# JeffreyXiang/ivid

Hardware: NVIDIA H100
Metric: 128x128 RGBD multiview samples/sec (higher is better)
Workload: dtype fp16 tensor-core operands, fp32 accumulate / residual stream / GroupNorm / softmax / sampler

## Files before the change

### include/ivid_b200.h

```cpp
#ifndef IVID_B200_H_
#define IVID_B200_H_

#include <stdint.h>

#ifdef __cplusplus
extern "C" {
#endif

#define IVID_OK 0
#define IVID_ERR_INVALID_ARGUMENT 1
#define IVID_ERR_NOT_IMPLEMENTED 2
#define IVID_ERR_CUDA 3
#define IVID_ERR_STATE 4

typedef struct ivid_unet ivid_unet_t;
typedef struct ivid_sampler ivid_sampler_t;

const char* ivid_last_error(void);
int ivid_version(void);
int ivid_device_info(int device, int* sm_count, int* cc_major, int* cc_minor);


int ivid_unet_create(const char* cfg_json, ivid_unet_t** out);
int ivid_unet_destroy(ivid_unet_t* h);

int ivid_unet_num_params(const ivid_unet_t* h, int* count);
int ivid_unet_param_info(const ivid_unet_t* h, int index, const char** name, int64_t shape[4], int* ndim,
                         int* is_buffer);
int ivid_unet_set_param(ivid_unet_t* h, const char* name, const float* host_data, const int64_t* shape, int ndim);
int ivid_unet_finalize(ivid_unet_t* h, int device);
int ivid_unet_set_precision(ivid_unet_t* h, int precision);
int ivid_fp8_e4m3_quantize(const float* in, uint8_t* out, uint64_t count);
int ivid_fp8_weight_exponent(const float* w, uint64_t count, int* e_out);
int ivid_unet_weight_arena(const ivid_unet_t* h, void** dev_ptr, uint64_t* bytes);

int ivid_unet_forward(ivid_unet_t* h, const float* x_dev, int Nx, const int64_t* t_dev, const int64_t* classes_dev,
                      float* eps_dev, int N, void* stream);

int ivid_conv_tile(int H, int W, int* tw, int* th, int* tn, int* fused_stats);

int ivid_unet_debug_tap(ivid_unet_t* h, int N, const char* layer, float* host_out, uint64_t capacity, int* C, int* H, int* W);

int ivid_unet_profile_begin(ivid_unet_t* h);
int ivid_unet_profile_end(ivid_unet_t* h, char* json_out, int capacity);

typedef struct {
  int kind;
  const float* y_dev;
  const float* mask_dev;
  const float* mask_rgb_dev;
  const float* noise_dev;
  uint64_t seed;
  uint32_t stream_id;
  int sr_scale;
} ivid_cond_t;
int ivid_unet_forward_cond(ivid_unet_t* h, const float* x_dev, int Nx, const ivid_cond_t* cond, const int64_t* t_dev,
                           const int64_t* classes_dev, float* eps_dev, int N, void* stream);

int ivid_unet_forward_hw(ivid_unet_t* h, const float* x_dev, int Nx, int H, int W, const ivid_cond_t* cond,
                         const int64_t* t_dev, const int64_t* classes_dev, float* eps_dev, int N, void* stream);

int ivid_unet_forward_reuse(ivid_unet_t* h, const float* x_dev, int Nx, int H, int W, const ivid_cond_t* cond,
                            const int64_t* t_dev, const int64_t* classes_dev, float* eps_dev, int N, int cache_branch,
                            void* stream);

int ivid_unet_forward_perturbed(ivid_unet_t* h, const float* x_dev, int Nx, int H, int W, const ivid_cond_t* cond,
                                const int64_t* t_dev, const int64_t* classes_dev, float* eps_dev, int N, int row0,
                                const int* layers_host, int num_layers, int cache_branch, void* stream);


int ivid_sampler_create(const double* betas, int timesteps, ivid_sampler_t** out);
int ivid_sampler_destroy(ivid_sampler_t* s);
int ivid_sampler_table(const ivid_sampler_t* s, int which, double* out, int count);

typedef struct {
  int kind;
  int use_cfg;
  float strength;
  int clip_denoised;
  float eta;
  const int64_t* classes_dev;
  ivid_cond_t cond;
  const float* replace_rgb_dev;
  const float* replace_rgb_mask_dev;
  double replace_rgb_weight;
  const float* replace_depth_dev;
  const float* replace_depth_mask_dev;
  double replace_depth_weight;
  const float* constrain_depth_dev;
  double constrain_depth_weight;
  const float* step_noise_dev;
  uint64_t seed;
  int height, width;
  int order;
  const float* prev_x0_dev;
  int t_last;
  int sde;
  int guidance_interval;
  int guidance_t_lo;
  int guidance_t_hi;
  int cache_interval;
  int cache_branch;
  int cache_reuse;
  int unipc;
  const float* prev2_x0_dev;
  int t_last2;
  const float* prev3_x0_dev;
  int t_last3;
  const float* prev_xt_dev;
  float* corrected_xt_dev;
  int pag;
  float pag_scale;
  const int* pag_layers;
  int pag_num_layers;
  int apg;
  double apg_eta;
  double apg_norm;
  double apg_momentum;
  float* apg_state_dev;
  int start_step;
  int dynamic_threshold;
  double threshold_ratio;
  double threshold_max;
} ivid_step_args_t;

int ivid_sampler_step(ivid_sampler_t* s, ivid_unet_t* unet, const float* x_t_dev, float* x_prev_dev,
                      float* pred_x0_dev, int N, int t, int t_prev, const ivid_step_args_t* args, void* stream);

int ivid_sampler_step_dev(ivid_sampler_t* s, ivid_unet_t* unet, const float* x_t_dev, float* x_prev_dev,
                          float* pred_x0_dev, int N, const int64_t* t_dev, const int64_t* t_prev_dev,
                          const ivid_step_args_t* args, void* stream);

int ivid_op_dynamic_threshold(const float* x_dev, int N, int M, double ratio, double threshold_max, float* s_out_dev,
                              float* x_out_dev, void* stream);

int ivid_op_apg(const float* d_c_dev, const float* d_u_dev, float* state_inout_dev, int N, int M, float s, double eta,
                double r, double beta, float* out_dev, void* stream);

int ivid_cfg_mix(const float* eps2n_dev, float strength, float* out_dev, uint64_t count, void* stream);

int ivid_guidance_mix(const float* eps_dev, uint64_t count, int cfg, float strength, int pag, float pag_scale, float* out_dev,
                      void* stream);

int ivid_sampler_run(ivid_sampler_t* s, ivid_unet_t* unet, float* x_inout_dev, int N, int steps,
                     const ivid_step_args_t* args, const float* noise_all_dev, const float* cond_noise_all_dev,
                     float* traj_x0_dev, float* traj_xt_dev, void* stream);

int ivid_sampler_diffuse(ivid_sampler_t* s, const float* x0_dev, const float* noise_dev, int N, uint64_t count_per_sample,
                         int t, uint64_t seed, float* out_dev, void* stream);

typedef struct ivid_warp ivid_warp_t;
typedef struct {
  double fov_deg;
  double near;
  double far;
  double atol;
  double rtol;
  int erode_rgb;
  double padding;
} ivid_warp_params_t;

int ivid_warp_create(int image_size, int render_size, int max_views, int batch, double near, double far, int device,
                     ivid_warp_t** out);
int ivid_warp_destroy(ivid_warp_t* w);
int ivid_warp_reset(ivid_warp_t* w);
int ivid_warp_num_views(const ivid_warp_t* w, int* n);
int ivid_warp_add_view(ivid_warp_t* w, const float* rgbd_dev, const float* modelviews_host, int shared_modelview,
                       const ivid_warp_params_t* params, void* stream);
int ivid_warp_mesh_from_depth(ivid_warp_t* w, const float* lin_depth_host, const float* modelview_host,
                              const ivid_warp_params_t* params, float* verts_host, uint32_t* faces_host, void* stream);
int ivid_warp_set_mesh(ivid_warp_t* w, int sample, int view, const float* verts_host, const uint32_t* faces_host,
                       const float* color_host, const float* modelview_host);
int ivid_warp_get_mesh(ivid_warp_t* w, int sample, int view, float* verts_host, uint32_t* faces_host, float* color_host);
int ivid_warp_render(ivid_warp_t* w, const float* target_mv_host, int shared_modelview, double fov_deg, float* color_dev,
                     float* depth_dev, float* mask_color_dev, float* mask_depth_dev, void* stream);
int ivid_warp_aggregate(ivid_warp_t* w, const float* target_mv_host, int shared_modelview, const ivid_warp_params_t* params,
                        float* cond_dev, void* stream);
int ivid_warp_postfilter(ivid_warp_t* w, const float* color_dev, const float* depth_dev, const float* mask_color_dev,
                         const float* mask_depth_dev, const ivid_warp_params_t* params, float* cond_dev, void* stream);

int ivid_warp_resolve_frame(ivid_warp_t* w, double project_near, double project_far, const uint8_t* lut_host, uint8_t* color8_host,
                            uint8_t* depth8_host, void* stream);

int ivid_warp_render_simple(ivid_warp_t* w, const float* verts_host, int nverts, const uint32_t* faces_host, int nfaces,
                            const float* color_host, const float* target_mv_host, double fov_deg, float* color_out_host,
                            float* depth_out_host, float* mask_out_host, void* stream);
int ivid_warp_forward_backward(ivid_warp_t* w, const float* lin_depth0_host, const float* color0_host, const float* mv1_host,
                               const float* mv0_host, int shared_modelview, const ivid_warp_params_t* params, float* out_host,
                               void* stream);

typedef struct {
  float origin[3];
  float voxel;
  int dims[3];
} ivid_fusion_grid_t;
int ivid_fusion_integrate(const float* depth_dev, const uint8_t* valid_dev, const float* color_dev, const float* modelviews_host,
                          int num_views, int image_size, float focal, const ivid_fusion_grid_t* grid, float trunc,
                          float* tsdf_sum_dev, float* weight_dev, float* color_sum_dev, float* color_weight_dev, void* stream);
int ivid_fusion_extract(const ivid_fusion_grid_t* grid, const float* tsdf_sum_dev, const float* weight_dev, const float* color_sum_dev,
                        const float* color_weight_dev, int64_t max_vertices, int64_t max_faces, float* vertices_dev,
                        uint8_t* colors_dev, int64_t* faces_dev, int64_t* num_vertices, int64_t* num_faces, void* stream);


int ivid_op_conv2d(const void* act_dev, int N, int H, int W, int Cin, const float* w_host, const float* bias_host,
                   int Cout, int ksize, const void* act2_dev, int Cin2, const float* w2_host, const float* bias2_host,
                   const float* residual_dev, void* out_dev, int out_fp16, void* stream);
int ivid_op_conv2d_e4m3(const void* act_dev, int N, int H, int W, int Cin, const float* w_host, const float* bias_host,
                        int Cout, int ksize, const void* act2_dev, int Cin2, const float* w2_host, const float* bias2_host,
                        const float* residual_dev, void* out_dev, int out_fp16, int* e_out, void* stream);
int ivid_op_group_norm(const float* x0_dev, int C0, const float* x1_dev, int C1, int N, int H, int W, int groups,
                       float eps, const float* gamma_host, const float* beta_host, const float* film_dev ,
                       int silu, int mode, void* out_fp16_dev, void* stream);
int ivid_op_group_norm_e4m3(const float* x0_dev, int C0, const float* x1_dev, int C1, int N, int H, int W, int groups,
                            float eps, const float* gamma_host, const float* beta_host, const float* film_dev,
                            int silu, int mode, void* out_e4m3_dev, void* stream);
typedef struct {
  const void* act0_dev; int C0; int ksize; const float* w0_host; const float* b0_host;
  int e4m3; int* e_out;
  const void* act1_dev; int C1; const void* act2_dev; int C2; const float* wskip_host; const float* bskip_host;
  const float* residual_dev; int residual_up;
  int N, H, W, Cout;
  void* out_dev; int out_mode; void* out16_dev; double* stats_dev;
} ivid_op_conv_t;
int ivid_op_conv2d_ex(const ivid_op_conv_t* args, void* stream);
typedef struct {
  const void* x0_dev; int C0; const void* x1_dev; int C1; int x_fp16;
  const double* stats0_dev; const double* stats1_dev;
  int N, H, W, groups; float eps;
  const float* gamma_host; const float* beta_host;
  const float* film_dev; int film_ld; int film_off; int film_add;
  int silu, mode;
  void* out_dev; int out_e4m3; void* out_lo_dev; void* out_raw16_dev; float* out_raw32_dev;
} ivid_op_gn_t;
int ivid_op_group_norm_apply(const ivid_op_gn_t* args, void* stream);
int ivid_op_gn_stats(const float* x_dev, int N, int H, int W, int C, double* stats_dev, void* stream);
typedef struct {
  int mode, conv;
  const void* x_dev; int N, H, W, C;
  const float* w_host; const float* b_host;
  float* out_dev; void* out16_dev; double* stats_dev; void* operand_dev;
} ivid_op_resample_t;
int ivid_op_resample(const ivid_op_resample_t* args, void* stream);
int ivid_op_attention(const void* qkv_dev, int N, int T, int C, void* out_dev, void* stream);
int ivid_op_attention_heads(const void* qkv_dev, int N, int T, int C, int head_channels, void* out_dev, void* stream);
int ivid_op_attention_perturbed(const void* qkv_dev, int N, int T, int C, int head_channels, int row0, void* out_dev,
                                void* stream);

#ifdef __cplusplus
}
#endif
#endif
```

### ivid_b200/_lib.py

```python
from __future__ import annotations

import ctypes
import os
from ctypes import POINTER, Structure, byref, c_char_p, c_double, c_float, c_int, c_int64, c_uint32, c_uint64, c_void_p

_HERE = os.path.dirname(os.path.abspath(__file__))
LIB_PATH = os.path.join(_HERE, "libivid_b200.so")

IVID_OK = 0
IVID_ERR_INVALID_ARGUMENT = 1
IVID_ERR_NOT_IMPLEMENTED = 2
IVID_ERR_CUDA = 3
IVID_ERR_STATE = 4


class CondT(Structure):
    _fields_ = [
        ("kind", c_int),
        ("y_dev", c_void_p),
        ("mask_dev", c_void_p),
        ("mask_rgb_dev", c_void_p),
        ("noise_dev", c_void_p),
        ("seed", c_uint64),
        ("stream_id", c_uint32),
        ("sr_scale", c_int),
    ]


class StepArgsT(Structure):
    _fields_ = [
        ("kind", c_int),
        ("use_cfg", c_int),
        ("strength", c_float),
        ("clip_denoised", c_int),
        ("eta", c_float),
        ("classes_dev", c_void_p),
        ("cond", CondT),
        ("replace_rgb_dev", c_void_p),
        ("replace_rgb_mask_dev", c_void_p),
        ("replace_rgb_weight", c_double),
        ("replace_depth_dev", c_void_p),
        ("replace_depth_mask_dev", c_void_p),
        ("replace_depth_weight", c_double),
        ("constrain_depth_dev", c_void_p),
        ("constrain_depth_weight", c_double),
        ("step_noise_dev", c_void_p),
        ("seed", c_uint64),
        ("height", c_int),
        ("width", c_int),
        ("order", c_int),
        ("prev_x0_dev", c_void_p),
        ("t_last", c_int),
        ("sde", c_int),
        ("guidance_interval", c_int),
        ("guidance_t_lo", c_int),
        ("guidance_t_hi", c_int),
        ("cache_interval", c_int),
        ("cache_branch", c_int),
        ("cache_reuse", c_int),
        ("unipc", c_int),
        ("prev2_x0_dev", c_void_p),
        ("t_last2", c_int),
        ("prev3_x0_dev", c_void_p),
        ("t_last3", c_int),
        ("prev_xt_dev", c_void_p),
        ("corrected_xt_dev", c_void_p),
        ("pag", c_int),
        ("pag_scale", c_float),
        ("pag_layers", POINTER(c_int)),
        ("pag_num_layers", c_int),
        ("apg", c_int),
        ("apg_eta", c_double),
        ("apg_norm", c_double),
        ("apg_momentum", c_double),
        ("apg_state_dev", c_void_p),
        ("start_step", c_int),
        ("dynamic_threshold", c_int),
        ("threshold_ratio", c_double),
        ("threshold_max", c_double),
    ]


class OpConvT(Structure):
    _fields_ = [
        ("act0_dev", c_void_p), ("C0", c_int), ("ksize", c_int), ("w0_host", c_void_p), ("b0_host", c_void_p),
        ("e4m3", c_int), ("e_out", POINTER(c_int)),
        ("act1_dev", c_void_p), ("C1", c_int), ("act2_dev", c_void_p), ("C2", c_int), ("wskip_host", c_void_p),
        ("bskip_host", c_void_p),
        ("residual_dev", c_void_p), ("residual_up", c_int),
        ("N", c_int), ("H", c_int), ("W", c_int), ("Cout", c_int),
        ("out_dev", c_void_p), ("out_mode", c_int), ("out16_dev", c_void_p), ("stats_dev", c_void_p),
    ]


class OpGnT(Structure):
    _fields_ = [
        ("x0_dev", c_void_p), ("C0", c_int), ("x1_dev", c_void_p), ("C1", c_int), ("x_fp16", c_int),
        ("stats0_dev", c_void_p), ("stats1_dev", c_void_p),
        ("N", c_int), ("H", c_int), ("W", c_int), ("groups", c_int), ("eps", c_float),
        ("gamma_host", c_void_p), ("beta_host", c_void_p),
        ("film_dev", c_void_p), ("film_ld", c_int), ("film_off", c_int), ("film_add", c_int),
        ("silu", c_int), ("mode", c_int),
        ("out_dev", c_void_p), ("out_e4m3", c_int), ("out_lo_dev", c_void_p), ("out_raw16_dev", c_void_p),
        ("out_raw32_dev", c_void_p),
    ]


class OpResampleT(Structure):
    _fields_ = [
        ("mode", c_int), ("conv", c_int),
        ("x_dev", c_void_p), ("N", c_int), ("H", c_int), ("W", c_int), ("C", c_int),
        ("w_host", c_void_p), ("b_host", c_void_p),
        ("out_dev", c_void_p), ("out16_dev", c_void_p), ("stats_dev", c_void_p), ("operand_dev", c_void_p),
    ]


class WarpParamsT(Structure):
    _fields_ = [("fov_deg", c_double), ("near", c_double), ("far", c_double), ("atol", c_double), ("rtol", c_double),
                ("erode_rgb", c_int), ("padding", c_double)]


class FusionGridT(Structure):
    _fields_ = [("origin", c_float * 3), ("voxel", c_float), ("dims", c_int * 3)]


SIGNATURES = {
    "ivid_last_error": (c_char_p, []),
    "ivid_version": (c_int, []),
    "ivid_device_info": (c_int, [c_int, POINTER(c_int), POINTER(c_int), POINTER(c_int)]),
    "ivid_unet_create": (c_int, [c_char_p, POINTER(c_void_p)]),
    "ivid_unet_destroy": (c_int, [c_void_p]),
    "ivid_unet_num_params": (c_int, [c_void_p, POINTER(c_int)]),
    "ivid_unet_param_info": (c_int, [c_void_p, c_int, POINTER(c_char_p), POINTER(c_int64), POINTER(c_int), POINTER(c_int)]),
    "ivid_unet_set_param": (c_int, [c_void_p, c_char_p, c_void_p, POINTER(c_int64), c_int]),
    "ivid_unet_finalize": (c_int, [c_void_p, c_int]),
    "ivid_unet_weight_arena": (c_int, [c_void_p, POINTER(c_void_p), POINTER(c_uint64)]),
    "ivid_unet_set_precision": (c_int, [c_void_p, c_int]),
    "ivid_fp8_e4m3_quantize": (c_int, [c_void_p, c_void_p, c_uint64]),
    "ivid_fp8_weight_exponent": (c_int, [c_void_p, c_uint64, POINTER(c_int)]),
    "ivid_unet_forward": (c_int, [c_void_p, c_void_p, c_int, c_void_p, c_void_p, c_void_p, c_int, c_void_p]),
    "ivid_unet_forward_cond": (c_int, [c_void_p, c_void_p, c_int, POINTER(CondT), c_void_p, c_void_p, c_void_p, c_int, c_void_p]),
    "ivid_unet_forward_hw": (c_int, [c_void_p, c_void_p, c_int, c_int, c_int, POINTER(CondT), c_void_p, c_void_p, c_void_p, c_int,
                                     c_void_p]),
    "ivid_unet_forward_reuse": (c_int, [c_void_p, c_void_p, c_int, c_int, c_int, POINTER(CondT), c_void_p, c_void_p, c_void_p,
                                        c_int, c_int, c_void_p]),
    "ivid_unet_forward_perturbed": (c_int, [c_void_p, c_void_p, c_int, c_int, c_int, POINTER(CondT), c_void_p, c_void_p, c_void_p,
                                            c_int, c_int, POINTER(c_int), c_int, c_int, c_void_p]),
    "ivid_conv_tile": (c_int, [c_int, c_int, POINTER(c_int), POINTER(c_int), POINTER(c_int), POINTER(c_int)]),
    "ivid_unet_debug_tap": (c_int, [c_void_p, c_int, c_char_p, c_void_p, c_uint64, POINTER(c_int), POINTER(c_int), POINTER(c_int)]),
    "ivid_unet_profile_begin": (c_int, [c_void_p]),
    "ivid_unet_profile_end": (c_int, [c_void_p, c_char_p, c_int]),
    "ivid_sampler_create": (c_int, [POINTER(c_double), c_int, POINTER(c_void_p)]),
    "ivid_sampler_destroy": (c_int, [c_void_p]),
    "ivid_sampler_table": (c_int, [c_void_p, c_int, POINTER(c_double), c_int]),
    "ivid_sampler_step": (c_int, [c_void_p, c_void_p, c_void_p, c_void_p, c_void_p, c_int, c_int, c_int, POINTER(StepArgsT), c_void_p]),
    "ivid_sampler_step_dev": (c_int, [c_void_p, c_void_p, c_void_p, c_void_p, c_void_p, c_int, c_void_p, c_void_p, POINTER(StepArgsT), c_void_p]),
    "ivid_cfg_mix": (c_int, [c_void_p, c_float, c_void_p, c_uint64, c_void_p]),
    "ivid_guidance_mix": (c_int, [c_void_p, c_uint64, c_int, c_float, c_int, c_float, c_void_p, c_void_p]),
    "ivid_op_dynamic_threshold": (c_int, [c_void_p, c_int, c_int, c_double, c_double, c_void_p, c_void_p, c_void_p]),
    "ivid_op_apg": (c_int, [c_void_p, c_void_p, c_void_p, c_int, c_int, c_float, c_double, c_double, c_double, c_void_p, c_void_p]),
    "ivid_sampler_run": (c_int, [c_void_p, c_void_p, c_void_p, c_int, c_int, POINTER(StepArgsT), c_void_p, c_void_p, c_void_p, c_void_p, c_void_p]),
    "ivid_sampler_diffuse": (c_int, [c_void_p, c_void_p, c_void_p, c_int, c_uint64, c_int, c_uint64, c_void_p, c_void_p]),
    "ivid_op_conv2d": (c_int, [c_void_p, c_int, c_int, c_int, c_int, c_void_p, c_void_p, c_int, c_int, c_void_p, c_int,
                               c_void_p, c_void_p, c_void_p, c_void_p, c_int, c_void_p]),
    "ivid_op_group_norm": (c_int, [c_void_p, c_int, c_void_p, c_int, c_int, c_int, c_int, c_int, c_float, c_void_p, c_void_p,
                                   c_void_p, c_int, c_int, c_void_p, c_void_p]),
    "ivid_op_conv2d_e4m3": (c_int, [c_void_p, c_int, c_int, c_int, c_int, c_void_p, c_void_p, c_int, c_int, c_void_p, c_int,
                                    c_void_p, c_void_p, c_void_p, c_void_p, c_int, POINTER(c_int), c_void_p]),
    "ivid_op_group_norm_e4m3": (c_int, [c_void_p, c_int, c_void_p, c_int, c_int, c_int, c_int, c_int, c_float, c_void_p,
                                        c_void_p, c_void_p, c_int, c_int, c_void_p, c_void_p]),
    "ivid_op_conv2d_ex": (c_int, [POINTER(OpConvT), c_void_p]),
    "ivid_op_group_norm_apply": (c_int, [POINTER(OpGnT), c_void_p]),
    "ivid_op_gn_stats": (c_int, [c_void_p, c_int, c_int, c_int, c_int, c_void_p, c_void_p]),
    "ivid_op_resample": (c_int, [POINTER(OpResampleT), c_void_p]),
    "ivid_op_attention": (c_int, [c_void_p, c_int, c_int, c_int, c_void_p, c_void_p]),
    "ivid_op_attention_heads": (c_int, [c_void_p, c_int, c_int, c_int, c_int, c_void_p, c_void_p]),
    "ivid_op_attention_perturbed": (c_int, [c_void_p, c_int, c_int, c_int, c_int, c_int, c_void_p, c_void_p]),
    "ivid_warp_create": (c_int, [c_int, c_int, c_int, c_int, c_double, c_double, c_int, POINTER(c_void_p)]),
    "ivid_warp_destroy": (c_int, [c_void_p]),
    "ivid_warp_reset": (c_int, [c_void_p]),
    "ivid_warp_num_views": (c_int, [c_void_p, POINTER(c_int)]),
    "ivid_warp_add_view": (c_int, [c_void_p, c_void_p, c_void_p, c_int, POINTER(WarpParamsT), c_void_p]),
    "ivid_warp_mesh_from_depth": (c_int, [c_void_p, c_void_p, c_void_p, POINTER(WarpParamsT), c_void_p, c_void_p, c_void_p]),
    "ivid_warp_set_mesh": (c_int, [c_void_p, c_int, c_int, c_void_p, c_void_p, c_void_p, c_void_p]),
    "ivid_warp_get_mesh": (c_int, [c_void_p, c_int, c_int, c_void_p, c_void_p, c_void_p]),
    "ivid_warp_render": (c_int, [c_void_p, c_void_p, c_int, c_double, c_void_p, c_void_p, c_void_p, c_void_p, c_void_p]),
    "ivid_warp_aggregate": (c_int, [c_void_p, c_void_p, c_int, POINTER(WarpParamsT), c_void_p, c_void_p]),
    "ivid_warp_resolve_frame": (c_int, [c_void_p, c_double, c_double, c_void_p, c_void_p, c_void_p, c_void_p]),
    "ivid_warp_render_simple": (c_int, [c_void_p, c_void_p, c_int, c_void_p, c_int, c_void_p, c_void_p, c_double, c_void_p, c_void_p, c_void_p, c_void_p]),
    "ivid_warp_forward_backward": (c_int, [c_void_p, c_void_p, c_void_p, c_void_p, c_void_p, c_int, POINTER(WarpParamsT), c_void_p, c_void_p]),
    "ivid_warp_postfilter": (c_int, [c_void_p, c_void_p, c_void_p, c_void_p, c_void_p, POINTER(WarpParamsT), c_void_p, c_void_p]),
    "ivid_fusion_integrate": (c_int, [c_void_p, c_void_p, c_void_p, c_void_p, c_int, c_int, c_float, POINTER(FusionGridT), c_float,
                                      c_void_p, c_void_p, c_void_p, c_void_p, c_void_p]),
    "ivid_fusion_extract": (c_int, [POINTER(FusionGridT), c_void_p, c_void_p, c_void_p, c_void_p, c_int64, c_int64, c_void_p, c_void_p,
                                    c_void_p, POINTER(c_int64), POINTER(c_int64), c_void_p]),
}

_lib = None


def lib() -> ctypes.CDLL:
    global _lib
    if _lib is None:
        if not os.path.exists(LIB_PATH):
            raise ImportError(
                f"{LIB_PATH} not found: build it with `python -m ivid_b200.build` (ivid_b200 has no CPU fallback)")
        l = ctypes.CDLL(LIB_PATH)
        for name, (res, args) in SIGNATURES.items():
            try:
                fn = getattr(l, name)
            except AttributeError:
                continue
            fn.restype = res
            fn.argtypes = args
        _lib = l
    return _lib


def last_error() -> str:
    m = lib().ivid_last_error()
    return m.decode() if m else ""


def check(status: int) -> None:
    if status == IVID_OK:
        return
    msg = last_error()
    if status == IVID_ERR_INVALID_ARGUMENT:
        raise AssertionError(msg)
    if status == IVID_ERR_NOT_IMPLEMENTED:
        raise NotImplementedError(msg)
    raise RuntimeError(f"ivid_b200 native error {status}: {msg}")


def ptr(t) -> c_void_p:
    if t is None:
        return c_void_p(None)
    return c_void_p(t.data_ptr())


def cur_stream(device=None) -> c_void_p:
    import torch
    return c_void_p(torch.cuda.current_stream(device).cuda_stream)
```

### ivid_b200/csrc/api.cu

```cuda
#include <algorithm>
#include <cmath>
#include <cstring>
#include <memory>
#include <string>
#include <vector>

#include "../../include/ivid_b200.h"
#include "ops.h"
#include "sampler.h"
#include "unet.h"

using namespace ivid;

struct ivid_unet { std::unique_ptr<Unet> impl; };
struct ivid_sampler { std::unique_ptr<Sampler> impl; };

static thread_local std::string g_last_error;
namespace ivid { void set_last_error(const std::string& msg) { g_last_error = msg; } }

template <class F>
static int guarded(F&& f) {
  try {
    f();
    return IVID_OK;
  } catch (const Error& e) {
    g_last_error = e.what();
    return e.code;
  } catch (const std::exception& e) {
    g_last_error = e.what();
    return IVID_ERR_STATE;
  } catch (...) {
    g_last_error = "unknown error";
    return IVID_ERR_STATE;
  }
}

#define IVID_NOT_NULL(p) IVID_REQUIRE((p) != nullptr, #p " must not be NULL")

extern "C" {

const char* ivid_last_error(void) { return g_last_error.c_str(); }
int ivid_version(void) { return 100; }

int ivid_device_info(int device, int* sm_count_out, int* cc_major, int* cc_minor) {
  return guarded([&] {
    cudaDeviceProp prop;
    IVID_CHECK_CUDA(cudaGetDeviceProperties(&prop, device));
    if (sm_count_out) *sm_count_out = prop.multiProcessorCount;
    if (cc_major) *cc_major = prop.major;
    if (cc_minor) *cc_minor = prop.minor;
  });
}

int ivid_unet_create(const char* cfg_json, ivid_unet_t** out) {
  return guarded([&] {
    IVID_NOT_NULL(cfg_json);
    IVID_NOT_NULL(out);
    auto h = std::make_unique<ivid_unet>();
    h->impl = std::make_unique<Unet>(std::string(cfg_json));
    *out = h.release();
  });
}
int ivid_unet_destroy(ivid_unet_t* h) {
  return guarded([&] { delete h; });
}
int ivid_unet_num_params(const ivid_unet_t* h, int* count) {
  return guarded([&] {
    IVID_NOT_NULL(h); IVID_NOT_NULL(count);
    *count = static_cast<int>(h->impl->params().size());
  });
}
int ivid_unet_param_info(const ivid_unet_t* h, int index, const char** name, int64_t shape[4], int* ndim, int* is_buffer) {
  return guarded([&] {
    IVID_NOT_NULL(h);
    const auto& ps = h->impl->params();
    IVID_REQUIRE(index >= 0 && index < static_cast<int>(ps.size()), "parameter index out of range");
    const ParamSpec& p = ps[index];
    if (name) *name = p.name.c_str();
    if (ndim) *ndim = static_cast<int>(p.shape.size());
    if (shape) for (size_t i = 0; i < 4; ++i) shape[i] = i < p.shape.size() ? p.shape[i] : 1;
    if (is_buffer) *is_buffer = p.is_buffer ? 1 : 0;
  });
}
int ivid_unet_set_param(ivid_unet_t* h, const char* name, const float* host_data, const int64_t* shape, int ndim) {
  return guarded([&] {
    IVID_NOT_NULL(h); IVID_NOT_NULL(name); IVID_NOT_NULL(host_data); IVID_NOT_NULL(shape);
    h->impl->set_param(name, host_data, shape, ndim);
  });
}
int ivid_unet_finalize(ivid_unet_t* h, int device) {
  return guarded([&] {
    IVID_NOT_NULL(h);
    h->impl->finalize(device);
  });
}
int ivid_unet_set_precision(ivid_unet_t* h, int precision) {
  return guarded([&] {
    IVID_NOT_NULL(h);
    h->impl->set_precision(precision);
  });
}
int ivid_fp8_e4m3_quantize(const float* in, uint8_t* out, uint64_t count) {
  return guarded([&] {
    IVID_REQUIRE(count == 0 || (in != nullptr && out != nullptr), "in and out must not be NULL");
    for (uint64_t i = 0; i < count; ++i) out[i] = fp8_e4m3_from_float(in[i]);
  });
}
int ivid_fp8_weight_exponent(const float* w, uint64_t count, int* e_out) {
  return guarded([&] {
    IVID_REQUIRE(count == 0 || w != nullptr, "w must not be NULL");
    IVID_NOT_NULL(e_out);
    float mx = 0.f;
    for (uint64_t i = 0; i < count; ++i) mx = std::max(mx, std::fabs(w[i]));
    *e_out = fp8_weight_exponent(mx);
  });
}
int ivid_unet_weight_arena(const ivid_unet_t* h, void** dev_ptr, uint64_t* bytes) {
  return guarded([&] {
    IVID_NOT_NULL(h);
    if (!h->impl->finalized()) throw Error(kErrState, "weight arena requested before finalize");
    if (dev_ptr) *dev_ptr = h->impl->arena();
    if (bytes) *bytes = h->impl->arena_bytes();
  });
}
int ivid_unet_forward_hw(ivid_unet_t* h, const float* x_dev, int Nx, int H, int W, const ivid_cond_t* cond,
                         const int64_t* t_dev, const int64_t* classes_dev, float* eps_dev, int N, void* stream) {
  return guarded([&] {
    IVID_NOT_NULL(h); IVID_NOT_NULL(x_dev); IVID_NOT_NULL(t_dev); IVID_NOT_NULL(eps_dev);
    h->impl->forward(x_dev, Nx, H, W, cond, t_dev, classes_dev, eps_dev, N, static_cast<cudaStream_t>(stream));
  });
}
int ivid_unet_forward_reuse(ivid_unet_t* h, const float* x_dev, int Nx, int H, int W, const ivid_cond_t* cond,
                            const int64_t* t_dev, const int64_t* classes_dev, float* eps_dev, int N, int cache_branch,
                            void* stream) {
  return guarded([&] {
    IVID_NOT_NULL(h); IVID_NOT_NULL(x_dev); IVID_NOT_NULL(t_dev); IVID_NOT_NULL(eps_dev);
    IVID_REQUIRE(cache_branch >= 0, "cache_branch must be in [0, num_res_blocks]");
    h->impl->forward(x_dev, Nx, H, W, cond, t_dev, classes_dev, eps_dev, N, static_cast<cudaStream_t>(stream), nullptr,
                     cache_branch);
  });
}
int ivid_unet_forward_perturbed(ivid_unet_t* h, const float* x_dev, int Nx, int H, int W, const ivid_cond_t* cond,
                                const int64_t* t_dev, const int64_t* classes_dev, float* eps_dev, int N, int row0,
                                const int* layers_host, int num_layers, int cache_branch, void* stream) {
  return guarded([&] {
    IVID_NOT_NULL(h); IVID_NOT_NULL(x_dev); IVID_NOT_NULL(t_dev); IVID_NOT_NULL(eps_dev);
    IVID_REQUIRE(num_layers >= 1 && layers_host != nullptr, "perturbed forward: at least one attention layer");
    IVID_REQUIRE(row0 >= 0 && row0 <= N, "perturbed forward: row0 must lie in [0, N]");
    AttnPerturb pert;
    pert.row0 = row0;
    pert.layers.assign(layers_host, layers_host + num_layers);
    h->impl->forward(x_dev, Nx, H, W, cond, t_dev, classes_dev, eps_dev, N, static_cast<cudaStream_t>(stream), nullptr,
                     cache_branch, &pert);
  });
}
int ivid_unet_forward(ivid_unet_t* h, const float* x_dev, int Nx, const int64_t* t_dev, const int64_t* classes_dev,
                      float* eps_dev, int N, void* stream) {
  const int S = h != nullptr ? h->impl->cfg().image_size : 0;
  return ivid_unet_forward_hw(h, x_dev, Nx, S, S, nullptr, t_dev, classes_dev, eps_dev, N, stream);
}
int ivid_unet_forward_cond(ivid_unet_t* h, const float* x_dev, int Nx, const ivid_cond_t* cond, const int64_t* t_dev,
                           const int64_t* classes_dev, float* eps_dev, int N, void* stream) {
  if (cond == nullptr) return guarded([&] { IVID_NOT_NULL(cond); });
  const int S = h != nullptr ? h->impl->cfg().image_size : 0;
  return ivid_unet_forward_hw(h, x_dev, Nx, S, S, cond, t_dev, classes_dev, eps_dev, N, stream);
}

int ivid_conv_tile(int H, int W, int* tw, int* th, int* tn, int* fused_stats) {
  return guarded([&] {
    int a, b, c;
    conv_tile(H, W, &a, &b, &c);
    if (tw) *tw = a;
    if (th) *th = b;
    if (tn) *tn = c;
    if (fused_stats) *fused_stats = conv_can_fuse_stats(H, W) ? 1 : 0;
  });
}

int ivid_unet_debug_tap(ivid_unet_t* h, int N, const char* layer, float* host_out, uint64_t capacity, int* C, int* H, int* W) {
  return guarded([&] {
    IVID_NOT_NULL(h); IVID_NOT_NULL(layer);
    h->impl->debug_tap(N, layer, host_out, static_cast<size_t>(capacity), C, H, W);
  });
}

int ivid_unet_profile_begin(ivid_unet_t* h) {
  return guarded([&] { IVID_NOT_NULL(h); h->impl->profile_begin(); });
}
int ivid_unet_profile_end(ivid_unet_t* h, char* json_out, int capacity) {
  return guarded([&] {
    IVID_NOT_NULL(h); IVID_NOT_NULL(json_out);
    const std::string js = h->impl->profile_end();
    IVID_REQUIRE(static_cast<int>(js.size()) < capacity, "profile buffer too small");
    std::memcpy(json_out, js.c_str(), js.size() + 1);
  });
}

int ivid_sampler_create(const double* betas, int timesteps, ivid_sampler_t** out) {
  return guarded([&] {
    IVID_NOT_NULL(betas); IVID_NOT_NULL(out);
    auto s = std::make_unique<ivid_sampler>();
    s->impl = std::make_unique<Sampler>(betas, timesteps);
    *out = s.release();
  });
}
int ivid_sampler_destroy(ivid_sampler_t* s) {
  return guarded([&] { delete s; });
}
int ivid_sampler_table(const ivid_sampler_t* s, int which, double* out, int count) {
  return guarded([&] {
    IVID_NOT_NULL(s); IVID_NOT_NULL(out);
    const auto& t = s->impl->table(which);
    IVID_REQUIRE(count == static_cast<int>(t.size()), "table length mismatch");
    std::memcpy(out, t.data(), sizeof(double) * t.size());
  });
}
int ivid_sampler_step(ivid_sampler_t* s, ivid_unet_t* unet, const float* x_t_dev, float* x_prev_dev, float* pred_x0_dev,
                      int N, int t, int t_prev, const ivid_step_args_t* args, void* stream) {
  return guarded([&] {
    IVID_NOT_NULL(s); IVID_NOT_NULL(unet); IVID_NOT_NULL(x_t_dev); IVID_NOT_NULL(x_prev_dev); IVID_NOT_NULL(args);
    s->impl->step(*unet->impl, x_t_dev, x_prev_dev, pred_x0_dev, N, t, t_prev, *args, t, static_cast<cudaStream_t>(stream));
  });
}
int ivid_sampler_step_dev(ivid_sampler_t* s, ivid_unet_t* unet, const float* x_t_dev, float* x_prev_dev, float* pred_x0_dev,
                          int N, const int64_t* t_dev, const int64_t* t_prev_dev, const ivid_step_args_t* args, void* stream) {
  return guarded([&] {
    IVID_NOT_NULL(s); IVID_NOT_NULL(unet); IVID_NOT_NULL(x_t_dev); IVID_NOT_NULL(x_prev_dev); IVID_NOT_NULL(args); IVID_NOT_NULL(t_dev);
    IVID_REQUIRE(args->kind == 0 || t_prev_dev != nullptr, "DDIM / DPM-Solver++ step needs t_prev");
    s->impl->step(*unet->impl, x_t_dev, x_prev_dev, pred_x0_dev, N, 0, 0, *args, 0, static_cast<cudaStream_t>(stream), t_dev, t_prev_dev);
  });
}
int ivid_cfg_mix(const float* eps2n_dev, float strength, float* out_dev, uint64_t count, void* stream) {
  return guarded([&] {
    IVID_NOT_NULL(eps2n_dev); IVID_NOT_NULL(out_dev);
    launch_cfg_mix(eps2n_dev, out_dev, static_cast<size_t>(count), strength, static_cast<cudaStream_t>(stream));
  });
}
int ivid_guidance_mix(const float* eps_dev, uint64_t count, int cfg, float strength, int pag, float pag_scale, float* out_dev,
                      void* stream) {
  return guarded([&] {
    IVID_NOT_NULL(eps_dev); IVID_NOT_NULL(out_dev);
    launch_guidance_mix(eps_dev, out_dev, static_cast<size_t>(count), cfg, strength, pag, pag_scale, static_cast<cudaStream_t>(stream));
  });
}
int ivid_op_dynamic_threshold(const float* x_dev, int N, int M, double ratio, double threshold_max, float* s_out_dev,
                              float* x_out_dev, void* stream) {
  return guarded([&] {
    IVID_NOT_NULL(x_dev); IVID_NOT_NULL(s_out_dev); IVID_NOT_NULL(x_out_dev);
    cudaStream_t st = static_cast<cudaStream_t>(stream);
    launch_dynamic_threshold(x_dev, N, M, ratio, threshold_max, s_out_dev, x_out_dev, st);
    IVID_CHECK_CUDA(cudaStreamSynchronize(st));
  });
}
int ivid_op_apg(const float* d_c_dev, const float* d_u_dev, float* state_inout_dev, int N, int M, float s, double eta,
                double r, double beta, float* out_dev, void* stream) {
  return guarded([&] {
    IVID_NOT_NULL(d_c_dev); IVID_NOT_NULL(d_u_dev); IVID_NOT_NULL(state_inout_dev); IVID_NOT_NULL(out_dev);
    cudaStream_t st = static_cast<cudaStream_t>(stream);
    launch_apg(d_c_dev, d_u_dev, state_inout_dev, N, M, s, eta, r, beta, out_dev, st);
    IVID_CHECK_CUDA(cudaStreamSynchronize(st));
  });
}
int ivid_sampler_run(ivid_sampler_t* s, ivid_unet_t* unet, float* x_inout_dev, int N, int steps,
                     const ivid_step_args_t* args, const float* noise_all_dev, const float* cond_noise_all_dev,
                     float* traj_x0_dev, float* traj_xt_dev, void* stream) {
  return guarded([&] {
    IVID_NOT_NULL(s); IVID_NOT_NULL(unet); IVID_NOT_NULL(x_inout_dev); IVID_NOT_NULL(args);
    s->impl->run(*unet->impl, x_inout_dev, N, steps, *args, noise_all_dev, cond_noise_all_dev, traj_x0_dev, traj_xt_dev,
                 static_cast<cudaStream_t>(stream));
  });
}
int ivid_sampler_diffuse(ivid_sampler_t* s, const float* x0_dev, const float* noise_dev, int N, uint64_t count_per_sample,
                         int t, uint64_t seed, float* out_dev, void* stream) {
  return guarded([&] {
    IVID_NOT_NULL(s); IVID_NOT_NULL(x0_dev); IVID_NOT_NULL(out_dev);
    s->impl->diffuse(x0_dev, noise_dev, N, static_cast<size_t>(count_per_sample), t, seed, out_dev,
                     static_cast<cudaStream_t>(stream));
  });
}

namespace {
struct DevBuf {
  void* p = nullptr;
  explicit DevBuf(size_t bytes) { if (bytes > 0) IVID_CHECK_CUDA(cudaMalloc(&p, bytes)); }
  ~DevBuf() { if (p) cudaFree(p); }
  DevBuf(const DevBuf&) = delete;
};
}

int ivid_op_conv2d_ex(const ivid_op_conv_t* a, void* stream) {
  return guarded([&] {
    IVID_NOT_NULL(a);
    IVID_NOT_NULL(a->act0_dev); IVID_NOT_NULL(a->w0_host); IVID_NOT_NULL(a->out_dev);
    IVID_REQUIRE(a->ksize == 3 || a->ksize == 1, "conv: kernel size must be 3 or 1");
    IVID_REQUIRE(a->C0 > 0 && a->C0 % 8 == 0 && a->C1 % 8 == 0 && a->C2 % 8 == 0, "conv: channels must be multiples of 8");
    IVID_REQUIRE(a->act1_dev == nullptr || a->wskip_host != nullptr, "conv: a skip input needs its weights (w2_host; wskip_host of ivid_op_conv2d_ex)");
    IVID_REQUIRE(a->act2_dev == nullptr || (a->act1_dev != nullptr && a->C2 > 0), "conv: act2_dev is the second part of a skip over act1_dev");
    IVID_REQUIRE(a->out_mode >= 0 && a->out_mode <= 2, "conv: out_mode must be 0, 1 or 2");
    const int C1 = a->act1_dev ? a->C1 : 0, C2 = a->act2_dev ? a->C2 : 0;
    const ConvPack pk = conv_pack(a->w0_host, a->b0_host, a->Cout, a->C0, a->ksize, conv_pad_k(a->C0), C1 ? a->wskip_host : nullptr,
                                  C1 ? a->bskip_host : nullptr, C1 + C2, C2 ? C1 : 0, a->e4m3 != 0);
    if (pk.refused != nullptr) throw Error(kErrInvalidArgument, std::string("conv: no e4m3 form: ") + pk.refused);
    cudaStream_t st = static_cast<cudaStream_t>(stream);
    DevBuf dw8(pk.w8.size()), dw(pk.w16.size() * 2), db(pk.bias.size() * 4);
    if (pk.e4m3) IVID_CHECK_CUDA(cudaMemcpyAsync(dw8.p, pk.w8.data(), pk.w8.size(), cudaMemcpyHostToDevice, st));
    if (pk.K > 0) IVID_CHECK_CUDA(cudaMemcpyAsync(dw.p, pk.w16.data(), pk.w16.size() * 2, cudaMemcpyHostToDevice, st));
    IVID_CHECK_CUDA(cudaMemcpyAsync(db.p, pk.bias.data(), pk.bias.size() * 4, cudaMemcpyHostToDevice, st));
    ConvDesc d;
    d.act0 = a->act0_dev; d.C0 = a->C0; d.taps0 = a->ksize * a->ksize;
    if (C1) { d.act1 = a->act1_dev; d.C1 = C1; d.taps1 = 1; }
    if (C2) { d.act2 = a->act2_dev; d.C2 = C2; d.taps2 = 1; }
    d.weight = dw.p; d.weight8 = dw8.p; d.acc_scale = std::ldexp(1.0f, -pk.e);
    d.cout_pad = pk.cout_pad; d.cout = a->Cout; d.bias = static_cast<const float*>(db.p);
    d.residual = a->residual_dev; d.ldr = a->Cout; d.residual_up = a->residual_up != 0;
    d.out = a->out_dev; d.ldc = a->Cout; d.out_mode = a->out_mode; d.out16 = a->out16_dev; d.stats = a->stats_dev;
    d.N = a->N; d.H = a->H; d.W = a->W;
    std::unique_ptr<ConvLaunch, void (*)(ConvLaunch*)> l(conv_launch_create(d), conv_launch_destroy);
    conv_launch_run(l.get(), st);
    IVID_CHECK_CUDA(cudaStreamSynchronize(st));
    if (a->e_out) *a->e_out = pk.e;
  });
}

static int op_conv2d(const void* act_dev, int N, int H, int W, int Cin, const float* w_host, const float* bias_host, int Cout,
                     int ksize, const void* act2_dev, int Cin2, const float* w2_host, const float* bias2_host,
                     const float* residual_dev, void* out_dev, int out_fp16, bool e4m3, int* e_out, void* stream) {
  ivid_op_conv_t a{};
  a.act0_dev = act_dev; a.C0 = Cin; a.ksize = ksize; a.w0_host = w_host; a.b0_host = bias_host;
  a.e4m3 = e4m3 ? 1 : 0; a.e_out = e_out;
  a.act1_dev = act2_dev; a.C1 = act2_dev ? Cin2 : 0; a.wskip_host = w2_host; a.bskip_host = bias2_host;
  a.residual_dev = residual_dev;
  a.N = N; a.H = H; a.W = W; a.Cout = Cout;
  a.out_dev = out_dev; a.out_mode = out_fp16 ? 1 : 0;
  return ivid_op_conv2d_ex(&a, stream);
}

int ivid_op_conv2d(const void* act_dev, int N, int H, int W, int Cin, const float* w_host, const float* bias_host,
                   int Cout, int ksize, const void* act2_dev, int Cin2, const float* w2_host, const float* bias2_host,
                   const float* residual_dev, void* out_dev, int out_fp16, void* stream) {
  return op_conv2d(act_dev, N, H, W, Cin, w_host, bias_host, Cout, ksize, act2_dev, Cin2, w2_host, bias2_host, residual_dev,
                   out_dev, out_fp16, false, nullptr, stream);
}
int ivid_op_conv2d_e4m3(const void* act_dev, int N, int H, int W, int Cin, const float* w_host, const float* bias_host,
                        int Cout, int ksize, const void* act2_dev, int Cin2, const float* w2_host, const float* bias2_host,
                        const float* residual_dev, void* out_dev, int out_fp16, int* e_out, void* stream) {
  return op_conv2d(act_dev, N, H, W, Cin, w_host, bias_host, Cout, ksize, act2_dev, Cin2, w2_host, bias2_host, residual_dev,
                   out_dev, out_fp16, true, e_out, stream);
}

int ivid_op_group_norm_apply(const ivid_op_gn_t* a, void* stream) {
  return guarded([&] {
    IVID_NOT_NULL(a);
    IVID_NOT_NULL(a->x0_dev); IVID_NOT_NULL(a->gamma_host); IVID_NOT_NULL(a->beta_host); IVID_NOT_NULL(a->out_dev);
    const int N = a->N, HW = a->H * a->W, C0 = a->C0, C1 = a->x1_dev ? a->C1 : 0, C = C0 + C1;
    IVID_REQUIRE(N > 0 && HW > 0 && C0 > 0, "group norm: empty tensor");
    IVID_REQUIRE(a->film_dev == nullptr || a->film_ld >= a->film_off + (a->film_add ? C : 2 * C),
                 "group norm: the FiLM row (film_off + C, or + 2C with a shift) must fit film_ld");
    const bool need0 = a->stats0_dev == nullptr, need1 = C1 > 0 && a->stats1_dev == nullptr;
    IVID_REQUIRE(!(need0 || need1) || !a->x_fp16, "group norm: statistics of fp16 sources must be supplied");
    cudaStream_t st = static_cast<cudaStream_t>(stream);
    DevBuf dg(C * 4), dbt(C * 4), st0(need0 ? static_cast<size_t>(N) * C0 * 16 : 0), st1(need1 ? static_cast<size_t>(N) * C1 * 16 : 0);
    IVID_CHECK_CUDA(cudaMemcpyAsync(dg.p, a->gamma_host, C * 4, cudaMemcpyHostToDevice, st));
    IVID_CHECK_CUDA(cudaMemcpyAsync(dbt.p, a->beta_host, C * 4, cudaMemcpyHostToDevice, st));
    if (need0) {
      IVID_CHECK_CUDA(cudaMemsetAsync(st0.p, 0, static_cast<size_t>(N) * C0 * 16, st));
      launch_gn_stats(static_cast<const float*>(a->x0_dev), static_cast<double*>(st0.p), N, HW, C0, st);
    }
    if (need1) {
      IVID_CHECK_CUDA(cudaMemsetAsync(st1.p, 0, static_cast<size_t>(N) * C1 * 16, st));
      launch_gn_stats(static_cast<const float*>(a->x1_dev), static_cast<double*>(st1.p), N, HW, C1, st);
    }
    GnApplyDesc g;
    g.x0 = a->x0_dev; g.x1 = C1 > 0 ? a->x1_dev : nullptr; g.C0 = C0; g.C1 = C1; g.x0_half = a->x_fp16 != 0;
    g.N = N; g.H = a->H; g.W = a->W; g.mode = a->mode; g.silu = a->silu;
    g.stats0 = need0 ? static_cast<const double*>(st0.p) : a->stats0_dev;
    g.stats1 = C1 == 0 ? nullptr : (need1 ? static_cast<const double*>(st1.p) : a->stats1_dev);
    g.groups = a->groups; g.eps = a->eps; g.gamma = static_cast<float*>(dg.p); g.beta = static_cast<float*>(dbt.p);
    g.film = a->film_dev; g.film_ld = a->film_ld; g.film_off = a->film_off; g.film_add = a->film_add != 0;
    g.out_act = a->out_dev; g.out_e4m3 = a->out_e4m3 != 0; g.out_lo = a->out_lo_dev;
    g.out_raw16 = a->out_raw16_dev; g.out_raw32 = a->out_raw32_dev;
    launch_gn_apply(g, st);
    IVID_CHECK_CUDA(cudaStreamSynchronize(st));
  });
}

int ivid_op_gn_stats(const float* x_dev, int N, int H, int W, int C, double* stats_dev, void* stream) {
  return guarded([&] {
    IVID_NOT_NULL(x_dev); IVID_NOT_NULL(stats_dev);
    IVID_REQUIRE(N > 0 && N <= 65535 && H > 0 && W > 0 && C > 0 && C % 4 == 0,
                 "gn_stats: N in [1, 65535], positive H and W, C a positive multiple of 4");
    cudaStream_t st = static_cast<cudaStream_t>(stream);
    launch_gn_stats(x_dev, stats_dev, N, H * W, C, st);
    IVID_CHECK_CUDA(cudaStreamSynchronize(st));
  });
}

int ivid_op_resample(const ivid_op_resample_t* a, void* stream) {
  return guarded([&] {
    IVID_NOT_NULL(a);
    IVID_NOT_NULL(a->x_dev); IVID_NOT_NULL(a->out_dev);
    IVID_REQUIRE(a->mode == 1 || a->mode == 2, "resample: mode must be 1 (up) or 2 (down)");
    IVID_REQUIRE(a->conv == 0 || a->conv == 1, "resample: conv must be 0 or 1");
    const int N = a->N, H = a->H, W = a->W, C = a->C;
    IVID_REQUIRE(N > 0 && N <= 65535 && H > 0 && W > 0 && C > 0 && C % 8 == 0,
                 "resample: N in [1, 65535], positive H and W, C a positive multiple of 8");
    IVID_REQUIRE(a->mode == 1 || (H % 2 == 0 && W % 2 == 0), "resample: downsampling needs an even H and W");
    IVID_REQUIRE(a->conv == 1 || a->operand_dev == nullptr, "resample: operand_dev belongs to the conv forms");
    if (a->conv) IVID_NOT_NULL(a->w_host);
    const int Ho = a->mode == 1 ? 2 * H : H / 2, Wo = a->mode == 1 ? 2 * W : W / 2;
    cudaStream_t st = static_cast<cudaStream_t>(stream);
    if (a->conv) {
      const ConvPack pk = conv_pack(a->w_host, a->b_host, C, C, 3, a->mode == 2 ? C : conv_pad_k(C), nullptr, nullptr, 0, 0, false);
      const size_t op_elems = static_cast<size_t>(N) * Ho * Wo * (a->mode == 2 ? 9 * C : C);
      DevBuf dw(pk.w16.size() * 2), db(pk.bias.size() * 4), dop(a->operand_dev ? 0 : op_elems * 2);
      void* opnd = a->operand_dev ? a->operand_dev : dop.p;
      IVID_CHECK_CUDA(cudaMemcpyAsync(dw.p, pk.w16.data(), pk.w16.size() * 2, cudaMemcpyHostToDevice, st));
      IVID_CHECK_CUDA(cudaMemcpyAsync(db.p, pk.bias.data(), pk.bias.size() * 4, cudaMemcpyHostToDevice, st));
      ConvDesc d;
      d.act0 = opnd; d.C0 = a->mode == 2 ? 9 * C : C; d.taps0 = a->mode == 2 ? 1 : 9;
      d.weight = dw.p; d.cout_pad = pk.cout_pad; d.cout = C; d.bias = static_cast<const float*>(db.p);
      d.out = a->out_dev; d.out16 = a->out16_dev; d.out_mode = 0; d.ldc = C; d.N = N; d.H = Ho; d.W = Wo;
      const bool fused = a->stats_dev != nullptr && conv_can_fuse_stats(Ho, Wo);
      if (fused) d.stats = a->stats_dev;
      std::unique_ptr<ConvLaunch, void (*)(ConvLaunch*)> l(conv_launch_create(d), conv_launch_destroy);
      if (a->mode == 2) launch_im2col_s2(a->x_dev, opnd, N, H, W, C, st);
      else launch_upsample2x_h16(a->x_dev, opnd, N, H, W, C, st);
      conv_launch_run(l.get(), st);
      if (a->stats_dev != nullptr && !fused) launch_gn_stats(a->out_dev, a->stats_dev, N, Ho * Wo, C, st);
    } else {
      launch_resample_f32(static_cast<const float*>(a->x_dev), a->out_dev, a->out16_dev, N, H, W, C, a->mode, st);
      if (a->stats_dev != nullptr) launch_gn_stats(a->out_dev, a->stats_dev, N, Ho * Wo, C, st);
    }
    IVID_CHECK_CUDA(cudaStreamSynchronize(st));
  });
}

static int op_group_norm(const float* x0_dev, int C0, const float* x1_dev, int C1, int N, int H, int W, int groups,
                         float eps, const float* gamma_host, const float* beta_host, const float* film_dev, int silu,
                         int mode, void* out_dev, bool e4m3, void* stream) {
  ivid_op_gn_t a{};
  a.x0_dev = x0_dev; a.C0 = C0; a.x1_dev = x1_dev; a.C1 = x1_dev ? C1 : 0;
  a.N = N; a.H = H; a.W = W; a.groups = groups; a.eps = eps; a.gamma_host = gamma_host; a.beta_host = beta_host;
  a.film_dev = film_dev; a.film_ld = 2 * (a.C0 + a.C1); a.film_off = 0;
  a.silu = silu; a.mode = mode; a.out_dev = out_dev; a.out_e4m3 = e4m3 ? 1 : 0;
  return ivid_op_group_norm_apply(&a, stream);
}

int ivid_op_group_norm(const float* x0_dev, int C0, const float* x1_dev, int C1, int N, int H, int W, int groups,
                       float eps, const float* gamma_host, const float* beta_host, const float* film_dev, int silu,
                       int mode, void* out_fp16_dev, void* stream) {
  return op_group_norm(x0_dev, C0, x1_dev, C1, N, H, W, groups, eps, gamma_host, beta_host, film_dev, silu, mode, out_fp16_dev,
                       false, stream);
}
int ivid_op_group_norm_e4m3(const float* x0_dev, int C0, const float* x1_dev, int C1, int N, int H, int W, int groups,
                            float eps, const float* gamma_host, const float* beta_host, const float* film_dev, int silu,
                            int mode, void* out_e4m3_dev, void* stream) {
  return op_group_norm(x0_dev, C0, x1_dev, C1, N, H, W, groups, eps, gamma_host, beta_host, film_dev, silu, mode, out_e4m3_dev,
                       true, stream);
}

int ivid_op_attention(const void* qkv_dev, int N, int T, int C, void* out_dev, void* stream) {
  return guarded([&] {
    IVID_NOT_NULL(qkv_dev); IVID_NOT_NULL(out_dev);
    cudaStream_t st = static_cast<cudaStream_t>(stream);
    std::unique_ptr<AttnLaunch, void (*)(AttnLaunch*)> l(attn_launch_create(qkv_dev, N, T, C, 64, out_dev), attn_launch_destroy);
    attn_launch_run(l.get(), st);
    IVID_CHECK_CUDA(cudaStreamSynchronize(st));
  });
}

int ivid_op_attention_heads(const void* qkv_dev, int N, int T, int C, int head_channels, void* out_dev, void* stream) {
  return guarded([&] {
    IVID_NOT_NULL(qkv_dev); IVID_NOT_NULL(out_dev);
    cudaStream_t st = static_cast<cudaStream_t>(stream);
    std::unique_ptr<AttnLaunch, void (*)(AttnLaunch*)> l(attn_launch_create(qkv_dev, N, T, C, head_channels, out_dev), attn_launch_destroy);
    attn_launch_run(l.get(), st);
    IVID_CHECK_CUDA(cudaStreamSynchronize(st));
  });
}

int ivid_op_attention_perturbed(const void* qkv_dev, int N, int T, int C, int head_channels, int row0, void* out_dev,
                                void* stream) {
  return guarded([&] {
    IVID_NOT_NULL(qkv_dev); IVID_NOT_NULL(out_dev);
    IVID_REQUIRE(row0 >= 0 && row0 <= N, "attention: row0 must lie in [0, N]");
    cudaStream_t st = static_cast<cudaStream_t>(stream);
    std::unique_ptr<AttnLaunch, void (*)(AttnLaunch*)> l(attn_launch_create(qkv_dev, N, T, C, head_channels, out_dev, row0),
                                                         attn_launch_destroy);
    attn_launch_run(l.get(), st);
    IVID_CHECK_CUDA(cudaStreamSynchronize(st));
  });
}

}
```

### ivid_b200/csrc/common.cuh

```cuda
#pragma once
#include <cuda.h>
#include <cuda_fp16.h>
#include <cuda_fp8.h>
#include <cuda_runtime.h>
#include <stdint.h>

namespace ivid {

__device__ __forceinline__ uint32_t smem_u32(const void* p) {
  return static_cast<uint32_t>(__cvta_generic_to_shared(p));
}

__device__ __forceinline__ float silu_f(float x) {
  float e, r;
  asm("ex2.approx.ftz.f32 %0, %1;" : "=f"(e) : "f"(x * -1.4426950408889634f));
  asm("rcp.approx.ftz.f32 %0, %1;" : "=f"(r) : "f"(1.0f + e));
  return x * r;
}

__device__ __forceinline__ __half split_term(float v, int seg) {
  const __half hi = __float2half_rn(v);
  return seg == 1 ? __float2half_rn(v - __half2float(hi)) : hi;
}

__device__ __forceinline__ void mbar_init(uint64_t* bar, uint32_t count) {
  asm volatile("mbarrier.init.shared::cta.b64 [%0], %1;\n" ::"r"(smem_u32(bar)), "r"(count));
}
__device__ __forceinline__ void fence_barrier_init() {
  asm volatile("fence.mbarrier_init.release.cluster;\n" ::: "memory");
}
__device__ __forceinline__ void fence_proxy_async_smem() {
  asm volatile("fence.proxy.async.shared::cta;\n" ::: "memory");
}
__device__ __forceinline__ void mbar_arrive_expect_tx(uint64_t* bar, uint32_t bytes) {
  asm volatile("mbarrier.arrive.expect_tx.shared::cta.b64 _, [%0], %1;\n" ::"r"(smem_u32(bar)), "r"(bytes)
               : "memory");
}
__device__ __forceinline__ void mbar_arrive(uint64_t* bar) {
  asm volatile("mbarrier.arrive.shared::cta.b64 _, [%0];\n" ::"r"(smem_u32(bar)) : "memory");
}
#ifndef IVID_MBAR_SPIN_LIMIT
#define IVID_MBAR_SPIN_LIMIT (1u << 26)
#endif
__device__ __forceinline__ void mbar_wait(uint64_t* bar, uint32_t parity) {
  uint32_t done = 0;
  uint32_t spins = 0;
  const uint32_t addr = smem_u32(bar);
  while (true) {
    asm volatile(
        "{\n\t"
        ".reg .pred p;\n\t"
        "mbarrier.try_wait.parity.shared::cta.b64 p, [%1], %2;\n\t"
        "selp.b32 %0, 1, 0, p;\n\t"
        "}\n"
        : "=r"(done)
        : "r"(addr), "r"(parity)
        : "memory");
    if (done) break;
    if (++spins > IVID_MBAR_SPIN_LIMIT) { __trap(); }
  }
}

__device__ __forceinline__ void bulk_load_1d(void* dst, const void* src, uint32_t bytes, uint64_t* bar) {
  asm volatile("cp.async.bulk.shared::cluster.global.mbarrier::complete_tx::bytes [%0], [%1], %2, [%3];\n" ::"r"(smem_u32(dst)),
               "l"(src), "r"(bytes), "r"(smem_u32(bar))
               : "memory");
}

__device__ __forceinline__ void tma_prefetch_desc(const CUtensorMap* m) {
  asm volatile("prefetch.tensormap [%0];\n" ::"l"(reinterpret_cast<uint64_t>(m)) : "memory");
}
__device__ __forceinline__ void tma_load_2d(const CUtensorMap* m, uint64_t* bar, void* dst, int c0, int c1) {
  asm volatile(
      "cp.async.bulk.tensor.2d.shared::cluster.global.mbarrier::complete_tx::bytes [%0], [%1, {%3, %4}], [%2];\n"
      ::"r"(smem_u32(dst)), "l"(reinterpret_cast<uint64_t>(m)), "r"(smem_u32(bar)), "r"(c0), "r"(c1)
      : "memory");
}
__device__ __forceinline__ void tma_load_3d(const CUtensorMap* m, uint64_t* bar, void* dst, int c0, int c1, int c2) {
  asm volatile(
      "cp.async.bulk.tensor.3d.shared::cluster.global.mbarrier::complete_tx::bytes [%0], [%1, {%3, %4, %5}], [%2];\n"
      ::"r"(smem_u32(dst)), "l"(reinterpret_cast<uint64_t>(m)), "r"(smem_u32(bar)), "r"(c0), "r"(c1), "r"(c2)
      : "memory");
}
__device__ __forceinline__ void tma_load_4d(const CUtensorMap* m, uint64_t* bar, void* dst, int c0, int c1, int c2,
                                            int c3) {
  asm volatile(
      "cp.async.bulk.tensor.4d.shared::cluster.global.mbarrier::complete_tx::bytes [%0], [%1, {%3, %4, %5, %6}], "
      "[%2];\n" ::"r"(smem_u32(dst)),
      "l"(reinterpret_cast<uint64_t>(m)), "r"(smem_u32(bar)), "r"(c0), "r"(c1), "r"(c2), "r"(c3)
      : "memory");
}
__device__ __forceinline__ void tma_prefetch_l2_4d(const CUtensorMap* m, int c0, int c1, int c2, int c3) {
  asm volatile("cp.async.bulk.prefetch.tensor.4d.L2.global.tile [%0, {%1, %2, %3, %4}];\n" ::"l"(reinterpret_cast<uint64_t>(m)),
               "r"(c0), "r"(c1), "r"(c2), "r"(c3)
               : "memory");
}
__device__ __forceinline__ void tma_store_4d(const CUtensorMap* m, const void* src, int c0, int c1, int c2, int c3) {
  asm volatile("cp.async.bulk.tensor.4d.global.shared::cta.bulk_group [%0, {%2, %3, %4, %5}], [%1];\n" ::"l"(
                   reinterpret_cast<uint64_t>(m)),
               "r"(smem_u32(src)), "r"(c0), "r"(c1), "r"(c2), "r"(c3)
               : "memory");
}
__device__ __forceinline__ void tma_store_commit() { asm volatile("cp.async.bulk.commit_group;\n" ::: "memory"); }
__device__ __forceinline__ void tma_store_wait_read() { asm volatile("cp.async.bulk.wait_group.read 0;\n" ::: "memory"); }

__device__ __forceinline__ void wgmma_fence() { asm volatile("wgmma.fence.sync.aligned;\n" ::: "memory"); }
__device__ __forceinline__ void wgmma_commit() { asm volatile("wgmma.commit_group.sync.aligned;\n" ::: "memory"); }
template <int kPending>
__device__ __forceinline__ void wgmma_wait() { asm volatile("wgmma.wait_group.sync.aligned %0;\n" ::"n"(kPending) : "memory"); }
template <int R>
__device__ __forceinline__ void reg_fence(float (&d)[R]) {
#pragma unroll
  for (int i = 0; i < R; ++i) asm volatile("" : "+f"(d[i])::"memory");
}

__device__ __forceinline__ uint64_t make_smem_desc_sw128(uint32_t smem_addr, uint32_t sbo_bytes, uint32_t lbo_bytes) {
  uint64_t d = 0;
  d |= static_cast<uint64_t>((smem_addr & 0x3FFFF) >> 4);
  d |= static_cast<uint64_t>((lbo_bytes >> 4) & 0x3FFF) << 16;
  d |= static_cast<uint64_t>((sbo_bytes >> 4) & 0x3FFF) << 32;
  d |= static_cast<uint64_t>(1) << 62;
  return d;
}

template <int N>
__device__ void wgmma_ss(float (&d)[N / 2], uint64_t desc_a, uint64_t desc_b, uint32_t scale_d);
template <int N>
__device__ void wgmma_rs_tb(float (&d)[N / 2], const uint32_t (&a)[4], uint64_t desc_b, uint32_t scale_d);
template <>
__device__ __forceinline__ void wgmma_ss<16>(float (&d)[8], uint64_t desc_a, uint64_t desc_b, uint32_t scale_d) {
  asm volatile(
      "{\n\t.reg .pred p;\n\tsetp.ne.b32 p, %10, 0;\n\t"
      "wgmma.mma_async.sync.aligned.m64n16k16.f32.f16.f16 {%0, %1, %2, %3, %4, %5, %6, %7}, %8, %9, p, 1, 1, 0, 0;\n\t}\n"
      : "+f"(d[0]), "+f"(d[1]), "+f"(d[2]), "+f"(d[3]), "+f"(d[4]), "+f"(d[5]), "+f"(d[6]), "+f"(d[7])
      : "l"(desc_a), "l"(desc_b), "r"(scale_d));
}
template <>
__device__ __forceinline__ void wgmma_ss<64>(float (&d)[32], uint64_t desc_a, uint64_t desc_b, uint32_t scale_d) {
  asm volatile(
      "{\n\t.reg .pred p;\n\tsetp.ne.b32 p, %34, 0;\n\t"
      "wgmma.mma_async.sync.aligned.m64n64k16.f32.f16.f16 {%0, %1, %2, %3, %4, %5, %6, %7, %8, %9, %10, %11, %12, %13, %14, %15, %16, %17, %18, %19, %20, %21, %22, %23, %24, %25, %26, %27, %28, %29, %30, %31}, %32, %33, p, 1, 1, 0, 0;\n\t}\n"
      : "+f"(d[0]), "+f"(d[1]), "+f"(d[2]), "+f"(d[3]), "+f"(d[4]), "+f"(d[5]), "+f"(d[6]), "+f"(d[7]), "+f"(d[8]), "+f"(d[9]), "+f"(d[10]), "+f"(d[11]), "+f"(d[12]), "+f"(d[13]), "+f"(d[14]), "+f"(d[15]), "+f"(d[16]), "+f"(d[17]), "+f"(d[18]), "+f"(d[19]), "+f"(d[20]), "+f"(d[21]), "+f"(d[22]), "+f"(d[23]), "+f"(d[24]), "+f"(d[25]), "+f"(d[26]), "+f"(d[27]), "+f"(d[28]), "+f"(d[29]), "+f"(d[30]), "+f"(d[31])
      : "l"(desc_a), "l"(desc_b), "r"(scale_d));
}
template <>
__device__ __forceinline__ void wgmma_ss<128>(float (&d)[64], uint64_t desc_a, uint64_t desc_b, uint32_t scale_d) {
  asm volatile(
      "{\n\t.reg .pred p;\n\tsetp.ne.b32 p, %66, 0;\n\t"
      "wgmma.mma_async.sync.aligned.m64n128k16.f32.f16.f16 {%0, %1, %2, %3, %4, %5, %6, %7, %8, %9, %10, %11, %12, %13, %14, %15, %16, %17, %18, %19, %20, %21, %22, %23, %24, %25, %26, %27, %28, %29, %30, %31, %32, %33, %34, %35, %36, %37, %38, %39, %40, %41, %42, %43, %44, %45, %46, %47, %48, %49, %50, %51, %52, %53, %54, %55, %56, %57, %58, %59, %60, %61, %62, %63}, %64, %65, p, 1, 1, 0, 0;\n\t}\n"
      : "+f"(d[0]), "+f"(d[1]), "+f"(d[2]), "+f"(d[3]), "+f"(d[4]), "+f"(d[5]), "+f"(d[6]), "+f"(d[7]), "+f"(d[8]), "+f"(d[9]), "+f"(d[10]), "+f"(d[11]), "+f"(d[12]), "+f"(d[13]), "+f"(d[14]), "+f"(d[15]), "+f"(d[16]), "+f"(d[17]), "+f"(d[18]), "+f"(d[19]), "+f"(d[20]), "+f"(d[21]), "+f"(d[22]), "+f"(d[23]), "+f"(d[24]), "+f"(d[25]), "+f"(d[26]), "+f"(d[27]), "+f"(d[28]), "+f"(d[29]), "+f"(d[30]), "+f"(d[31]), "+f"(d[32]), "+f"(d[33]), "+f"(d[34]), "+f"(d[35]), "+f"(d[36]), "+f"(d[37]), "+f"(d[38]), "+f"(d[39]), "+f"(d[40]), "+f"(d[41]), "+f"(d[42]), "+f"(d[43]), "+f"(d[44]), "+f"(d[45]), "+f"(d[46]), "+f"(d[47]), "+f"(d[48]), "+f"(d[49]), "+f"(d[50]), "+f"(d[51]), "+f"(d[52]), "+f"(d[53]), "+f"(d[54]), "+f"(d[55]), "+f"(d[56]), "+f"(d[57]), "+f"(d[58]), "+f"(d[59]), "+f"(d[60]), "+f"(d[61]), "+f"(d[62]), "+f"(d[63])
      : "l"(desc_a), "l"(desc_b), "r"(scale_d));
}
template <>
__device__ __forceinline__ void wgmma_rs_tb<64>(float (&d)[32], const uint32_t (&a)[4], uint64_t desc_b, uint32_t scale_d) {
  asm volatile(
      "{\n\t.reg .pred p;\n\tsetp.ne.b32 p, %37, 0;\n\t"
      "wgmma.mma_async.sync.aligned.m64n64k16.f32.f16.f16 {%0, %1, %2, %3, %4, %5, %6, %7, %8, %9, %10, %11, %12, %13, %14, %15, %16, %17, %18, %19, %20, %21, %22, %23, %24, %25, %26, %27, %28, %29, %30, %31}, {%32, %33, %34, %35}, %36, p, 1, 1, 1;\n\t}\n"
      : "+f"(d[0]), "+f"(d[1]), "+f"(d[2]), "+f"(d[3]), "+f"(d[4]), "+f"(d[5]), "+f"(d[6]), "+f"(d[7]), "+f"(d[8]), "+f"(d[9]), "+f"(d[10]), "+f"(d[11]), "+f"(d[12]), "+f"(d[13]), "+f"(d[14]), "+f"(d[15]), "+f"(d[16]), "+f"(d[17]), "+f"(d[18]), "+f"(d[19]), "+f"(d[20]), "+f"(d[21]), "+f"(d[22]), "+f"(d[23]), "+f"(d[24]), "+f"(d[25]), "+f"(d[26]), "+f"(d[27]), "+f"(d[28]), "+f"(d[29]), "+f"(d[30]), "+f"(d[31])
      : "r"(a[0]), "r"(a[1]), "r"(a[2]), "r"(a[3]), "l"(desc_b), "r"(scale_d));
}


template <int N>
__device__ void wgmma_ss_e4m3(float (&d)[N / 2], uint64_t desc_a, uint64_t desc_b, uint32_t scale_d);
template <>
__device__ __forceinline__ void wgmma_ss_e4m3<16>(float (&d)[8], uint64_t desc_a, uint64_t desc_b, uint32_t scale_d) {
  asm volatile(
      "{\n\t.reg .pred p;\n\tsetp.ne.b32 p, %10, 0;\n\t"
      "wgmma.mma_async.sync.aligned.m64n16k32.f32.e4m3.e4m3 {%0, %1, %2, %3, %4, %5, %6, %7}, %8, %9, p, 1, 1;\n\t}\n"
      : "+f"(d[0]), "+f"(d[1]), "+f"(d[2]), "+f"(d[3]), "+f"(d[4]), "+f"(d[5]), "+f"(d[6]), "+f"(d[7])
      : "l"(desc_a), "l"(desc_b), "r"(scale_d));
}
template <>
__device__ __forceinline__ void wgmma_ss_e4m3<64>(float (&d)[32], uint64_t desc_a, uint64_t desc_b, uint32_t scale_d) {
  asm volatile(
      "{\n\t.reg .pred p;\n\tsetp.ne.b32 p, %34, 0;\n\t"
      "wgmma.mma_async.sync.aligned.m64n64k32.f32.e4m3.e4m3 {%0, %1, %2, %3, %4, %5, %6, %7, %8, %9, %10, %11, %12, %13, %14, %15, %16, %17, %18, %19, %20, %21, %22, %23, %24, %25, %26, %27, %28, %29, %30, %31}, %32, %33, p, 1, 1;\n\t}\n"
      : "+f"(d[0]), "+f"(d[1]), "+f"(d[2]), "+f"(d[3]), "+f"(d[4]), "+f"(d[5]), "+f"(d[6]), "+f"(d[7]), "+f"(d[8]), "+f"(d[9]), "+f"(d[10]), "+f"(d[11]), "+f"(d[12]), "+f"(d[13]), "+f"(d[14]), "+f"(d[15]), "+f"(d[16]), "+f"(d[17]), "+f"(d[18]), "+f"(d[19]), "+f"(d[20]), "+f"(d[21]), "+f"(d[22]), "+f"(d[23]), "+f"(d[24]), "+f"(d[25]), "+f"(d[26]), "+f"(d[27]), "+f"(d[28]), "+f"(d[29]), "+f"(d[30]), "+f"(d[31])
      : "l"(desc_a), "l"(desc_b), "r"(scale_d));
}
template <>
__device__ __forceinline__ void wgmma_ss_e4m3<128>(float (&d)[64], uint64_t desc_a, uint64_t desc_b, uint32_t scale_d) {
  asm volatile(
      "{\n\t.reg .pred p;\n\tsetp.ne.b32 p, %66, 0;\n\t"
      "wgmma.mma_async.sync.aligned.m64n128k32.f32.e4m3.e4m3 {%0, %1, %2, %3, %4, %5, %6, %7, %8, %9, %10, %11, %12, %13, %14, %15, %16, %17, %18, %19, %20, %21, %22, %23, %24, %25, %26, %27, %28, %29, %30, %31, %32, %33, %34, %35, %36, %37, %38, %39, %40, %41, %42, %43, %44, %45, %46, %47, %48, %49, %50, %51, %52, %53, %54, %55, %56, %57, %58, %59, %60, %61, %62, %63}, %64, %65, p, 1, 1;\n\t}\n"
      : "+f"(d[0]), "+f"(d[1]), "+f"(d[2]), "+f"(d[3]), "+f"(d[4]), "+f"(d[5]), "+f"(d[6]), "+f"(d[7]), "+f"(d[8]), "+f"(d[9]), "+f"(d[10]), "+f"(d[11]), "+f"(d[12]), "+f"(d[13]), "+f"(d[14]), "+f"(d[15]), "+f"(d[16]), "+f"(d[17]), "+f"(d[18]), "+f"(d[19]), "+f"(d[20]), "+f"(d[21]), "+f"(d[22]), "+f"(d[23]), "+f"(d[24]), "+f"(d[25]), "+f"(d[26]), "+f"(d[27]), "+f"(d[28]), "+f"(d[29]), "+f"(d[30]), "+f"(d[31]), "+f"(d[32]), "+f"(d[33]), "+f"(d[34]), "+f"(d[35]), "+f"(d[36]), "+f"(d[37]), "+f"(d[38]), "+f"(d[39]), "+f"(d[40]), "+f"(d[41]), "+f"(d[42]), "+f"(d[43]), "+f"(d[44]), "+f"(d[45]), "+f"(d[46]), "+f"(d[47]), "+f"(d[48]), "+f"(d[49]), "+f"(d[50]), "+f"(d[51]), "+f"(d[52]), "+f"(d[53]), "+f"(d[54]), "+f"(d[55]), "+f"(d[56]), "+f"(d[57]), "+f"(d[58]), "+f"(d[59]), "+f"(d[60]), "+f"(d[61]), "+f"(d[62]), "+f"(d[63])
      : "l"(desc_a), "l"(desc_b), "r"(scale_d));
}

__device__ __forceinline__ float4 ldg_f4(const float* p) { return __ldg(reinterpret_cast<const float4*>(p)); }
__device__ __forceinline__ void stg_f4(float* p, float4 v) { *reinterpret_cast<float4*>(p) = v; }
__device__ __forceinline__ uint32_t pack_h2(float a, float b) {
  __half2 h = __floats2half2_rn(a, b);
  return *reinterpret_cast<uint32_t*>(&h);
}
__device__ __forceinline__ uint16_t pack_e4m3x2(float a, float b) {
  return static_cast<uint16_t>(__nv_cvt_float2_to_fp8x2(make_float2(a, b), __NV_SATFINITE, __NV_E4M3));
}

}
```

### ivid_b200/csrc/conv_gemm.cuh

```cuda
#pragma once
#include <type_traits>

#include "common.cuh"

namespace ivid {

struct ConvGemmParams {
  int N, H, W;
  int TW, TH, TN;
  int tiles_w, tiles_h, tiles_n;
  int n_blocks;
  int seg_chunks[3];
  int seg_taps[3];
  int Cout;
  int ldc;
  int ldr;
  int out_mode;
  const float* bias;
  const float* residual;
  int res_up;
  void* out;
  __half* out16;
  double* stats;
  float acc_scale;
};

struct ConvMaps {
  CUtensorMap a[3];
  CUtensorMap b;
  CUtensorMap r;
  CUtensorMap o;
  CUtensorMap o16;
};
struct ConvMaps8 : ConvMaps {
  CUtensorMap b8;
};

template <int BN, bool SLAB = false>
struct ConvGemmCfg {
  static constexpr int BM = 128;
  static constexpr int BK = 64;
  static constexpr int A_BYTES = BM * BK * 2;
  static constexpr int B_BYTES = ((BN * BK * 2 + 1023) / 1024) * 1024;
  static constexpr int STAGE_BYTES = A_BYTES + B_BYTES;
  static constexpr int STAGES = BN == 128 && !SLAB ? 3 : 4;
  static constexpr int SLAB_BYTES = 16 * 10 * 128;
  static constexpr int SLAB_STAGES = 2;
  static constexpr int RING_BYTES = SLAB ? SLAB_STAGES * SLAB_BYTES + STAGES * B_BYTES : STAGES * STAGE_BYTES;
  static constexpr int BAR_BYTES = 128;
  static constexpr int STAT_BYTES = 8 * 2 * BN * 4;
  static constexpr bool STATS_ON_RING = SLAB;
  static constexpr int SMEM_BYTES = RING_BYTES + BAR_BYTES + (STATS_ON_RING ? 0 : STAT_BYTES) + 1024;
  static constexpr int CONSUMER_THREADS = 256;
  static constexpr int THREADS = CONSUMER_THREADS + 32;

  static constexpr int F32_CH = SLAB ? BN / 4 : (BN < 32 ? BN : 32);
  static constexpr int F32_BOX = BM * F32_CH * 4;
  static constexpr int UNIT_BOXES = !SLAB && BN == 128 ? 2 : 1;
  static constexpr int UNIT_CH = F32_CH * UNIT_BOXES;
  static constexpr int UNITS = BN / UNIT_CH;
  static constexpr int UNIT_STRIDE = SLAB ? B_BYTES : STAGE_BYTES;
  static constexpr int F16_CH = BN < 64 ? BN : 64;
  static constexpr int F16_BOX = BM * F16_CH * 2;
  static constexpr int F16_TILE = BM * BN * 2;
  static_assert(UNIT_BOXES * F32_BOX <= UNIT_STRIDE, "an fp32 unit must fit its ring slot");
  static_assert(SLAB ? UNITS == STAGES : UNITS < STAGES && F16_TILE <= STAGE_BYTES, "fp32 units and the fp16 tile must fit the ring");
  static_assert(!SLAB || F16_TILE + STAT_BYTES <= SLAB_STAGES * SLAB_BYTES, "the fp16 tile and statistics must fit the slab slots");
};

struct ConvKCursor {
  int seg = 0, t = 0, ch = 0, base = 0;
};

template <int BN, bool A8 = false, bool SLAB = false>
__global__ void __launch_bounds__(ConvGemmCfg<BN>::THREADS, 2)
conv_gemm_kernel(const __grid_constant__ std::conditional_t<A8, ConvMaps8, ConvMaps> maps, const __grid_constant__ ConvGemmParams p) {
  using Cfg = ConvGemmCfg<BN, SLAB>;
  constexpr int STAGES = Cfg::STAGES;
  constexpr int SLAB_STAGES = Cfg::SLAB_STAGES;
  extern __shared__ uint8_t smem_raw[];
  uint8_t* smem = smem_raw + ((1024u - (smem_u32(smem_raw) & 1023u)) & 1023u);
  uint64_t* full_bar = reinterpret_cast<uint64_t*>(smem + Cfg::RING_BYTES);
  uint64_t* empty_bar = full_bar + STAGES;
  uint64_t* slab_full = empty_bar + STAGES;
  uint64_t* slab_empty = slab_full + SLAB_STAGES;
  float* stat_smem = reinterpret_cast<float*>(Cfg::STATS_ON_RING ? smem + Cfg::F16_TILE : smem + Cfg::RING_BYTES + Cfg::BAR_BYTES);
  uint8_t* const slab_ring = smem;
  uint8_t* const w_ring = smem + SLAB_STAGES * Cfg::SLAB_BYTES;

  const int tid = threadIdx.x;
  const int warp = tid >> 5, lane = tid & 31;
  const int wg = warp >> 2;

  if (tid == 0) {
    for (int s = 0; s < STAGES; ++s) {
      mbar_init(&full_bar[s], 1);
      mbar_init(&empty_bar[s], 8u);
    }
    if constexpr (SLAB) {
      for (int s = 0; s < SLAB_STAGES; ++s) {
        mbar_init(&slab_full[s], 1);
        mbar_init(&slab_empty[s], 8u);
      }
    }
    fence_barrier_init();
  }
  __syncthreads();

  int nunits = 0;
  for (int sg = 0; sg < 3; ++sg) nunits += p.seg_chunks[sg] * p.seg_taps[sg];
  const int nunits8 = A8 ? p.seg_chunks[0] * p.seg_taps[0] : 0;

  const int mt = static_cast<int>(blockIdx.x) / p.n_blocks, nb = static_cast<int>(blockIdx.x) % p.n_blocks;
  const int colbase = nb * BN;
  const int tiles_per_img = p.tiles_w * p.tiles_h;
  const int tn = mt / tiles_per_img;
  const int rem = mt - tn * tiles_per_img;
  const int th = rem / p.tiles_w;
  const int tw = rem - th * p.tiles_w;
  const int n0 = tn * p.TN, h0 = th * p.TH, w0 = tw * p.TW;
  uint8_t* const unit_ring = SLAB ? w_ring : smem;

  if (warp == Cfg::CONSUMER_THREADS / 32) {
    if (lane == 0) {
      const int rw0 = p.res_up ? w0 >> 1 : w0, rh0 = p.res_up ? h0 >> 1 : h0;
      tma_prefetch_desc(&maps.a[0]);
      tma_prefetch_desc(&maps.b);
      if constexpr (A8) tma_prefetch_desc(&maps.b8);
      if (p.residual != nullptr) {
#pragma unroll
        for (int q = 0; q < Cfg::UNITS * Cfg::UNIT_BOXES; ++q) tma_prefetch_l2_4d(&maps.r, colbase + q * Cfg::F32_CH, rw0, rh0, n0);
      }
      if constexpr (SLAB) {
        const uint32_t slab_bytes = static_cast<uint32_t>(p.TW * (p.TH + 2)) * 128u;
        uint32_t u = 0, a = 0;
        int base = 0;
#pragma unroll 1
        for (int sg = 0; sg < 3; ++sg) {
          const int chunks = p.seg_chunks[sg];
          const int nx = p.seg_taps[sg] == 9 ? 3 : 1;
          const bool e4m3 = A8 && sg == 0;
#pragma unroll 1
          for (int ch = 0; ch < chunks; ++ch) {
#pragma unroll 1
            for (int xi = 0; xi < nx; ++xi, ++a) {
              const int sl = static_cast<int>(a % SLAB_STAGES);
              if (a >= SLAB_STAGES) mbar_wait(&slab_empty[sl], ((a / SLAB_STAGES) - 1) & 1);
              mbar_arrive_expect_tx(&slab_full[sl], nx == 3 ? slab_bytes : static_cast<uint32_t>(Cfg::A_BYTES));
              tma_load_4d(&maps.a[sg], &slab_full[sl], slab_ring + sl * Cfg::SLAB_BYTES, ch * (e4m3 ? 128 : 64),
                          w0 + (nx == 3 ? xi - 1 : 0), h0 - (nx == 3 ? 1 : 0), n0);
#pragma unroll 1
              for (int yi = 0; yi < nx; ++yi, ++u) {
                const int s = static_cast<int>(u % STAGES);
                if (u >= STAGES) mbar_wait(&empty_bar[s], ((u / STAGES) - 1) & 1);
                mbar_arrive_expect_tx(&full_bar[s], BN * Cfg::BK * 2);
                const int t = nx == 3 ? 3 * yi + xi : 0;
                uint8_t* sb = w_ring + s * Cfg::B_BYTES;
                if constexpr (A8) {
                  if (e4m3) { tma_load_2d(&maps.b8, &full_bar[s], sb, (t * chunks + ch) * 128, colbase); continue; }
                }
                tma_load_2d(&maps.b, &full_bar[s], sb, base + (t * chunks + ch) * 64, colbase);
              }
            }
          }
          if (!e4m3) base += p.seg_taps[sg] * chunks * 64;
        }
      } else {
        ConvKCursor c;
        while (p.seg_chunks[c.seg] == 0) ++c.seg;
#pragma unroll 1
        for (int u = 0; u < nunits; ++u) {
          const uint32_t g = static_cast<uint32_t>(u);
          const int s = static_cast<int>(g % STAGES);
          if (g >= STAGES) mbar_wait(&empty_bar[s], ((g / STAGES) - 1) & 1);
          const int taps = p.seg_taps[c.seg], chunks = p.seg_chunks[c.seg];
          uint8_t* sa = smem + s * Cfg::STAGE_BYTES;
          uint8_t* sb = sa + Cfg::A_BYTES;
          const int dy = (taps == 9) ? (c.t / 3 - 1) : 0;
          const int dx = (taps == 9) ? (c.t % 3 - 1) : 0;
          mbar_arrive_expect_tx(&full_bar[s], Cfg::A_BYTES + BN * Cfg::BK * 2);
          bool e4m3 = false;
          if constexpr (A8) {
            if (c.seg == 0) {
              tma_load_4d(&maps.a[0], &full_bar[s], sa, c.ch * 128, w0 + dx, h0 + dy, n0);
              tma_load_2d(&maps.b8, &full_bar[s], sb, (c.t * chunks + c.ch) * 128, colbase);
              e4m3 = true;
            }
          }
          if (!e4m3) {
            const int kcol = c.base + (c.t * chunks + c.ch) * 64;
            tma_load_4d(&maps.a[c.seg], &full_bar[s], sa, c.ch * 64, w0 + dx, h0 + dy, n0);
            tma_load_2d(&maps.b, &full_bar[s], sb, kcol, colbase);
          }
          if (++c.ch == chunks) {
            c.ch = 0;
            if (++c.t == taps) { c.t = 0; if (!A8 || c.seg != 0) c.base += taps * chunks * 64; ++c.seg; }
          }
          while (c.seg < 3 && p.seg_chunks[c.seg] == 0) ++c.seg;
        }
      }
      if (p.residual != nullptr) {
        const uint32_t bytes = static_cast<uint32_t>(Cfg::UNIT_BOXES * Cfg::F32_BOX) >> (p.res_up ? 2 : 0);
#pragma unroll 1
        for (int i = 0; i < Cfg::UNITS; ++i) {
          const uint32_t g = static_cast<uint32_t>(nunits + i);
          const int s = static_cast<int>(g % STAGES);
          const int q = SLAB ? s : i;
          if (g >= STAGES) mbar_wait(&empty_bar[s], ((g / STAGES) - 1) & 1);
          mbar_arrive_expect_tx(&full_bar[s], bytes);
#pragma unroll
          for (int k = 0; k < Cfg::UNIT_BOXES; ++k)
            tma_load_4d(&maps.r, &full_bar[s], unit_ring + s * Cfg::UNIT_STRIDE + k * Cfg::F32_BOX,
                        colbase + q * Cfg::UNIT_CH + k * Cfg::F32_CH, rw0, rh0, n0);
        }
      }
    }
    return;
  }

  float acc[BN / 2];
#pragma unroll
  for (int i = 0; i < BN / 2; ++i) acc[i] = 0.f;

  if constexpr (SLAB) {
    const uint32_t row_bytes = static_cast<uint32_t>(p.TW) * 128u;
    uint32_t u = 0, a = 0;
#pragma unroll 1
    for (int sg = 0; sg < 3; ++sg) {
      const int nx = p.seg_taps[sg] == 9 ? 3 : 1;
      const int loads = p.seg_chunks[sg] * nx;
#pragma unroll 1
      for (int l = 0; l < loads; ++l, ++a) {
        const uint32_t sl = a % SLAB_STAGES;
        mbar_wait(&slab_full[sl], (a / SLAB_STAGES) & 1);
        const uint32_t sa = smem_u32(slab_ring + sl * Cfg::SLAB_BYTES) + wg * 64 * 128;
#pragma unroll 1
        for (int yi = 0; yi < nx; ++yi, ++u) {
          const uint32_t s = u % STAGES;
          mbar_wait(&full_bar[s], (u / STAGES) & 1);
          wgmma_fence();
          const uint64_t da = make_smem_desc_sw128(sa + yi * row_bytes, 1024, 16);
          const uint64_t db = make_smem_desc_sw128(smem_u32(w_ring + s * Cfg::B_BYTES), 1024, 16);
          if (A8 && sg == 0) {
#pragma unroll
            for (int k = 0; k < 4; ++k) wgmma_ss_e4m3<BN>(acc, da + 2 * k, db + 2 * k, (u | k) != 0 ? 1u : 0u);
          } else {
#pragma unroll
            for (int k = 0; k < 4; ++k) wgmma_ss<BN>(acc, da + 2 * k, db + 2 * k, (u | k) != 0 ? 1u : 0u);
          }
          wgmma_commit();
          wgmma_wait<1>();
          if (u > 0 && lane == 0) {
            mbar_arrive(&empty_bar[(u - 1) % STAGES]);
            if (yi == 0) mbar_arrive(&slab_empty[(a - 1) % SLAB_STAGES]);
          }
        }
      }
    }
    wgmma_wait<0>();
    reg_fence(acc);
    if (lane == 0) {
      mbar_arrive(&empty_bar[(u - 1) % STAGES]);
      mbar_arrive(&slab_empty[(a - 1) % SLAB_STAGES]);
    }
  } else {
#pragma unroll 1
    for (int u = 0; u < nunits; ++u) {
      const uint32_t g = static_cast<uint32_t>(u);
      const int s = static_cast<int>(g % STAGES);
      mbar_wait(&full_bar[s], (g / STAGES) & 1);
      const uint32_t sa = smem_u32(smem + s * Cfg::STAGE_BYTES);
      const uint32_t sb = sa + Cfg::A_BYTES;
      wgmma_fence();
      const uint64_t da = make_smem_desc_sw128(sa + wg * 64 * 128, 1024, 16);
      const uint64_t db = make_smem_desc_sw128(sb, 1024, 16);
      if (A8 && u < nunits8) {
#pragma unroll
        for (int k = 0; k < 4; ++k) wgmma_ss_e4m3<BN>(acc, da + 2 * k, db + 2 * k, (u | k) != 0 ? 1u : 0u);
      } else {
#pragma unroll
        for (int k = 0; k < 4; ++k) wgmma_ss<BN>(acc, da + 2 * k, db + 2 * k, (u | k) != 0 ? 1u : 0u);
      }
      wgmma_commit();
      wgmma_wait<1>();
      if (u > 0 && lane == 0) mbar_arrive(&empty_bar[(g - 1) % STAGES]);
    }
    wgmma_wait<0>();
    reg_fence(acc);
    if (lane == 0) mbar_arrive(&empty_bar[static_cast<uint32_t>(nunits - 1) % STAGES]);
  }

  const int wr = warp & 3;
  const int quad = lane & 3;
  constexpr int RB32 = Cfg::F32_CH * 4, RB16 = Cfg::F16_CH * 2;
  const uint32_t s_res = static_cast<uint32_t>(nunits) % STAGES;
  auto row_base = [](uint32_t r, int rb) {
    const uint32_t m = rb >= 128 ? 7u : rb == 64 ? 3u : rb == 32 ? 1u : 0u;
    return r * rb ^ ((((r * rb) >> 7) & m) << 4);
  };
  const uint32_t units_u32 = smem_u32(unit_ring);
  auto unit_at = [&](int u) { return units_u32 + (SLAB ? u : (s_res + u) % STAGES) * Cfg::UNIT_STRIDE; };
  auto f32_at = [&](int j, uint32_t t) {
    if constexpr (Cfg::F32_CH >= 8) {
      const int cl = 8 * j;
      return unit_at(cl / Cfg::UNIT_CH) + (cl % Cfg::UNIT_CH) / Cfg::F32_CH * Cfg::F32_BOX + (t ^ (cl % Cfg::F32_CH) * 4);
    } else {
      return unit_at(2 * j + (quad >> 1)) + t;
    }
  };
  const int rows_per_n = p.TW * p.TH;
  bool ok[2];
#pragma unroll
  for (int i = 0; i < 2; ++i) ok[i] = n0 + (wg * 64 + wr * 16 + (lane >> 2) + 8 * i) / rows_per_n < p.N;

  if (p.residual != nullptr) {
#pragma unroll 1
    for (int q = 0; q < Cfg::UNITS; ++q) {
      const uint32_t g = static_cast<uint32_t>(nunits + q);
      mbar_wait(&full_bar[g % STAGES], (g / STAGES) & 1);
    }
  }
  {
    uint32_t tr[2];
#pragma unroll
    for (int i = 0; i < 2; ++i) {
      const int row = wg * 64 + wr * 16 + (lane >> 2) + 8 * i;
      const int nl = row / rows_per_n, hl = (row / p.TW) % p.TH, xl = row % p.TW;
      const uint32_t rr = p.res_up ? (nl * (p.TH >> 1) + (hl >> 1)) * (p.TW >> 1) + (xl >> 1) : row;
      tr[i] = row_base(rr, RB32) ^ ((8 * quad) % RB32);
    }
    const float* bias = p.bias + colbase + 2 * quad;
#pragma unroll
    for (int j = 0; j < BN / 8; ++j) {
      const float2 b = make_float2(__ldg(bias + 8 * j), __ldg(bias + 8 * j + 1));
#pragma unroll
      for (int i = 0; i < 2; ++i) {
        float v0, v1;
        if (A8) {
          v0 = fmaf(acc[4 * j + 2 * i], p.acc_scale, b.x); v1 = fmaf(acc[4 * j + 2 * i + 1], p.acc_scale, b.y);
        } else {
          v0 = acc[4 * j + 2 * i] + b.x; v1 = acc[4 * j + 2 * i + 1] + b.y;
        }
        if (p.residual != nullptr) {
          float r0, r1;
          asm volatile("ld.shared.v2.f32 {%0, %1}, [%2];\n" : "=f"(r0), "=f"(r1) : "r"(f32_at(j, tr[i])) : "memory");
          v0 += r0; v1 += r1;
        }
        acc[4 * j + 2 * i] = v0; acc[4 * j + 2 * i + 1] = v1;
      }
    }
  }

  if (p.out_mode == 2) {
    const uint32_t hw = static_cast<uint32_t>(p.H) * p.W;
#pragma unroll
    for (int i = 0; i < 2; ++i) {
      if (!ok[i]) continue;
      const int row = wg * 64 + wr * 16 + (lane >> 2) + 8 * i;
      const int nl = row / rows_per_n, hl = (row / p.TW) % p.TH, xl = row % p.TW;
      float* o = reinterpret_cast<float*>(p.out) + (static_cast<size_t>(n0 + nl) * p.Cout + colbase + 2 * quad) * hw +
                 static_cast<uint32_t>(h0 + hl) * p.W + (w0 + xl);
#pragma unroll
      for (int j = 0; j < BN / 8; ++j, o += 8 * static_cast<size_t>(hw)) {
        const int c = colbase + 8 * j + 2 * quad;
        if (c >= p.Cout) continue;
        o[0] = acc[4 * j + 2 * i];
        if (c + 1 < p.Cout) o[hw] = acc[4 * j + 2 * i + 1];
      }
    }
    return;
  }
  asm volatile("bar.sync 1, %0;\n" ::"n"(Cfg::CONSUMER_THREADS) : "memory");

  const uint32_t f16_u32 = SLAB ? smem_u32(slab_ring) : smem_u32(smem) + ((s_res + Cfg::UNITS) % STAGES) * Cfg::STAGE_BYTES;
  uint32_t t32[2], t16[2];
#pragma unroll
  for (int i = 0; i < 2; ++i) {
    const uint32_t row = wg * 64 + wr * 16 + (lane >> 2) + 8 * i;
    t32[i] = row_base(row, RB32) ^ ((8 * quad) % RB32);
    t16[i] = row_base(row, RB16) ^ (4 * quad);
  }
  const bool do_stats = p.stats != nullptr;
  const int c_left = p.Cout - (colbase + 2 * quad);
  const uint32_t st_u32 = smem_u32(stat_smem) + (warp * 2 * BN + 2 * quad) * 4;
#pragma unroll
  for (int j = 0; j < BN / 8; ++j) {
    float s0 = 0.f, s1 = 0.f, q0 = 0.f, q1 = 0.f;
#pragma unroll
    for (int i = 0; i < 2; ++i) {
      float v0 = acc[4 * j + 2 * i], v1 = acc[4 * j + 2 * i + 1];
      const uint32_t a16 = f16_u32 + (8 * j) / Cfg::F16_CH * Cfg::F16_BOX + (t16[i] ^ ((8 * j) % Cfg::F16_CH) * 2);
      if (p.out_mode == 0) {
        asm volatile("st.shared.v2.f32 [%0], {%1, %2};\n" ::"r"(f32_at(j, t32[i])), "f"(v0), "f"(v1) : "memory");
        if (p.out16 != nullptr) asm volatile("st.shared.b32 [%0], %1;\n" ::"r"(a16), "r"(pack_h2(v0, v1)) : "memory");
      } else {
        const __half2 hv = __floats2half2_rn(v0, v1);
        asm volatile("st.shared.b32 [%0], %1;\n" ::"r"(a16), "r"(*reinterpret_cast<const uint32_t*>(&hv)) : "memory");
        const float2 r = __half22float2(hv);
        v0 = r.x; v1 = r.y;
      }
      if (ok[i] && 8 * j < c_left) {
        s0 += v0; s1 += v1;
        q0 = fmaf(v0, v0, q0); q1 = fmaf(v1, v1, q1);
      }
    }
    if (do_stats) {
#pragma unroll
      for (int off = 4; off < 32; off <<= 1) {
        s0 += __shfl_xor_sync(0xffffffffu, s0, off);
        s1 += __shfl_xor_sync(0xffffffffu, s1, off);
        q0 += __shfl_xor_sync(0xffffffffu, q0, off);
        q1 += __shfl_xor_sync(0xffffffffu, q1, off);
      }
      if (lane < 4) {
        const uint32_t st = st_u32 + 32 * j;
        asm volatile("st.shared.v2.f32 [%0], {%1, %2};\n" ::"r"(st), "f"(s0), "f"(s1) : "memory");
        asm volatile("st.shared.v2.f32 [%0], {%1, %2};\n" ::"r"(st + 4 * BN), "f"(q0), "f"(q1) : "memory");
      }
    }
  }
  fence_proxy_async_smem();
  asm volatile("bar.sync 1, %0;\n" ::"n"(Cfg::CONSUMER_THREADS) : "memory");
  if (tid == 0) {
    if (p.out_mode == 0) {
#pragma unroll
      for (int q = 0; q < Cfg::UNITS * Cfg::UNIT_BOXES; ++q) {
        const int u = q / Cfg::UNIT_BOXES, k = q % Cfg::UNIT_BOXES;
        const int col = colbase + q * Cfg::F32_CH;
        if (col < p.Cout)
          tma_store_4d(&maps.o, unit_ring + (SLAB ? u : (s_res + u) % STAGES) * Cfg::UNIT_STRIDE + k * Cfg::F32_BOX, col, w0, h0, n0);
      }
    }
    if (p.out_mode == 1 || p.out16 != nullptr) {
#pragma unroll
      for (int q = 0; q < BN / Cfg::F16_CH; ++q) {
        const int col = colbase + q * Cfg::F16_CH;
        if (col < p.Cout) tma_store_4d(&maps.o16, (SLAB ? slab_ring : smem + ((s_res + Cfg::UNITS) % STAGES) * Cfg::STAGE_BYTES) + q * Cfg::F16_BOX, col, w0, h0, n0);
      }
    }
    tma_store_commit();
  }
  if (do_stats) {
    const int n_tile = (128 + rows_per_n - 1) / rows_per_n;
    for (int e = tid; e < n_tile * BN; e += Cfg::CONSUMER_THREADS) {
      const int sn = e / BN, c = e - sn * BN;
      const int n = n0 + sn, col = colbase + c;
      if (n >= p.N || col >= p.Cout) continue;
      float ssum = 0.f, qsum = 0.f;
      for (int w8 = 0; w8 < 8; ++w8) {
        if ((w8 * 16) / rows_per_n != sn) continue;
        ssum += stat_smem[w8 * 2 * BN + c];
        qsum += stat_smem[w8 * 2 * BN + BN + c];
      }
      double* st = p.stats + (static_cast<size_t>(n) * p.Cout + col) * 2;
      atomicAdd(st, static_cast<double>(ssum));
      atomicAdd(st + 1, static_cast<double>(qsum));
    }
  }
  if (tid == 0) tma_store_wait_read();
}

}
```

### ivid_b200/csrc/ops.cu

```cuda
#include "ops.h"

#include <algorithm>
#include <cmath>
#include <mutex>

#include "attention.cuh"
#include "attention_hd.cuh"
#include "conv_gemm.cuh"
#include "elementwise.cuh"
#include "embed.cuh"

namespace ivid {

struct ConvLaunch {
  ConvMaps8 maps;
  ConvGemmParams p;
  int BN;
  bool a8;
  bool slab;
  int grid;
};

int conv_pad_cout(int cout) {
  if (cout >= 64) return ((cout + 63) / 64) * 64;
  return ((cout + 15) / 16) * 16;
}
static int pow2_divisor(int v, int cap) {
  int t = 1;
  while (t * 2 <= cap && v % (t * 2) == 0) t *= 2;
  return t;
}
void conv_tile(int H, int W, int* TW, int* TH, int* TN) {
  IVID_REQUIRE(H > 0 && W > 0, "conv: spatial size must be positive");
  *TW = pow2_divisor(W, 16);
  *TH = pow2_divisor(H, 128 / *TW);
  *TN = 128 / (*TW * *TH);
}
bool conv_can_fuse_stats(int H, int W) {
  int TW, TH, TN;
  conv_tile(H, W, &TW, &TH, &TN);
  return TW * TH >= 32;
}
int conv_pick_bn(int cout_pad) {
  if (cout_pad % 128 == 0) return 128;
  if (cout_pad % 64 == 0) return 64;
  if (cout_pad % 16 == 0 && cout_pad <= 48) return 16;
  throw Error(kErrInvalidArgument, "conv: unsupported padded Cout " + std::to_string(cout_pad));
}

bool conv_can_res_up(int W, int cout) { return W >= 16 && W % 2 == 0 && cout % 8 == 0; }
bool conv_can_out16(int cout) { return cout % 8 == 0; }
int conv_pad_k(int c) { return ((c + 63) / 64) * 64; }
int conv_pad_k8(int c) { return ((c + 127) / 128) * 128; }
int conv_seg_cols(int taps, int c) { return taps * conv_pad_k(c); }

ConvPack conv_pack(const float* w, const float* b, int cout, int cin, int ksz, int pitch, const float* w2, const float* b2,
                   int cin2, int cin2a, bool e4m3) {
  ConvPack pk;
  const int taps = ksz * ksz;
  pk.cout_pad = conv_pad_cout(cout);
  float scale = 1.f;
  if (e4m3) {
    IVID_REQUIRE(pitch == conv_pad_k(cin), "internal: an e4m3 segment 0 is an ordinary 3x3 or 1x1 conv");
    float mx = 0.f;
    for (size_t i = 0; i < static_cast<size_t>(cout) * cin * taps; ++i) mx = std::max(mx, std::fabs(w[i]));
    const int e = fp8_weight_exponent(mx);
    const float kMinNormal16 = std::ldexp(1.0f, -14);
    if (cin % 16 != 0) pk.refused = "its input channels are not a multiple of 16";
    else if (e < -100 || e > 100) pk.refused = "its weight exponent is outside [-100, 100]";
    for (size_t i = 0; pk.refused == nullptr && i < static_cast<size_t>(cout) * cin2; ++i) {
      const float v = std::fabs(w2[i]), sv = v * std::ldexp(1.0f, e);
      if (sv > 65504.f) pk.refused = "its skip weights times 2^e overflow fp16";
      else if (v >= kMinNormal16 && sv < kMinNormal16) pk.refused = "its skip weights times 2^e become fp16 subnormals";
    }
    pk.e4m3 = pk.refused == nullptr;
    if (pk.e4m3) { pk.e = e; scale = std::ldexp(1.0f, e); }
  }
  const int s0 = cin2a > 0 ? cin2a : cin2, s1 = cin2 - s0;
  const int k0 = pk.e4m3 ? 0 : conv_seg_cols(1, taps * pitch);
  pk.K = k0 + conv_seg_cols(1, s0) + conv_seg_cols(1, s1);
  pk.w16.assign(static_cast<size_t>(pk.cout_pad) * pk.K, __float2half_rn(0.f));
  const int cp8 = conv_pad_k8(cin), K8 = pk.e4m3 ? taps * cp8 : 0;
  pk.w8.assign(static_cast<size_t>(pk.cout_pad) * K8, 0);
  for (int co = 0; co < cout; ++co) {
    __half* row = pk.w16.data() + static_cast<size_t>(co) * pk.K;
    for (int tap = 0; tap < taps; ++tap)
      for (int ci = 0; ci < cin; ++ci) {
        const float v = w[(static_cast<size_t>(co) * cin + ci) * taps + tap];
        if (pk.e4m3) pk.w8[static_cast<size_t>(co) * K8 + tap * cp8 + ci] = fp8_e4m3_from_float(v * scale);
        else row[tap * pitch + ci] = __float2half_rn(v);
      }
    for (int ci = 0; ci < cin2; ++ci)
      row[k0 + (ci < s0 ? ci : conv_pad_k(s0) + ci - s0)] = __float2half_rn(w2[static_cast<size_t>(co) * cin2 + ci] * scale);
  }
  pk.bias.assign(pk.cout_pad, 0.f);
  for (int i = 0; i < cout; ++i) {
    if (b != nullptr) pk.bias[i] = b[i];
    if (b2 != nullptr) pk.bias[i] += b2[i];
  }
  return pk;
}

template <int BN, bool SLAB>
static void epilogue_box_channels(int* f32_ch, int* f16_ch) {
  *f32_ch = ConvGemmCfg<BN, SLAB>::F32_CH;
  *f16_ch = ConvGemmCfg<BN, SLAB>::F16_CH;
}
static void epilogue_box_channels(int BN, bool slab, int* f32_ch, int* f16_ch) {
  switch (BN) {
    case 128: slab ? epilogue_box_channels<128, true>(f32_ch, f16_ch) : epilogue_box_channels<128, false>(f32_ch, f16_ch); break;
    case 64: slab ? epilogue_box_channels<64, true>(f32_ch, f16_ch) : epilogue_box_channels<64, false>(f32_ch, f16_ch); break;
    default: slab ? epilogue_box_channels<16, true>(f32_ch, f16_ch) : epilogue_box_channels<16, false>(f32_ch, f16_ch); break;
  }
}

ConvLaunch* conv_launch_create(const ConvDesc& d) {
  IVID_REQUIRE(d.C0 > 0 && d.C0 % 8 == 0, "conv: segment-0 channels must be a positive multiple of 8");
  IVID_REQUIRE(d.C1 % 8 == 0, "conv: segment-1 channels must be a multiple of 8");
  IVID_REQUIRE(d.taps0 == 9 || d.taps0 == 1, "conv: only 3x3 (pad 1) and 1x1 kernels are on this path");
  IVID_REQUIRE(d.taps1 == 9 || d.taps1 == 1, "conv: only 3x3 (pad 1) and 1x1 kernels are on this path");
  IVID_REQUIRE(d.C2 % 8 == 0 && (d.taps2 == 9 || d.taps2 == 1), "conv: segment 2 must be a multiple of 8 channels, 3x3 or 1x1");
  IVID_REQUIRE(d.N > 0 && static_cast<int64_t>(d.N) * d.H * d.W < (int64_t{1} << 31),
               "conv: N*H*W must be below 2^31 (32-bit pixel indices in the epilogue)");
  const bool a8 = d.weight8 != nullptr;
  IVID_REQUIRE(!a8 || d.C0 % 16 == 0, "conv: an e4m3 segment 0 needs a multiple of 16 channels (16-byte TMA rows)");
  auto* l = new ConvLaunch();
  l->a8 = a8;
  ConvGemmParams& p = l->p;
  p.N = d.N; p.H = d.H; p.W = d.W;
  conv_tile(d.H, d.W, &p.TW, &p.TH, &p.TN);
  p.tiles_w = d.W / p.TW;
  p.tiles_h = d.H / p.TH;
  p.tiles_n = (d.N + p.TN - 1) / p.TN;
  const bool any3x3 = d.taps0 == 9 || (d.C1 > 0 && d.taps1 == 9) || (d.C2 > 0 && d.taps2 == 9);
  l->slab = any3x3 && p.TN == 1 && p.TW >= 8;
  IVID_REQUIRE(!l->slab || p.TW * (p.TH + 2) * 128 <= (ConvGemmCfg<128, true>::SLAB_BYTES), "internal: conv slab larger than its slot");
  l->BN = conv_pick_bn(d.cout_pad);
  p.n_blocks = d.cout_pad / l->BN;
  p.seg_chunks[0] = a8 ? conv_pad_k8(d.C0) / 128 : conv_pad_k(d.C0) / 64; p.seg_taps[0] = d.taps0;
  p.acc_scale = d.acc_scale;
  p.seg_chunks[1] = conv_pad_k(d.C1) / 64; p.seg_taps[1] = d.C1 > 0 ? d.taps1 : 0;
  p.seg_chunks[2] = conv_pad_k(d.C2) / 64; p.seg_taps[2] = d.C2 > 0 ? d.taps2 : 0;
  p.Cout = d.cout; p.ldc = d.ldc; p.ldr = d.ldr; p.out_mode = d.out_mode;
  p.bias = d.bias; p.residual = d.residual; p.out = d.out;
  p.stats = (d.stats != nullptr && conv_can_fuse_stats(d.H, d.W) && d.out_mode != 2) ? d.stats : nullptr;
  IVID_REQUIRE(d.stats == nullptr || p.stats != nullptr, "conv: fused statistics need >= 32 pixels per sample per warp");
  IVID_REQUIRE(d.out_mode == 2 || (d.cout % 8 == 0 && d.ldc % 8 == 0), "conv: NHWC output needs Cout % 8 == 0");
  IVID_REQUIRE(d.residual == nullptr || (d.out_mode != 2 && d.ldr % 4 == 0 && d.ldr >= d.cout),
               "conv: residual needs an NHWC output and a row pitch of >= Cout, a multiple of 4 elements");
  p.res_up = 0;
  if (d.residual != nullptr && d.residual_up) {
    IVID_REQUIRE(conv_can_res_up(d.W, d.cout) && d.H % 2 == 0, "conv: upsampled residual needs an even W >= 16 and Cout % 8 == 0");
    p.res_up = 1;
  }
  auto aligned = [](const void* q) { return (reinterpret_cast<uintptr_t>(q) & 15u) == 0; };
  IVID_REQUIRE(d.out_mode == 2 || (aligned(d.out) && aligned(d.out16) && aligned(d.residual)),
               "conv: NHWC output, fp16 copy and residual must be 16-byte aligned");
  p.out16 = nullptr;
  if (d.out16 != nullptr) {
    IVID_REQUIRE(d.out_mode == 0 && conv_can_out16(d.cout), "conv: fp16 output copy needs an fp32 NHWC output and Cout % 8 == 0");
    p.out16 = static_cast<__half*>(d.out16);
  }
  const int Ktot = (a8 ? 0 : conv_seg_cols(d.taps0, d.C0)) + conv_seg_cols(d.taps1, d.C1) + conv_seg_cols(d.taps2, d.C2);
  ConvMaps8& M = l->maps;
  auto rows = [&](int taps) { return l->slab && taps == 9 ? p.TH + 2 : p.TH; };
  M.a[0] = a8 ? make_act_map(d.act0, d.N, d.H, d.W, d.C0, p.TW, rows(d.taps0), p.TN, CU_TENSOR_MAP_DATA_TYPE_UINT8)
              : make_act_map(d.act0, d.N, d.H, d.W, d.C0, p.TW, rows(d.taps0), p.TN);
  M.a[1] = d.C1 > 0 ? make_act_map(d.act1, d.N, d.H, d.W, d.C1, p.TW, rows(d.taps1), p.TN) : M.a[0];
  M.a[2] = d.C2 > 0 ? make_act_map(d.act2, d.N, d.H, d.W, d.C2, p.TW, rows(d.taps2), p.TN) : M.a[0];
  if (a8) {
    M.b8 = make_weight_map(d.weight8, d.cout_pad, d.taps0 * conv_pad_k8(d.C0), l->BN, CU_TENSOR_MAP_DATA_TYPE_UINT8);
    M.b = Ktot > 0 ? make_weight_map(d.weight, d.cout_pad, Ktot, l->BN) : M.b8;
  } else {
    M.b = make_weight_map(d.weight, d.cout_pad, Ktot, l->BN);
  }
  int f32_ch = 0, f16_ch = 0;
  epilogue_box_channels(l->BN, l->slab, &f32_ch, &f16_ch);
  const auto f32 = CU_TENSOR_MAP_DATA_TYPE_FLOAT32;
  M.r = M.o = M.o16 = M.a[0];
  if (d.residual != nullptr) {
    const int up = p.res_up ? 1 : 0;
    M.r = make_act_map(d.residual, d.N, d.H >> up, d.W >> up, d.cout, p.TW >> up, p.TH >> up, p.TN, f32, d.ldr, f32_ch);
  }
  if (d.out_mode == 0) M.o = make_act_map(d.out, d.N, d.H, d.W, d.cout, p.TW, p.TH, p.TN, f32, d.ldc, f32_ch);
  const void* o16 = d.out_mode == 1 ? d.out : d.out_mode == 0 ? d.out16 : nullptr;
  if (o16 != nullptr) M.o16 = make_act_map(o16, d.N, d.H, d.W, d.cout, p.TW, p.TH, p.TN, CU_TENSOR_MAP_DATA_TYPE_FLOAT16, d.ldc, f16_ch);
  l->grid = p.tiles_w * p.tiles_h * p.tiles_n * p.n_blocks;
  return l;
}
void conv_launch_destroy(ConvLaunch* l) { delete l; }
int conv_launch_bn(const ConvLaunch* l) { return l->BN; }
bool conv_launch_a8(const ConvLaunch* l) { return l->a8; }

template <int BN, bool A8, bool SLAB>
static void run_conv(const ConvLaunch* l, cudaStream_t s) {
  using Cfg = ConvGemmCfg<BN, SLAB>;
  static std::once_flag once;
  std::call_once(once, [] {
    IVID_CHECK_CUDA(cudaFuncSetAttribute(conv_gemm_kernel<BN, A8, SLAB>, cudaFuncAttributeMaxDynamicSharedMemorySize, Cfg::SMEM_BYTES));
  });
  if constexpr (A8) conv_gemm_kernel<BN, true, SLAB><<<l->grid, Cfg::THREADS, Cfg::SMEM_BYTES, s>>>(l->maps, l->p);
  else conv_gemm_kernel<BN, false, SLAB><<<l->grid, Cfg::THREADS, Cfg::SMEM_BYTES, s>>>(static_cast<const ConvMaps&>(l->maps), l->p);
  IVID_CHECK_CUDA(cudaGetLastError());
}
template <bool A8, bool SLAB>
static void run_conv_bn(const ConvLaunch* l, cudaStream_t s) {
  switch (l->BN) {
    case 128: run_conv<128, A8, SLAB>(l, s); break;
    case 64: run_conv<64, A8, SLAB>(l, s); break;
    default: run_conv<16, A8, SLAB>(l, s); break;
  }
}
void conv_launch_run_out(const ConvLaunch* l, void* out, cudaStream_t s) {
  IVID_REQUIRE(l->p.out_mode == 2, "internal: only an NCHW conv output is patched at run time (NHWC outputs are in tensor maps)");
  ConvLaunch tmp = *l;
  tmp.p.out = out;
  conv_launch_run(&tmp, s);
}
void conv_launch_run(const ConvLaunch* l, cudaStream_t s) {
  if (l->a8) {
    if (l->slab) run_conv_bn<true, true>(l, s);
    else run_conv_bn<true, false>(l, s);
  } else {
    if (l->slab) run_conv_bn<false, true>(l, s);
    else run_conv_bn<false, false>(l, s);
  }
}

static int ew_grid(size_t work_items, int block) {
  const size_t blocks = (work_items + block - 1) / block;
  const size_t cap = static_cast<size_t>(sm_count()) * 16;
  return static_cast<int>(std::max<size_t>(1, std::min(blocks, cap)));
}

struct AttnLaunch {
  CUtensorMap mapQ, mapKV;
  AttnParams p;
  AttnHdParams hp;
  int head_ch = 64;
  int nv = 0;
  bool qres = false;
  int smem = 0;
  int grid;
  int N = 0, T = 0, C = 0, row0 = 0;
  const __half* qkv = nullptr;
  __half* out = nullptr;
};

AttnLaunch* attn_launch_create(const void* qkv, int N, int T, int C, int head_ch, void* out, int row0) {
  if (head_ch <= 0 || head_ch % 64 != 0)
    throw Error(kErrNotImplemented, "attention: head width " + std::to_string(head_ch) + " is not a multiple of 64");
  IVID_REQUIRE(C % head_ch == 0, "attention: channels must be a multiple of the head width " + std::to_string(head_ch));
  IVID_REQUIRE(T >= 1, "attention: sequence length must be positive");
  if (row0 < 0) row0 = N;
  IVID_REQUIRE(row0 <= N, "attention: the perturbed-row start must lie in [0, N]");
  auto* l = new AttnLaunch();
  l->N = N; l->T = T; l->C = C; l->row0 = row0;
  l->qkv = static_cast<const __half*>(qkv);
  l->out = static_cast<__half*>(out);
  l->head_ch = head_ch;
  l->p.N = N; l->p.T = T; l->p.C = C; l->p.heads = C / 64;
  l->p.q_tiles = (T + 127) / 128;
  l->p.out = reinterpret_cast<__half*>(out);
  const uint64_t dims[3] = {static_cast<uint64_t>(3 * C), static_cast<uint64_t>(T), static_cast<uint64_t>(N)};
  const uint64_t str[2] = {static_cast<uint64_t>(3 * C) * 2, static_cast<uint64_t>(T) * 3 * C * 2};
  const uint32_t boxq[3] = {64, 128, 1};
  const uint32_t boxkv[3] = {64, AttnCfg::KV, 1};
  l->mapQ = make_tensor_map(CU_TENSOR_MAP_DATA_TYPE_FLOAT16, 3, const_cast<void*>(qkv), dims, str, boxq,
                            CU_TENSOR_MAP_SWIZZLE_128B);
  l->mapKV = make_tensor_map(CU_TENSOR_MAP_DATA_TYPE_FLOAT16, 3, const_cast<void*>(qkv), dims, str, boxkv,
                             CU_TENSOR_MAP_SWIZZLE_128B);
  l->grid = row0 * l->p.heads * l->p.q_tiles;
  if (head_ch == 64) return l;
  using Cfg = AttnHdCfg;
  const int k = head_ch / 64;
  const int slices = (k + 3) / 4;
  l->nv = (k + slices - 1) / slices;
  l->qres = k <= Cfg::RESIDENT_Q_MAX_CHUNKS;
  AttnHdParams& hp = l->hp;
  hp.N = N; hp.T = T; hp.C = C; hp.d = head_ch; hp.heads = C / head_ch; hp.chunks = k;
  hp.q_tiles = l->p.q_tiles;
  hp.slices = (k + l->nv - 1) / l->nv;
  hp.scale_log2 = static_cast<float>(1.4426950408889634 / std::sqrt(static_cast<double>(head_ch)));
  hp.out = l->p.out;
  const int q_bytes = l->qres ? k * Cfg::QCHUNK_BYTES : 0;
  const int fixed = q_bytes + 1024  + 1024 ;
  const int budget = l->nv == 2 ? Cfg::MAX_SMEM_2CTA : Cfg::MAX_SMEM;
  hp.stages = std::min(Cfg::MAX_STAGES, (budget - fixed) / Cfg::stage_bytes(l->qres));
  IVID_REQUIRE(hp.stages >= 4, "attention: shared-memory ring too shallow");
  l->smem = fixed + hp.stages * Cfg::stage_bytes(l->qres);
  l->grid = row0 * hp.heads * hp.q_tiles * hp.slices;
  return l;
}
void attn_launch_destroy(AttnLaunch* l) { delete l; }

template <int NV, bool QRES>
static void run_attn_hd(const AttnLaunch* l, cudaStream_t s) {
  static std::once_flag once;
  std::call_once(once, [] {
    IVID_CHECK_CUDA(cudaFuncSetAttribute(attention_hd_kernel<NV, QRES>, cudaFuncAttributeMaxDynamicSharedMemorySize, AttnHdCfg::MAX_SMEM));
  });
  attention_hd_kernel<NV, QRES><<<l->grid, AttnHdCfg::THREADS, l->smem, s>>>(l->mapQ, l->mapKV, l->hp);
  IVID_CHECK_CUDA(cudaGetLastError());
}

void attn_launch_run(const AttnLaunch* l, cudaStream_t s) {
  attn_launch_run_identity(l, s);
  attn_launch_run_softmax(l, s);
}
void attn_launch_run_identity(const AttnLaunch* l, cudaStream_t s) {
  if (l->row0 == l->N) return;
  const size_t rows = static_cast<size_t>(l->N - l->row0) * l->T;
  attention_identity_kernel<<<ew_grid(rows * (l->C / 8), 256), 256, 0, s>>>(l->qkv, l->out, static_cast<size_t>(l->row0) * l->T, rows,
                                                                         l->C, l->head_ch);
  IVID_CHECK_CUDA(cudaGetLastError());
}
void attn_launch_run_softmax(const AttnLaunch* l, cudaStream_t s) {
  if (l->row0 == 0) return;
  if (l->head_ch != 64) {
    switch (l->nv * 2 + (l->qres ? 1 : 0)) {
      case 5: run_attn_hd<2, true>(l, s); break;
      case 7: run_attn_hd<3, true>(l, s); break;
      case 9: run_attn_hd<4, true>(l, s); break;
      case 6: run_attn_hd<3, false>(l, s); break;
      case 8: run_attn_hd<4, false>(l, s); break;
      default: throw Error(kErrState, "internal: attention slice width " + std::to_string(l->nv));
    }
    return;
  }
  static std::once_flag once;
  std::call_once(once, [] {
    IVID_CHECK_CUDA(cudaFuncSetAttribute(attention_kernel, cudaFuncAttributeMaxDynamicSharedMemorySize, AttnCfg::SMEM_BYTES));
  });
  attention_kernel<<<l->grid, AttnCfg::THREADS, AttnCfg::SMEM_BYTES, s>>>(l->mapQ, l->mapKV, l->p);
  IVID_CHECK_CUDA(cudaGetLastError());
}


void launch_gn_stats(const float* x, double* stats, int N, int HW, int C, cudaStream_t s) {
  IVID_REQUIRE(C % 4 == 0, "gn_stats: C % 4");
  dim3 grid((HW + kStatsPixPerBlock - 1) / kStatsPixPerBlock, N);
  gn_stats_kernel<<<grid, 256, 0, s>>>(x, stats, HW, C);
  IVID_CHECK_CUDA(cudaGetLastError());
}

void launch_gn_apply(const GnApplyDesc& d, cudaStream_t s) {
  IVID_REQUIRE(d.C0 % 8 == 0 && d.C1 % 8 == 0, "gn_apply: channel counts must be multiples of 8");
  const int C = d.C0 + d.C1;
  IVID_REQUIRE(d.groups >= 1 && d.groups <= 64 && C % d.groups == 0, "group norm: groups must divide channels (<= 64 groups)");
  IVID_REQUIRE(d.stats0 != nullptr && d.gamma != nullptr && d.beta != nullptr, "gn_apply: statistics / affine parameters missing");
  GnApplyParams p;
  p.x0 = static_cast<const float*>(d.x0); p.x1 = static_cast<const float*>(d.x1); p.C0 = d.C0; p.C1 = d.C1; p.N = d.N; p.H = d.H; p.W = d.W; p.mode = d.mode;
  p.x0h = d.x0_half ? reinterpret_cast<const __half*>(d.x0) : nullptr;
  p.x1h = d.x0_half ? reinterpret_cast<const __half*>(d.x1) : nullptr;
  p.silu = d.silu ? 1 : 0;
  p.stats0 = d.stats0; p.stats1 = d.stats1; p.groups = d.groups; p.inv_count = 1.0 / (static_cast<double>(d.H) * d.W);
  p.eps = d.eps; p.gamma = d.gamma; p.beta = d.beta; p.film = d.film; p.film_ld = d.film_ld; p.film_off = d.film_off;
  p.film_add = d.film_add ? 1 : 0;
  p.out_act = reinterpret_cast<__half*>(d.out_act); p.out_raw16 = reinterpret_cast<__half*>(d.out_raw16);
  p.out_act8 = d.out_e4m3 ? reinterpret_cast<uint8_t*>(d.out_act) : nullptr;
  p.out_raw32 = d.out_raw32;
  p.out_lo = reinterpret_cast<__half*>(d.out_lo);
  IVID_REQUIRE(d.out_lo == nullptr || (d.mode == 0 && d.x0_half && d.out_raw16 == nullptr && d.out_raw32 == nullptr),
               "gn_apply: the split (hi/lo) output exists on the same-resolution fp16-source path only");
  IVID_REQUIRE(!d.out_e4m3 || (d.out_lo == nullptr && C % 16 == 0), "gn_apply: an e4m3 output needs C % 16 == 0 and no split output");
  const int Ho = d.mode == 1 ? d.H * 2 : (d.mode == 2 ? d.H / 2 : d.H);
  const int Wo = d.mode == 1 ? d.W * 2 : (d.mode == 2 ? d.W / 2 : d.W);
  {
    const int blocks_per_n = std::max(1, (sm_count() * 3) / std::max(d.N, 1));
    const int by_wave = (Ho * Wo + blocks_per_n - 1) / blocks_per_n;
    const int small = std::max(1, 1024 / (C / 8));
    p.pix_per_block = std::max(1, std::min(Ho * Wo, std::max(by_wave, small)));
  }
  int pix_space = Ho * Wo;
  if (d.mode == 1) {
    pix_space = d.H * d.W;
    p.pix_per_block = std::max(1, (p.pix_per_block + 3) / 4);
  }
  dim3 grid((pix_space + p.pix_per_block - 1) / p.pix_per_block, d.N);
  const size_t smem = static_cast<size_t>(C) * 8;
  if (p.mode == 0 && p.x0h != nullptr && p.out_raw16 == nullptr && p.out_raw32 == nullptr) {
    const bool hoist = 256 % (C / 8) == 0;
    if (p.out_lo != nullptr) {
      if (hoist) gn_apply_h16_kernel<true, true><<<grid, 256, smem, s>>>(p);
      else gn_apply_h16_kernel<false, true><<<grid, 256, smem, s>>>(p);
    } else if (d.out_e4m3) {
      if (hoist) gn_apply_h16_kernel<true, false, true><<<grid, 256, smem, s>>>(p);
      else gn_apply_h16_kernel<false, false, true><<<grid, 256, smem, s>>>(p);
    } else if (hoist) gn_apply_h16_kernel<true><<<grid, 256, smem, s>>>(p);
    else gn_apply_h16_kernel<false><<<grid, 256, smem, s>>>(p);
  } else if (d.out_e4m3) {
    gn_apply_kernel<true><<<grid, 256, smem, s>>>(p);
  } else {
    gn_apply_kernel<><<<grid, 256, smem, s>>>(p);
  }
  IVID_CHECK_CUDA(cudaGetLastError());
}
void launch_im2col_s2(const void* x16, void* col, int N, int H, int W, int C, cudaStream_t s) {
  IVID_REQUIRE(C % 8 == 0 && H % 2 == 0 && W % 2 == 0, "im2col_s2: C % 8, even spatial size");
  const size_t items = static_cast<size_t>(N) * (H / 2) * (W / 2) * 9 * (C / 8);
  im2col_s2_h16_kernel<<<ew_grid(items, 256), 256, 0, s>>>(reinterpret_cast<const __half*>(x16), reinterpret_cast<__half*>(col), N, H, W, C);
  IVID_CHECK_CUDA(cudaGetLastError());
}
void launch_upsample2x_h16(const void* x16, void* out, int N, int H, int W, int C, cudaStream_t s) {
  IVID_REQUIRE(C % 8 == 0, "upsample2x: C % 8");
  const size_t items = static_cast<size_t>(N) * H * W * 4 * (C / 8);
  upsample2x_h16_kernel<<<ew_grid(items, 256), 256, 0, s>>>(reinterpret_cast<const __half*>(x16), reinterpret_cast<__half*>(out), N, H, W, C);
  IVID_CHECK_CUDA(cudaGetLastError());
}
void launch_resample_f32(const float* x, float* out, void* out16, int N, int H, int W, int C, int mode, cudaStream_t s) {
  IVID_REQUIRE(C % 4 == 0 && (mode == 1 || (H % 2 == 0 && W % 2 == 0)), "resample_f32: C % 4, even spatial size for pooling");
  const size_t items = static_cast<size_t>(N) * (mode == 1 ? 4 * H * W : (H / 2) * (W / 2)) * (C / 4);
  resample_f32_kernel<<<ew_grid(items, 256), 256, 0, s>>>(x, out, reinterpret_cast<__half*>(out16), N, H, W, C, mode);
  IVID_CHECK_CUDA(cudaGetLastError());
}
void launch_pack_input(const float* x, void* out, int N, int Nx, int Cin, int HW, cudaStream_t s) {
  IVID_REQUIRE(Cin >= 1 && Cin <= 16, "pack_input: 1..16 input channels (two-term split inside 64 operand channels)");
  pack_input_kernel<<<ew_grid(static_cast<size_t>(N) * HW, 256), 256, 0, s>>>(x, reinterpret_cast<__half*>(out), N, Nx,
                                                                                 Cin, HW);
  IVID_CHECK_CUDA(cudaGetLastError());
}

void launch_eps_gather(const float* Y, const float* bias, float* eps, int N, int H, int W, int Co, int ldy, cudaStream_t s) {
  IVID_REQUIRE(Co >= 1 && Co <= 7 && 9 * Co <= ldy, "eps_gather: 9*Co tap columns must fit the row pitch");
  IVID_REQUIRE(Co != 4 || ldy % 4 == 0, "eps_gather: row pitch must keep float4 alignment");
  eps_gather_kernel<<<ew_grid(static_cast<size_t>(N) * H * W, 256), 256, 0, s>>>(Y, bias, eps, N, H, W, Co, ldy);
  IVID_CHECK_CUDA(cudaGetLastError());
}

void launch_posenc(const int64_t* t, int Nt, const float* freqs, int half, float* out, int N, cudaStream_t s) {
  posenc_kernel<<<N, 128, 0, s>>>(t, Nt, freqs, half, out, N);
  IVID_CHECK_CUDA(cudaGetLastError());
}

void launch_film_table(const float* emb, const float* Wp, const float* bias, float* x_t, float* out, int N, int K, int O, cudaStream_t s) {
  IVID_REQUIRE(K % 32 == 0 && O % 4 == 0, "film table: K % 32 == 0");
  static std::once_flag once;
  std::call_once(once, [] {
    IVID_CHECK_CUDA(cudaFuncSetAttribute(film_table_kernel, cudaFuncAttributeMaxDynamicSharedMemorySize, FilmCfg::SMEM_BYTES));
  });
  const int nblk = (N + 31) / 32;
  silu_transpose_kernel<<<std::min(256, (nblk * K * 32 + 255) / 256), 256, 0, s>>>(emb, x_t, N, K, 1);
  const int tiles = (O + FilmCfg::TO - 1) / FilmCfg::TO;
  dim3 grid(std::min(tiles, std::max(1, sm_count() / nblk)), nblk);
  film_table_kernel<<<grid, FilmCfg::THREADS, FilmCfg::SMEM_BYTES, s>>>(Wp, x_t, bias, out, N, K, O);
  IVID_CHECK_CUDA(cudaGetLastError());
}

void launch_linear(const float* in, const float* W, const float* bias, float* out, int N, int K, int O, int silu_in,
                   const float* label_emb, const int64_t* classes, int Ncls, cudaStream_t s) {
  if ((K == 256 || K == 512 || K == 1024) && O <= 8192) {
    dim3 grid((O + 7) / 8, (N + 31) / 32);
    const size_t smem = static_cast<size_t>(32) * K * 4;
    static std::once_flag once;
    std::call_once(once, [] {
      IVID_CHECK_CUDA(cudaFuncSetAttribute(linear_warp_kernel<2>, cudaFuncAttributeMaxDynamicSharedMemorySize, 32 * 256 * 4));
      IVID_CHECK_CUDA(cudaFuncSetAttribute(linear_warp_kernel<4>, cudaFuncAttributeMaxDynamicSharedMemorySize, 32 * 512 * 4));
      IVID_CHECK_CUDA(cudaFuncSetAttribute(linear_warp_kernel<8>, cudaFuncAttributeMaxDynamicSharedMemorySize, 32 * 1024 * 4));
    });
    auto go = [&](auto kern) { kern<<<grid, 256, smem, s>>>(in, W, bias, out, N, O, silu_in, label_emb, classes, Ncls); };
    if (K == 256) go(linear_warp_kernel<2>); else if (K == 512) go(linear_warp_kernel<4>); else go(linear_warp_kernel<8>);
    IVID_CHECK_CUDA(cudaGetLastError());
    return;
  }
  if (K % 32 == 0) {
    if (O >= 128 * 64) {
      dim3 grid((O + 127) / 128, (N + 31) / 32);
      linear_tiled_kernel<4><<<grid, 256, 0, s>>>(in, W, bias, out, N, K, O, silu_in, label_emb, classes, Ncls);
    } else {
      dim3 grid((O + 63) / 64, (N + 31) / 32);
      linear_tiled_kernel<2><<<grid, 256, 0, s>>>(in, W, bias, out, N, K, O, silu_in, label_emb, classes, Ncls);
    }
    IVID_CHECK_CUDA(cudaGetLastError());
    return;
  }
  dim3 grid((O + 63) / 64, (N + 31) / 32);
  linear_rows_kernel<<<grid, 256, 0, s>>>(in, W, bias, out, N, K, O, silu_in, label_emb, classes, Ncls);
  IVID_CHECK_CUDA(cudaGetLastError());
}

}
```

### ivid_b200/csrc/ops.h

```cpp
#pragma once
#include <cuda.h>
#include <cuda_fp16.h>
#include <cuda_runtime.h>
#include <stdint.h>

#include <vector>

#include "host_util.h"

namespace ivid {

struct ConvLaunch;
struct AttnLaunch;

struct ConvDesc {
  const void* act0 = nullptr; int C0 = 0; int taps0 = 9;
  const void* act1 = nullptr; int C1 = 0; int taps1 = 1;
  const void* act2 = nullptr; int C2 = 0; int taps2 = 1;
  void* out16 = nullptr;
  const void* weight = nullptr;
  const void* weight8 = nullptr;
  float acc_scale = 1.f;
  int cout_pad = 0;
  int cout = 0;
  const float* bias = nullptr;
  const float* residual = nullptr; int ldr = 0;
  bool residual_up = false;
  void* out = nullptr; int ldc = 0; int out_mode = 0;
  double* stats = nullptr;
  int N = 0, H = 0, W = 0;
};

ConvLaunch* conv_launch_create(const ConvDesc& d);
void conv_launch_destroy(ConvLaunch* l);
void conv_launch_run(const ConvLaunch* l, cudaStream_t s);
int conv_launch_bn(const ConvLaunch* l);
bool conv_launch_a8(const ConvLaunch* l);
void conv_launch_run_out(const ConvLaunch* l, void* out, cudaStream_t s);
int conv_pick_bn(int cout_pad);
bool conv_can_out16(int cout);
bool conv_can_res_up(int W, int cout);
void conv_tile(int H, int W, int* TW, int* TH, int* TN);
bool conv_can_fuse_stats(int H, int W);
int conv_pad_cout(int cout);
int conv_pad_k(int c);
int conv_pad_k8(int c);
int conv_seg_cols(int taps, int c);

struct ConvPack {
  std::vector<__half> w16;
  std::vector<uint8_t> w8;
  std::vector<float> bias;
  int cout_pad = 0, K = 0;
  bool e4m3 = false;
  int e = 0;
  const char* refused = nullptr;
};
ConvPack conv_pack(const float* w, const float* b, int cout, int cin, int ksz, int pitch, const float* w2, const float* b2,
                   int cin2, int cin2a, bool e4m3);

AttnLaunch* attn_launch_create(const void* qkv, int N, int T, int C, int head_ch, void* out, int row0 = -1);
void attn_launch_destroy(AttnLaunch* l);
void attn_launch_run(const AttnLaunch* l, cudaStream_t s);
void attn_launch_run_softmax(const AttnLaunch* l, cudaStream_t s);
void attn_launch_run_identity(const AttnLaunch* l, cudaStream_t s);

void launch_gn_stats(const float* x, double* stats, int N, int HW, int C, cudaStream_t s);
struct GnApplyDesc {
  const void* x0 = nullptr; const void* x1 = nullptr; int C0 = 0, C1 = 0;
  bool x0_half = false;
  int N = 0, H = 0, W = 0; int mode = 0; int silu = 1;
  const double* stats0 = nullptr; const double* stats1 = nullptr;
  int groups = 32; float eps = 1e-5f;
  const float* gamma = nullptr; const float* beta = nullptr;
  const float* film = nullptr; int film_ld = 0, film_off = 0;
  bool film_add = false;
  void* out_act = nullptr; void* out_raw16 = nullptr; float* out_raw32 = nullptr;
  void* out_lo = nullptr;
  bool out_e4m3 = false;
};
void launch_gn_apply(const GnApplyDesc& d, cudaStream_t s);
void launch_eps_gather(const float* Y, const float* bias, float* eps, int N, int H, int W, int Co, int ldy, cudaStream_t s);
void launch_im2col_s2(const void* x16, void* col, int N, int H, int W, int C, cudaStream_t s);
void launch_upsample2x_h16(const void* x16, void* out, int N, int H, int W, int C, cudaStream_t s);
void launch_resample_f32(const float* x, float* out, void* out16, int N, int H, int W, int C, int mode, cudaStream_t s);
void launch_pack_input(const float* x, void* out, int N, int Nx, int Cin, int HW, cudaStream_t s);

struct CondPackDesc {
  const float* x = nullptr; const float* y = nullptr; const float* mask = nullptr; const float* mask_rgb = nullptr;
  const float* noise = nullptr; void* out = nullptr; int N = 0, Nx = 0, H = 0, W = 0; int kind = 0;
  int scale = 2;
  uint64_t seed = 0; uint32_t stream = 0; const int* stream_dev = nullptr;
};
void launch_cond_pack(const CondPackDesc& d, cudaStream_t s);
void launch_cfg_mix(const float* eps2, float* out, size_t count, float strength, cudaStream_t s);
void launch_guidance_mix(const float* eps, float* out, size_t count, int cfg, float strength, int pag, float pag_scale,
                         cudaStream_t s);
void launch_dynamic_threshold(const float* x, int N, int M, double ratio, double threshold_max, float* s_out, float* x_out,
                              cudaStream_t s);
void launch_apg(const float* dc, const float* du, float* state, int N, int M, float s, double eta, double norm, double beta,
                float* out, cudaStream_t st);

void launch_posenc(const int64_t* t, int Nt, const float* freqs, int half, float* out, int N, cudaStream_t s);
void launch_film_table(const float* emb, const float* Wp, const float* bias, float* x_t, float* out, int N, int K, int O, cudaStream_t s);
void launch_linear(const float* in, const float* W, const float* bias, float* out, int N, int K, int O, int silu_in,
                   const float* label_emb, const int64_t* classes, int Ncls, cudaStream_t s);

}
```

### ivid_b200/csrc/unet.cu

```cuda
#include "unet.h"

#include <algorithm>
#include <cmath>
#include <cstring>

#include "json_min.h"

namespace ivid {

static UnetConfig parse_config(const std::string& text) {
  JsonValue j;
  try {
    j = JsonParser(text).parse();
  } catch (const std::exception& e) {
    throw Error(kErrInvalidArgument, e.what());
  }
  IVID_REQUIRE(j.kind == JsonValue::kObject, "backbone config must be a JSON object");
  if (j.has("backbone") && j.at("backbone").kind == JsonValue::kObject) j = JsonValue(j.at("backbone"));
  if (j.has("args") && j.at("args").kind == JsonValue::kObject) j = JsonValue(j.at("args"));
  UnetConfig c;
  auto geti = [&](const char* k, int& dst, bool required) {
    if (j.has(k)) dst = static_cast<int>(j.at(k).num);
    else IVID_REQUIRE(!required, std::string("backbone config: missing '") + k + "'");
  };
  auto getb = [&](const char* k, bool& dst) { if (j.has(k)) dst = j.at(k).kind == JsonValue::kBool ? j.at(k).b : j.at(k).num != 0; };
  geti("image_size", c.image_size, true);
  geti("in_channels", c.in_channels, true);
  geti("model_channels", c.model_channels, true);
  geti("out_channels", c.out_channels, true);
  geti("num_res_blocks", c.num_res_blocks, true);
  IVID_REQUIRE(j.has("attention_resolutions"), "backbone config: missing 'attention_resolutions'");
  for (auto& v : j.at("attention_resolutions").arr) c.attention_resolutions.push_back(static_cast<int>(v.num));
  if (j.has("channel_mult")) {
    c.channel_mult.clear();
    for (auto& v : j.at("channel_mult").arr) c.channel_mult.push_back(v.num);
  }
  if (j.has("dropout")) c.dropout = j.at("dropout").num;
  getb("conv_resample", c.conv_resample);
  geti("num_classes", c.num_classes, false);
  getb("has_null_class", c.has_null_class);
  if (c.num_classes == 0) c.has_null_class = false;
  getb("use_fp16", c.use_fp16);
  geti("num_groups", c.num_groups, false);
  geti("num_heads", c.num_heads, false);
  geti("num_head_channels", c.num_head_channels, false);
  getb("use_scale_shift_norm", c.use_scale_shift_norm);
  getb("resblock_updown", c.resblock_updown);
  return c;
}

Unet::Unet(const std::string& cfg_json) : cfg_(parse_config(cfg_json)) { build_topology(); }

int Unet::add_param(const std::string& name, std::vector<int64_t> shape, bool is_buffer) {
  ParamSpec p;
  p.name = name;
  p.shape = std::move(shape);
  p.is_buffer = is_buffer;
  pindex_[name] = static_cast<int>(params_.size());
  params_.push_back(std::move(p));
  return static_cast<int>(params_.size()) - 1;
}

const ParamSpec& Unet::P(const std::string& name) const {
  auto it = pindex_.find(name);
  if (it == pindex_.end()) throw Error(kErrState, "internal: unknown parameter " + name);
  const ParamSpec& p = params_[it->second];
  if (!p.set) throw Error(kErrState, "parameter '" + name + "' was never set (load_state_dict incomplete)");
  return p;
}

void Unet::build_topology() {
  const UnetConfig& c = cfg_;
  IVID_REQUIRE(c.in_channels <= 16, "in_channels must be <= 16");
  IVID_REQUIRE(c.num_groups >= 1 && c.num_groups <= 64, "num_groups must be in [1,64]");
  const int mc = c.model_channels;
  const int E = mc * 4;
  embed_dim_ = E;

  add_param("time_embed.0.freqs", {mc / 2}, true);
  add_param("time_embed.1.weight", {E, mc});
  add_param("time_embed.1.bias", {E});
  add_param("time_embed.3.weight", {E, E});
  add_param("time_embed.3.bias", {E});
  if (c.num_classes > 0) add_param("label_emb.weight", {c.num_classes, E});

  auto head_width = [&](int ch) {
    int hc;
    if (c.num_head_channels != -1) {
      IVID_REQUIRE(c.num_head_channels > 0 && ch % c.num_head_channels == 0,
                   "q,k,v channels " + std::to_string(ch) + " is not divisible by num_head_channels " + std::to_string(c.num_head_channels));
      hc = c.num_head_channels;
    } else {
      IVID_REQUIRE(c.num_heads > 0 && ch % c.num_heads == 0,
                   "attention channels " + std::to_string(ch) + " are not divisible by num_heads " + std::to_string(c.num_heads));
      hc = ch / c.num_heads;
    }
    if (hc % 64 != 0)
      throw Error(kErrNotImplemented, "attention head width " + std::to_string(hc) + " is not a multiple of 64 channels");
    return hc;
  };
  std::vector<int> widths;
  auto add_res = [&](const std::string& pfx, int cin, int cout, int mode, int cat0 = 0) {
    ResBlockDef r;
    r.pfx = pfx; r.cin = cin; r.cout = cout; r.mode = mode; r.cat0 = cat0;
    IVID_REQUIRE(cin % c.num_groups == 0 && cout % c.num_groups == 0, "num_groups must divide channels");
    widths.insert(widths.end(), {cin, cout, cat0});
    add_param(pfx + ".in_layers.0.weight", {cin});
    add_param(pfx + ".in_layers.0.bias", {cin});
    add_param(pfx + ".in_layers.2.weight", {cout, cin, 3, 3});
    add_param(pfx + ".in_layers.2.bias", {cout});
    const int ew = c.use_scale_shift_norm ? 2 * cout : cout;
    add_param(pfx + ".emb_layers.1.weight", {ew, E});
    add_param(pfx + ".emb_layers.1.bias", {ew});
    add_param(pfx + ".out_layers.0.weight", {cout});
    add_param(pfx + ".out_layers.0.bias", {cout});
    add_param(pfx + ".out_layers.3.weight", {cout, cout, 3, 3});
    add_param(pfx + ".out_layers.3.bias", {cout});
    r.skip_conv = (cin != cout);
    if (r.skip_conv) {
      add_param(pfx + ".skip_connection.weight", {cout, cin, 1, 1});
      add_param(pfx + ".skip_connection.bias", {cout});
    }
    r.film_off = film_total_;
    film_total_ += ew;
    res_.push_back(r);
    return static_cast<int>(res_.size()) - 1;
  };
  auto add_attn = [&](const std::string& pfx, int ch) {
    AttnBlockDef a;
    a.pfx = pfx; a.C = ch; a.head_ch = head_width(ch);
    add_param(pfx + ".norm.weight", {ch});
    add_param(pfx + ".norm.bias", {ch});
    add_param(pfx + ".qkv.weight", {3 * ch, ch, 1});
    add_param(pfx + ".qkv.bias", {3 * ch});
    add_param(pfx + ".proj_out.weight", {ch, ch, 1});
    add_param(pfx + ".proj_out.bias", {ch});
    attn_.push_back(a);
    return static_cast<int>(attn_.size()) - 1;
  };
  auto add_resample = [&](const std::string& pfx, int ch, int mode) {
    ResampleDef r;
    r.pfx = pfx; r.C = ch; r.mode = mode; r.conv = c.conv_resample;
    widths.push_back(ch);
    if (r.conv) {
      const std::string sub = mode == 2 ? ".op" : ".conv";
      add_param(pfx + sub + ".weight", {ch, ch, 3, 3});
      add_param(pfx + sub + ".bias", {ch});
    }
    resample_.push_back(r);
    return static_cast<int>(resample_.size()) - 1;
  };
  auto in_attn = [&](int ds) {
    return std::find(c.attention_resolutions.begin(), c.attention_resolutions.end(), ds) != c.attention_resolutions.end();
  };

  int ch = static_cast<int>(c.channel_mult[0] * mc);
  const int input_ch = ch;
  in_ch_stem_ = ch;
  add_param("input_blocks.0.0.weight", {ch, c.in_channels, 3, 3});
  add_param("input_blocks.0.0.bias", {ch});
  {
    BlockDef b;
    b.is_input = true;
    blocks_.push_back(b);
  }
  int ds = c.image_size;
  std::vector<int> input_block_chs{ch};
  int ib = 1;
  const int levels = static_cast<int>(c.channel_mult.size());
  for (int level = 0; level < levels; ++level) {
    const int outc = static_cast<int>(c.channel_mult[level] * mc);
    for (int r = 0; r < c.num_res_blocks; ++r) {
      BlockDef b;
      b.is_input = true;
      const std::string pfx = "input_blocks." + std::to_string(ib);
      b.layers.push_back({LayerKind::kResBlock, add_res(pfx + ".0", ch, outc, 0)});
      ch = outc;
      if (in_attn(ds)) b.layers.push_back({LayerKind::kAttention, add_attn(pfx + ".1", ch)});
      blocks_.push_back(b);
      input_block_chs.push_back(ch);
      ++ib;
    }
    if (level != levels - 1) {
      BlockDef b;
      b.is_input = true;
      if (c.resblock_updown) b.layers.push_back({LayerKind::kResBlock, add_res("input_blocks." + std::to_string(ib) + ".0", ch, ch, 2)});
      else b.layers.push_back({LayerKind::kResample, add_resample("input_blocks." + std::to_string(ib) + ".0", ch, 2)});
      blocks_.push_back(b);
      input_block_chs.push_back(ch);
      ++ib;
      ds /= 2;
    }
  }
  {
    BlockDef b;
    b.layers.push_back({LayerKind::kResBlock, add_res("middle_block.0", ch, ch, 0)});
    b.layers.push_back({LayerKind::kAttention, add_attn("middle_block.1", ch)});
    b.layers.push_back({LayerKind::kResBlock, add_res("middle_block.2", ch, ch, 0)});
    blocks_.push_back(b);
  }
  int ob = 0;
  for (int level = levels - 1; level >= 0; --level) {
    const int outc = static_cast<int>(mc * c.channel_mult[level]);
    for (int i = 0; i <= c.num_res_blocks; ++i) {
      BlockDef b;
      b.is_output = true;
      const std::string pfx = "output_blocks." + std::to_string(ob);
      const int ich = input_block_chs.back();
      input_block_chs.pop_back();
      int li = 0;
      b.layers.push_back({LayerKind::kResBlock, add_res(pfx + "." + std::to_string(li++), ch + ich, outc, 0, ch)});
      ch = outc;
      if (in_attn(ds)) b.layers.push_back({LayerKind::kAttention, add_attn(pfx + "." + std::to_string(li++), ch)});
      if (level != 0 && i == c.num_res_blocks) {
        if (c.resblock_updown) b.layers.push_back({LayerKind::kResBlock, add_res(pfx + "." + std::to_string(li++), ch, ch, 1)});
        else b.layers.push_back({LayerKind::kResample, add_resample(pfx + "." + std::to_string(li++), ch, 1)});
        ds *= 2;
      }
      blocks_.push_back(b);
      ++ob;
    }
  }
  final_ch_ = ch;
  IVID_REQUIRE(ch == input_ch, "final channel count must equal the stem width (adm.py:486 uses input_ch)");
  for (int w : widths)
    if (w % 8 != 0)
      throw Error(kErrNotImplemented, "channel width " + std::to_string(w) + " is not a multiple of 8 (16-byte NHWC fp16 rows)");
  add_param("out.0.weight", {ch});
  add_param("out.0.bias", {ch});
  add_param("out.2.weight", {c.out_channels, input_ch, 3, 3});
  add_param("out.2.bias", {c.out_channels});
}

void Unet::set_param(const std::string& name, const float* data, const int64_t* shape, int ndim) {
  auto it = pindex_.find(name);
  if (it == pindex_.end()) throw Error(kErrInvalidArgument, "unexpected key in state_dict: " + name);
  ParamSpec& p = params_[it->second];
  bool same = static_cast<int>(p.shape.size()) == ndim;
  for (int i = 0; same && i < ndim; ++i) same = p.shape[i] == shape[i];
  if (!same) throw Error(kErrInvalidArgument, "size mismatch for " + name);
  p.host.assign(data, data + p.numel());
  p.set = true;
}

namespace {
struct ArenaBuilder {
  std::vector<uint8_t> buf;
  size_t alloc(size_t bytes) {
    const size_t off = (buf.size() + 255) & ~size_t(255);
    buf.resize(off + bytes, 0);
    return off;
  }
  template <class T> T* at(size_t off) { return reinterpret_cast<T*>(buf.data() + off); }
};

void pack_stem_rows(__half* dst, int Ktot, const float* w, int cout, int cin, int cin_pad) {
  for (int co = 0; co < cout; ++co)
    for (int tap = 0; tap < 9; ++tap)
      for (int ci = 0; ci < cin; ++ci) {
        const float v = w[(static_cast<size_t>(co) * cin + ci) * 9 + tap];
        const __half hi = __float2half_rn(v);
        const __half lo = __float2half_rn(v - __half2float(hi));
        __half* row = dst + static_cast<size_t>(co) * Ktot + tap * cin_pad;
        row[ci] = hi; row[cin + ci] = hi; row[2 * cin + ci] = lo;
      }
}

void pack_out_rows(__half* dst, int C, int Cp, const float* w, int co_n) {
  const int K = 3 * Cp;
  for (int tap = 0; tap < 9; ++tap)
    for (int c = 0; c < co_n; ++c)
      for (int ci = 0; ci < C; ++ci) {
        const float v = w[(static_cast<size_t>(c) * C + ci) * 9 + tap];
        const __half hi = __float2half_rn(v);
        const __half lo = __float2half_rn(v - __half2float(hi));
        __half* row = dst + static_cast<size_t>(tap * co_n + c) * K;
        row[ci] = hi; row[Cp + ci] = hi; row[2 * Cp + ci] = lo;
      }
}
}

void Unet::set_precision(int precision) {
  IVID_REQUIRE(precision == 0 || precision == 1, "precision must be 0 (fp16) or 1 (fp8 ResBlock convs)");
  precision_ = precision;
}

void Unet::finalize(int device) {
  IVID_CHECK_CUDA(cudaSetDevice(device));
  for (const auto& p : params_)
    if (!p.set) throw Error(kErrState, "parameter '" + p.name + "' was never set (load_state_dict incomplete)");
  plans_.clear();
  if (arena_) { cudaFree(arena_); arena_ = nullptr; }
  device_ = device;
  ArenaBuilder ab;
  auto put_f32 = [&](const std::vector<float>& v, size_t pad_to = 0) {
    const size_t n = std::max(v.size(), pad_to);
    const size_t off = ab.alloc(n * 4);
    std::memcpy(ab.at<float>(off), v.data(), v.size() * 4);
    return off;
  };
  auto pack_gn = [&](const std::string& pfx, int C) {
    GnW g; g.C = C;
    g.g_off = put_f32(P(pfx + ".weight").host);
    g.b_off = put_f32(P(pfx + ".bias").host);
    return g;
  };
  auto put_conv = [&](const std::string& wname, const std::string& bname, int cout, int cin, int pitch, int ksz,
                       const std::string& skip_w = "", const std::string& skip_b = "", int cin2 = 0, int cin2a = 0,
                       bool e4m3 = false) {
    const ConvPack pk = conv_pack(P(wname).host.data(), P(bname).host.data(), cout, cin, ksz, pitch,
                                  cin2 > 0 ? P(skip_w).host.data() : nullptr, cin2 > 0 ? P(skip_b).host.data() : nullptr,
                                  cin2, cin2a, e4m3);
    ConvW cw;
    cw.cout = cout; cw.cout_pad = pk.cout_pad; cw.K = pk.K; cw.fp8 = pk.e4m3; cw.e8 = pk.e;
    if (pk.e4m3) {
      cw.w8_off = ab.alloc(pk.w8.size());
      std::memcpy(ab.at<uint8_t>(cw.w8_off), pk.w8.data(), pk.w8.size());
    }
    if (pk.K > 0) {
      cw.w_off = ab.alloc(pk.w16.size() * 2);
      std::memcpy(ab.at<__half>(cw.w_off), pk.w16.data(), pk.w16.size() * 2);
    }
    cw.b_off = put_f32(pk.bias);
    return cw;
  };
  auto pack_lin = [&](const std::string& pfx) {
    const ParamSpec& w = P(pfx + ".weight");
    LinW l; l.O = static_cast<int>(w.shape[0]); l.K = static_cast<int>(w.shape[1]);
    l.w_off = put_f32(w.host);
    l.b_off = put_f32(P(pfx + ".bias").host);
    return l;
  };

  freqs_off_ = put_f32(P("time_embed.0.freqs").host);
  te1_ = pack_lin("time_embed.1");
  te2_ = pack_lin("time_embed.3");
  if (cfg_.num_classes > 0) label_off_ = put_f32(P("label_emb.weight").host);
  {
    film_.O = film_total_; film_.K = embed_dim_;
    film_.w_off = ab.alloc(static_cast<size_t>(film_total_) * embed_dim_ * 4);
    film_.b_off = ab.alloc(static_cast<size_t>(film_total_) * 4);
    for (const auto& r : res_) {
      const auto& w = P(r.pfx + ".emb_layers.1.weight").host;
      const auto& b = P(r.pfx + ".emb_layers.1.bias").host;
      if (embed_dim_ % 32 == 0) {
        float* dst = ab.at<float>(film_.w_off);
        const int rows_w = static_cast<int>(w.size() / embed_dim_);
        for (int o = 0; o < rows_w; ++o)
          for (int kc = 0; kc < embed_dim_; kc += 32)
            for (int g = 0; g < 8; ++g)
              std::memcpy(dst + (static_cast<size_t>(kc / 32) * film_total_ + r.film_off + o) * 32 + ((g ^ ((r.film_off + o) & 7)) << 2),
                          w.data() + static_cast<size_t>(o) * embed_dim_ + kc + g * 4, 16);
      } else {
        std::memcpy(ab.at<float>(film_.w_off) + static_cast<size_t>(r.film_off) * embed_dim_, w.data(), w.size() * 4);
      }
      std::memcpy(ab.at<float>(film_.b_off) + r.film_off, b.data(), b.size() * 4);
    }
  }
  in_conv_ = put_conv("input_blocks.0.0.weight", "input_blocks.0.0.bias", in_ch_stem_, cfg_.in_channels, 64, 3);
  IVID_REQUIRE(3 * cfg_.in_channels <= 64, "in_channels must be <= 21 (two-term input split inside 64 operand channels)");
  pack_stem_rows(ab.at<__half>(in_conv_.w_off), in_conv_.K, P("input_blocks.0.0.weight").host.data(), in_ch_stem_, cfg_.in_channels, 64);
  for (auto& r : resample_)
    if (r.conv) {
      const std::string sub = r.mode == 2 ? ".op" : ".conv";
      r.w = put_conv(r.pfx + sub + ".weight", r.pfx + sub + ".bias", r.C, r.C, r.mode == 2 ? r.C : conv_pad_k(r.C), 3);
    }
  for (auto& r : res_) {
    r.gn1 = pack_gn(r.pfx + ".in_layers.0", r.cin);
    r.conv1 = put_conv(r.pfx + ".in_layers.2.weight", r.pfx + ".in_layers.2.bias", r.cout, r.cin, conv_pad_k(r.cin), 3,
                       "", "", 0, 0, precision_ == 1);
    r.gn2 = pack_gn(r.pfx + ".out_layers.0", r.cout);
    r.conv2 = put_conv(r.pfx + ".out_layers.3.weight", r.pfx + ".out_layers.3.bias", r.cout, r.cout, conv_pad_k(r.cout), 3,
                       r.pfx + ".skip_connection.weight", r.pfx + ".skip_connection.bias", r.skip_conv ? r.cin : 0, r.cat0,
                       precision_ == 1);
  }
  for (auto& a : attn_) {
    a.gn = pack_gn(a.pfx + ".norm", a.C);
    a.qkv = put_conv(a.pfx + ".qkv.weight", a.pfx + ".qkv.bias", 3 * a.C, a.C, conv_pad_k(a.C), 1);
    a.proj = put_conv(a.pfx + ".proj_out.weight", a.pfx + ".proj_out.bias", a.C, a.C, conv_pad_k(a.C), 1);
  }
  out_gn_ = pack_gn("out.0", final_ch_);
  out_conv_ = put_conv("out.2.weight", "out.2.bias", cfg_.out_channels, final_ch_, conv_pad_k(final_ch_), 3);
  out_split_ = 9 * cfg_.out_channels <= 64 && getenv("IVID_NO_OUTSPLIT") == nullptr;
  if (out_split_) {
    out1x1_.cout = 64; out1x1_.cout_pad = 64; out1x1_.K = 3 * conv_pad_k(final_ch_);
    out1x1_.w_off = ab.alloc(static_cast<size_t>(64) * out1x1_.K * 2);
    pack_out_rows(ab.at<__half>(out1x1_.w_off), final_ch_, conv_pad_k(final_ch_), P("out.2.weight").host.data(), cfg_.out_channels);
    out1x1_.b_off = put_f32(std::vector<float>(64, 0.f));
  }

  arena_bytes_ = (ab.buf.size() + 255) & ~size_t(255);
  IVID_CHECK_CUDA(cudaMalloc(&arena_, arena_bytes_));
  IVID_CHECK_CUDA(cudaMemcpy(arena_, ab.buf.data(), ab.buf.size(), cudaMemcpyHostToDevice));
}

Unet::~Unet() {
  plans_.clear();
  if (cap_stream_) cudaStreamDestroy(cap_stream_);
  if (arena_) cudaFree(arena_);
}

struct Plan {
  int N = 0;
  int H = 0, W = 0;
  AttnPerturb pert;
  uint64_t last_use = 0;
  uint8_t* ws = nullptr;
  size_t ws_bytes = 0;
  double* stats_base = nullptr;
  size_t stats_bytes = 0;
  struct OpRec {
    const char* label;
    double flops;
    double bytes;
    std::string note;
    std::function<void(cudaStream_t)> fn;
    int block;
  };
  std::vector<OpRec> ops;
  int op_block = -1;
  void add_op(const char* label, double flops, double bytes, std::string note, std::function<void(cudaStream_t)> fn) {
    ops.push_back(OpRec{label, flops, bytes, std::move(note), std::move(fn), op_block});
  }
  int n_blocks = 0;
  std::vector<size_t> block_stats;
  bool cache_valid = false;
  bool kept(int block, int branch) const {
    return branch < 0 || block < 0 || block <= branch || block >= n_blocks - 1 - branch;
  }
  void run(cudaStream_t s, cudaEvent_t* ev = nullptr, int branch = -1) const {
    if (branch < 0) {
      IVID_CHECK_CUDA(cudaMemsetAsync(stats_base, 0, stats_bytes, s));
    } else {
      uint8_t* base = reinterpret_cast<uint8_t*>(stats_base);
      const size_t head = block_stats[branch + 1], tail = block_stats[n_blocks - 1 - branch];
      IVID_CHECK_CUDA(cudaMemsetAsync(base, 0, head, s));
      if (tail < stats_bytes) IVID_CHECK_CUDA(cudaMemsetAsync(base + tail, 0, stats_bytes - tail, s));
    }
    if (ev) IVID_CHECK_CUDA(cudaEventRecord(ev[0], s));
    for (size_t i = 0; i < ops.size(); ++i) {
      if (kept(ops[i].block, branch)) ops[i].fn(s);
      if (ev) IVID_CHECK_CUDA(cudaEventRecord(ev[i + 1], s));
    }
  }
  std::vector<ConvLaunch*> convs;
  std::vector<AttnLaunch*> attns;
  const float* x = nullptr; int Nx = 0; ivid_cond_t cond{}; const int64_t* t = nullptr; const int64_t* classes = nullptr;
  float* eps = nullptr;
  const HeadHook* hook = nullptr;
  const int* cond_stream_dev = nullptr;
  struct GraphKey {
    const void* x; int Nx; const void* t; const void* classes; void* eps;
    int kind; const void* y; const void* mask; const void* mask_rgb; const void* noise; uint64_t seed; uint32_t stream_id;
    const void* stream_dev;
    uint64_t hook_key;
    int sr_scale;
    int cache_branch;
    bool operator==(const GraphKey& o) const {
      return hook_key == o.hook_key && sr_scale == o.sr_scale && cache_branch == o.cache_branch && x == o.x && Nx == o.Nx && t == o.t && classes == o.classes && eps == o.eps && kind == o.kind && y == o.y && mask == o.mask &&
             mask_rgb == o.mask_rgb && noise == o.noise && seed == o.seed && stream_id == o.stream_id && stream_dev == o.stream_dev;
    }
  };
  struct GraphEntry { GraphKey key; cudaGraphExec_t exec; uint64_t last_use; };
  struct Tap { std::string name; const float* d32; const __half* d16; int C, H, W; };
  std::vector<Tap> taps;
  std::vector<GraphEntry> graphs;
  uint64_t runs = 0;
  uint64_t graph_hits = 0, graph_captures = 0;
  ~Plan() {
    for (auto& g : graphs) cudaGraphExecDestroy(g.exec);
    for (auto* c : convs) conv_launch_destroy(c);
    for (auto* a : attns) attn_launch_destroy(a);
    if (ws) cudaFree(ws);
  }
};

namespace {
enum Slot { kIn, kA1, kA2, kXh, kXr, kH, kQkv, kCol, kPe, kE1, kEmb, kFilm, kXt, kSlots };
struct Act {
  float* data = nullptr;
  __half* d16 = nullptr;
  double* stats = nullptr;
  bool has16 = false;
  int id = -1;
  int C = 0, H = 0, W = 0;
};
struct BlockOut {
  int C, H, W;
  bool may16;
  bool need32 = false;
  bool only16 = false;
  size_t off16 = 0, off32 = 0;
};
}

void Unet::check_geometry(int H, int W) const {
  const int levels = static_cast<int>(cfg_.channel_mult.size());
  const int m = 1 << (levels - 1);
  if (H <= 0 || W <= 0 || H % m != 0 || W % m != 0)
    throw Error(kErrState, "input size " + std::to_string(H) + "x" + std::to_string(W) + " is not a multiple of " + std::to_string(m) +
                               " (2^(levels-1)): the skip connections' sizes would not match after " + std::to_string(levels - 1) + " downsamplings");
}

Plan* Unet::get_plan(int N, int H, int W, const AttnPerturb& pert) {
  Plan* found = nullptr;
  for (auto& p : plans_)
    if (p->N == N && p->H == H && p->W == W && p->pert.row0 == pert.row0 && p->pert.layers == pert.layers) found = p.get();
  if (found == nullptr) {
    check_geometry(H, W);
    if (plans_.size() >= 4) {
      IVID_CHECK_CUDA(cudaDeviceSynchronize());
      plans_.erase(plans_.begin());
    }
    plans_.emplace_back(build_plan(N, H, W, pert));
    found = plans_.back().get();
  }
  found->last_use = ++plan_uses_;
  return found;
}

Plan* Unet::build_plan(int N, int SH, int SW, const AttnPerturb& pert) {
  std::unique_ptr<Plan> plan(new Plan());
  plan->N = N;
  plan->pert = pert;
  std::vector<bool> perturbed(attn_.size(), false);
  for (int i : pert.layers) perturbed[i] = true;
  plan->H = SH; plan->W = SW;
  plan->n_blocks = static_cast<int>(blocks_.size());
  plan->block_stats.assign(blocks_.size(), 0);
  Plan* pl = plan.get();
  const int G = cfg_.num_groups;
  const float eps = 1e-5f;
  auto W8 = [&](size_t off) { return arena_ + off; };
  auto Wf = [&](size_t off) { return reinterpret_cast<const float*>(arena_ + off); };
  auto bind = [&](ConvDesc& d, const ConvW& w) {
    d.weight = w.K > 0 ? W8(w.w_off) : nullptr;
    d.weight8 = w.fp8 ? W8(w.w8_off) : nullptr;
    d.acc_scale = std::ldexp(1.0f, -w.e8);
    d.cout_pad = w.cout_pad; d.cout = w.cout; d.bias = Wf(w.b_off);
  };

  size_t slot_bytes[kSlots] = {}, slot_off[kSlots] = {};
  std::vector<BlockOut> outs;
  size_t stats_bytes = 0, stats_off = 0;
  auto walk = [&](uint8_t* base) {
    const bool create = base != nullptr;
    auto scratch = [&](Slot s, size_t bytes) -> void* {
      if (!create) { slot_bytes[s] = std::max(slot_bytes[s], bytes); return nullptr; }
      IVID_REQUIRE(bytes <= slot_bytes[s], "internal: scratch request exceeds its slot");
      return base + slot_off[s];
    };
    auto s16 = [&](Slot s, int H, int Wd, int C) { return scratch(s, static_cast<size_t>(N) * H * Wd * C * 2); };
    auto s32 = [&](Slot s, int H, int Wd, int C) { return static_cast<float*>(scratch(s, static_cast<size_t>(N) * H * Wd * C * 4)); };
    auto sop = [&](Slot s, int H, int Wd, int C, bool e4m3) { return scratch(s, static_cast<size_t>(N) * H * Wd * C * (e4m3 ? 1 : 2)); };
    size_t soff = 0;
    auto take_stats = [&](int C) -> double* {
      const size_t o = soff;
      soff += (static_cast<size_t>(N) * C * 16 + 255) & ~size_t(255);
      if (!create) return nullptr;
      IVID_REQUIRE(soff <= stats_bytes, "internal: statistics request exceeds the arena");
      return reinterpret_cast<double*>(base + stats_off + o);
    };
    int next_id = 0;
    auto new_act = [&](int C, int H, int Wd, bool may16) {
      Act a; a.C = C; a.H = H; a.W = Wd;
      a.id = next_id++;
      a.has16 = conv_can_out16(C);
      if (!create) {
        outs.push_back(BlockOut{C, H, Wd, may16 && a.has16 && conv_can_fuse_stats(H, Wd)});
      } else {
        IVID_REQUIRE(a.id < static_cast<int>(outs.size()) && outs[a.id].C == C && outs[a.id].H == H && outs[a.id].W == Wd,
                     "internal: block output differs from the sizing pass");
        const BlockOut& o = outs[a.id];
        if (a.has16) a.d16 = reinterpret_cast<__half*>(base + o.off16);
        if (!o.only16) a.data = reinterpret_cast<float*>(base + o.off32);
      }
      a.stats = take_stats(C);
      return a;
    };
    auto use32 = [&](const Act& a) -> const float* {
      if (!create) outs[a.id].need32 = true;
      else IVID_REQUIRE(a.data != nullptr, "internal: fp32 tensor was not materialised");
      return a.data;
    };
    auto keep32 = [&](const Act& a) { use32(a); };
    auto write_to = [&](ConvDesc& d, const Act& a) {
      if (a.data != nullptr) { d.out = a.data; d.out16 = a.d16; d.out_mode = 0; }
      else { d.out = a.d16; d.out_mode = 1; }
      d.ldc = a.C; d.N = N; d.H = a.H; d.W = a.W;
    };
    auto add_conv = [&](ConvDesc d, const Act* stats_of = nullptr, double k_alg = 0.0, double n_alg = 0.0) {
      if (!create) return;
      const bool fused = stats_of != nullptr && conv_can_fuse_stats(d.H, d.W);
      if (fused) d.stats = stats_of->stats;
      ConvLaunch* l = conv_launch_create(d);
      pl->convs.push_back(l);
      const double K = k_alg > 0.0 ? k_alg : static_cast<double>(d.taps0) * d.C0 + (d.C1 > 0 ? static_cast<double>(d.taps1) * d.C1 : 0.0) +
                       (d.C2 > 0 ? static_cast<double>(d.taps2) * d.C2 : 0.0);
      const double M = static_cast<double>(d.N) * d.H * d.W;
      const double Nalg = n_alg > 0.0 ? n_alg : static_cast<double>(d.cout);
      static const char* names[2][3] = {{"conv_gemm<16>", "conv_gemm<64>", "conv_gemm<128>"},
                                        {"conv_gemm<16,e4m3>", "conv_gemm<64,e4m3>", "conv_gemm<128,e4m3>"}};
      const int bn = conv_launch_bn(l);
      const bool a8 = conv_launch_a8(l);
      const double K0 = static_cast<double>(d.taps0) * d.C0;
      pl->add_op(names[a8 ? 1 : 0][bn == 128 ? 2 : bn == 64 ? 1 : 0], 2.0 * M * K * Nalg,
                 M * (d.C0 * (a8 ? 1 : 2) + (d.C1 + d.C2) * 2) + M * d.cout * ((d.out_mode == 1 ? 2 : 4) + (d.out16 ? 2 : 0) + (d.residual ? 4 : 0)) +
                     (a8 ? K0 + 2 * (K - K0) : 2 * K) * d.cout_pad,
                 std::to_string(d.H) + "x" + std::to_string(d.W) + " " + std::to_string(d.C0) + (d.C1 ? "+" + std::to_string(d.C1) : "") + (d.C2 ? "+" + std::to_string(d.C2) : "") +
                     "->" + std::to_string(d.cout) + " k" + std::to_string(d.taps0) + (d.residual ? " res" : "") + (d.stats ? " stats" : "") +
                     (d.out_mode == 1 ? " f16" : "") + (d.out16 ? " +f16" : ""),
                 [l](cudaStream_t s) { conv_launch_run(l, s); });
      if (stats_of != nullptr && !fused) {
        const float* x = stats_of->data; double* st = stats_of->stats;
        IVID_REQUIRE(x != nullptr, "internal: statistics pass over a tensor without fp32 storage");
        const int HW = stats_of->H * stats_of->W, C = stats_of->C;
        pl->add_op("gn_stats", 0, static_cast<double>(N) * HW * C * 4, "", [=](cudaStream_t s) { launch_gn_stats(x, st, N, HW, C, s); });
      }
    };

    pl->op_block = -1;
    float* s_pe = s32(kPe, 1, 1, cfg_.model_channels);
    float* s_e1 = s32(kE1, 1, 1, embed_dim_);
    float* s_emb = s32(kEmb, 1, 1, embed_dim_);
    float* s_film = s32(kFilm, 1, 1, film_total_);
    float* s_xt = static_cast<float*>(scratch(kXt, static_cast<size_t>((N + 31) / 32) * embed_dim_ * 32 * 4));
    if (create) {
      const float* freqs = Wf(freqs_off_);
      const int half = cfg_.model_channels / 2, mc = cfg_.model_channels, E = embed_dim_;
      const float *w1 = Wf(te1_.w_off), *b1 = Wf(te1_.b_off), *w2 = Wf(te2_.w_off), *b2 = Wf(te2_.b_off);
      const float* lab = cfg_.num_classes > 0 ? Wf(label_off_) : nullptr;
      const float *wf = Wf(film_.w_off), *bf = Wf(film_.b_off);
      const int FT = film_total_;
      pl->add_op("embed", 2.0 * N * E * (mc + E), 4.0 * E * (mc + E), "posenc+time_embed", [=](cudaStream_t s) {
        launch_posenc(pl->t, N, freqs, half, s_pe, N, s);
        launch_linear(s_pe, w1, b1, s_e1, N, mc, E, 0, nullptr, nullptr, 1, s);
        launch_linear(s_e1, w2, b2, s_emb, N, E, E, 1, pl->classes ? lab : nullptr, pl->classes, N, s);
      });
      pl->taps.push_back({"emb", s_emb, nullptr, E, 1, 1});
      pl->taps.push_back({"film", s_film, nullptr, FT, 1, 1});
      pl->add_op("embed", 2.0 * N * E * FT, 4.0 * E * FT, "film table O=" + std::to_string(FT), [=](cudaStream_t s) {
        if (E % 32 == 0) launch_film_table(s_emb, wf, bf, s_xt, s_film, N, E, FT, s);
        else launch_linear(s_emb, wf, bf, s_film, N, E, FT, 1, nullptr, nullptr, 1, s);
      });
    }
    auto add_gn = [&](GnApplyDesc d, const Act& a0, const Act* a1, const GnW& g, int film_off) {
      if (!create) return;
      d.stats0 = a0.stats; d.stats1 = a1 ? a1->stats : nullptr;
      d.groups = G; d.eps = eps;
      d.gamma = Wf(g.g_off); d.beta = Wf(g.b_off);
      d.film = film_off >= 0 ? s_film : nullptr;
      d.film_ld = film_total_; d.film_off = std::max(film_off, 0);
      d.film_add = film_off >= 0 && !cfg_.use_scale_shift_norm;
      const int Ho = d.mode == 1 ? d.H * 2 : (d.mode == 2 ? d.H / 2 : d.H);
      const int Wo = d.mode == 1 ? d.W * 2 : (d.mode == 2 ? d.W / 2 : d.W);
      const double in_el = static_cast<double>(d.N) * d.H * d.W * (d.C0 + d.C1);
      const double out_el = static_cast<double>(d.N) * Ho * Wo * (d.C0 + d.C1);
      pl->add_op("gn_apply", 0, in_el * (d.x0_half ? 2 : 4) + out_el * (d.out_e4m3 ? 1 : 2) + (d.out_raw16 ? out_el * 2 : 0) + (d.out_raw32 ? out_el * 4 : 0),
                 std::to_string(d.H) + "x" + std::to_string(d.W) + " C" + std::to_string(d.C0) + (d.C1 ? "+" + std::to_string(d.C1) : "") +
                     " m" + std::to_string(d.mode) + (d.x0_half ? " h16" : "") + (d.out_raw16 ? " raw16" : "") + (d.out_raw32 ? " raw32" : "") +
                     (d.out_e4m3 ? " e4m3" : ""),
                 [d](cudaStream_t s) { launch_gn_apply(d, s); });
    };

    void* s_in = s16(kIn, SH, SW, 64);
    if (create) {
      const int Cin = cfg_.in_channels, HW = SH * SW;
      pl->add_op("pack_input", 0, static_cast<double>(N) * HW * (Cin * 4 + 128), "", [=](cudaStream_t s) {
        if (pl->cond.kind == 0) {
          launch_pack_input(pl->x, s_in, N, pl->Nx, Cin, HW, s);
        } else {
          CondPackDesc cp;
          cp.x = pl->x; cp.y = pl->cond.y_dev; cp.mask = pl->cond.mask_dev; cp.mask_rgb = pl->cond.mask_rgb_dev;
          cp.noise = pl->cond.noise_dev; cp.out = s_in; cp.N = N; cp.Nx = pl->Nx; cp.H = SH; cp.W = SW;
          cp.kind = pl->cond.kind; cp.seed = pl->cond.seed; cp.stream = pl->cond.stream_id; cp.stream_dev = pl->cond_stream_dev;
          cp.scale = pl->cond.sr_scale > 0 ? pl->cond.sr_scale : 2;
          launch_cond_pack(cp, s);
        }
      });
    }
    pl->op_block = 0;
    Act cur = new_act(in_ch_stem_, SH, SW, true);
    {
      ConvDesc d;
      d.act0 = s_in; d.C0 = 64; d.taps0 = 9;
      bind(d, in_conv_);
      write_to(d, cur);
      add_conv(d, &cur, 9.0 * cfg_.in_channels);
      if (create) pl->taps.push_back({"input_blocks.0.0", cur.data, cur.d16, cur.C, cur.H, cur.W});
    }
    std::vector<Act> skips;
    skips.push_back(cur);

    auto run_res = [&](const ResBlockDef& r, const Act& x0, const Act* x1) -> Act {
      const int Cin = x0.C + (x1 ? x1->C : 0);
      IVID_REQUIRE(Cin == r.cin, "internal: ResBlock input width mismatch at " + r.pfx);
      keep32(x0);
      if (x1) keep32(*x1);
      const int H = x0.H, Wd = x0.W;
      const int Ho = r.mode == 1 ? H * 2 : (r.mode == 2 ? H / 2 : H);
      const int Wo = r.mode == 1 ? Wd * 2 : (r.mode == 2 ? Wd / 2 : Wd);
      const bool identity = !r.skip_conv;
      const bool res_up = identity && r.mode == 1 && x1 == nullptr && conv_can_res_up(Wo, r.cout);
      const bool need_xr = identity && (r.mode != 0 || x1 != nullptr) && !res_up;
      GnApplyDesc g1;
      const bool use16 = r.mode == 0 && !need_xr && x0.has16 && (x1 == nullptr || x1->has16);
      if (use16) { g1.x0 = x0.d16; g1.x1 = x1 ? x1->d16 : nullptr; g1.x0_half = true; }
      else { g1.x0 = use32(x0); g1.x1 = x1 ? use32(*x1) : nullptr; }
      g1.C0 = x0.C; g1.C1 = x1 ? x1->C : 0;
      g1.N = N; g1.H = H; g1.W = Wd; g1.mode = r.mode; g1.silu = 1;
      IVID_REQUIRE(!(r.skip_conv && r.mode != 0), "internal: up/down ResBlocks keep the channel count");
      void* a1 = sop(kA1, Ho, Wo, r.cin, r.conv1.fp8);
      void* xh = r.skip_conv && !use16 ? s16(kXh, H, Wd, r.cin) : nullptr;
      float* xr = need_xr ? s32(kXr, Ho, Wo, r.cin) : nullptr;
      g1.out_act = a1; g1.out_raw16 = xh; g1.out_raw32 = xr; g1.out_e4m3 = r.conv1.fp8;
      add_gn(g1, x0, x1, r.gn1, -1);
      const bool h_half = conv_can_fuse_stats(Ho, Wo);
      Act h; h.C = r.cout; h.H = Ho; h.W = Wo;
      h.data = static_cast<float*>(scratch(kH, static_cast<size_t>(N) * Ho * Wo * r.cout * (h_half ? 2 : 4)));
      h.stats = take_stats(r.cout);
      {
        ConvDesc d;
        d.act0 = a1; d.C0 = r.cin; d.taps0 = 9;
        bind(d, r.conv1);
        d.out = h.data; d.ldc = r.cout; d.out_mode = h_half ? 1 : 0; d.N = N; d.H = Ho; d.W = Wo;
        add_conv(d, &h);
      }
      void* a2 = sop(kA2, Ho, Wo, r.cout, r.conv2.fp8);
      GnApplyDesc g2;
      g2.x0 = h.data; g2.x0_half = h_half; g2.C0 = r.cout; g2.N = N; g2.H = Ho; g2.W = Wo; g2.mode = 0; g2.silu = 1;
      g2.out_act = a2; g2.out_e4m3 = r.conv2.fp8;
      add_gn(g2, h, nullptr, r.gn2, r.film_off);
      Act out = new_act(r.cout, Ho, Wo, !identity);
      {
        ConvDesc d;
        d.act0 = a2; d.C0 = r.cout; d.taps0 = 9;
        if (r.skip_conv && use16) {
          d.act1 = x0.d16; d.C1 = x0.C; d.taps1 = 1;
          if (x1 != nullptr) { d.act2 = x1->d16; d.C2 = x1->C; d.taps2 = 1; }
        } else if (r.skip_conv) {
          IVID_REQUIRE(r.cat0 % 64 == 0, "internal: raw-copy skip conv over a concat whose first part is not a multiple of 64");
          d.act1 = xh; d.C1 = r.cin; d.taps1 = 1;
        }
        bind(d, r.conv2);
        if (identity) { d.residual = need_xr ? xr : use32(x0); d.ldr = r.cout; d.residual_up = res_up; }
        write_to(d, out);
        add_conv(d, &out);
      }
      if (create) pl->taps.push_back({r.pfx, out.data, out.d16, out.C, out.H, out.W});
      return out;
    };
    auto run_attn = [&](const AttnBlockDef& a, int idx, const Act& x) -> Act {
      IVID_REQUIRE(x.C == a.C, "internal: attention width mismatch at " + a.pfx);
      const int T = x.H * x.W;
      void* a1 = s16(kA1, x.H, x.W, a.C);
      void* qkv = s16(kQkv, x.H, x.W, 3 * a.C);
      void* a2 = s16(kA2, x.H, x.W, a.C);
      GnApplyDesc g;
      if (x.has16) { g.x0 = x.d16; g.x0_half = true; } else g.x0 = use32(x);
      g.C0 = a.C; g.N = N; g.H = x.H; g.W = x.W; g.mode = 0; g.silu = 0; g.out_act = a1;
      add_gn(g, x, nullptr, a.gn, -1);
      {
        ConvDesc d;
        d.act0 = a1; d.C0 = a.C; d.taps0 = 1;
        bind(d, a.qkv);
        d.out = qkv; d.ldc = 3 * a.C; d.out_mode = 1; d.N = N; d.H = x.H; d.W = x.W;
        add_conv(d);
      }
      if (create) {
        const int row0 = perturbed[idx] ? pert.row0 : N;
        AttnLaunch* l = attn_launch_create(qkv, N, T, a.C, a.head_ch, a2, row0);
        pl->attns.push_back(l);
        const std::string shape = "T=" + std::to_string(T) + " heads=" + std::to_string(a.C / a.head_ch) + " d=" + std::to_string(a.head_ch);
        if (row0 > 0)
          pl->add_op("attention", 4.0 * row0 * static_cast<double>(T) * T * a.C, static_cast<double>(row0) * T * a.C * 8, shape,
                     [l](cudaStream_t s) { attn_launch_run_softmax(l, s); });
        if (row0 < N)
          pl->add_op("attention_identity", 0, static_cast<double>(N - row0) * T * a.C * 4, shape + " rows=" + std::to_string(N - row0),
                     [l](cudaStream_t s) { attn_launch_run_identity(l, s); });
      }
      Act out = new_act(a.C, x.H, x.W, false);
      {
        ConvDesc d;
        d.act0 = a2; d.C0 = a.C; d.taps0 = 1;
        bind(d, a.proj);
        d.residual = use32(x); d.ldr = a.C;
        write_to(d, out);
        add_conv(d, &out);
      }
      if (create) pl->taps.push_back({a.pfx, out.data, out.d16, out.C, out.H, out.W});
      return out;
    };

    auto run_resample = [&](const ResampleDef& r, const Act& x) -> Act {
      IVID_REQUIRE(x.C == r.C, "internal: resampling layer width mismatch at " + r.pfx);
      const int Ho = r.mode == 1 ? x.H * 2 : x.H / 2, Wo = r.mode == 1 ? x.W * 2 : x.W / 2;
      Act out = new_act(r.C, Ho, Wo, false);
      const int H = x.H, Wd = x.W, C = r.C;
      if (r.conv) {
        IVID_REQUIRE(x.has16, "internal: resampling conv needs the fp16 copy of its input");
        const void* x16 = x.d16;
        ConvDesc d;
        if (r.mode == 2) {
          void* col = s16(kCol, Ho, Wo, 9 * C);
          if (create)
            pl->add_op("resample", 0, static_cast<double>(N) * Ho * Wo * 9 * C * 4, "im2col s2 " + std::to_string(H) + "x" + std::to_string(Wd) + " C" + std::to_string(C),
                       [=](cudaStream_t s) { launch_im2col_s2(x16, col, N, H, Wd, C, s); });
          d.act0 = col; d.C0 = 9 * C; d.taps0 = 1;
        } else {
          void* up = s16(kA1, Ho, Wo, C);
          if (create)
            pl->add_op("resample", 0, static_cast<double>(N) * Ho * Wo * C * 2.5, "nearest 2x " + std::to_string(H) + "x" + std::to_string(Wd) + " C" + std::to_string(C),
                       [=](cudaStream_t s) { launch_upsample2x_h16(x16, up, N, H, Wd, C, s); });
          d.act0 = up; d.C0 = C; d.taps0 = 9;
        }
        bind(d, r.w);
        write_to(d, out);
        add_conv(d, &out, 9.0 * C);
      } else {
        const float* src = use32(x);
        if (create) {
          float* dst = out.data; void* dst16 = out.d16; double* st = out.stats;
          const int mode = r.mode;
          pl->add_op("resample", 0, static_cast<double>(N) * (H * Wd + Ho * Wo * 1.5) * C * 4, (mode == 1 ? "nearest 2x f32 " : "avgpool f32 ") + std::to_string(H) + "x" + std::to_string(Wd),
                     [=](cudaStream_t s) { launch_resample_f32(src, dst, dst16, N, H, Wd, C, mode, s); });
          pl->add_op("gn_stats", 0, static_cast<double>(N) * Ho * Wo * C * 4, "", [=](cudaStream_t s) { launch_gn_stats(dst, st, N, Ho * Wo, C, s); });
        }
      }
      if (create) pl->taps.push_back({r.pfx, out.data, out.d16, out.C, out.H, out.W});
      return out;
    };

    for (size_t bi = 1; bi < blocks_.size(); ++bi) {
      const BlockDef& b = blocks_[bi];
      if (create) pl->block_stats[bi] = soff;
      pl->op_block = static_cast<int>(bi);
      bool first = true;
      for (const auto& l : b.layers) {
        switch (l.kind) {
          case LayerKind::kResBlock:
            if (b.is_output && first) {
              Act sk = skips.back();
              skips.pop_back();
              cur = run_res(res_[l.idx], cur, &sk);
            } else {
              cur = run_res(res_[l.idx], cur, nullptr);
            }
            break;
          case LayerKind::kAttention: cur = run_attn(attn_[l.idx], l.idx, cur); break;
          case LayerKind::kResample: cur = run_resample(resample_[l.idx], cur); break;
        }
        first = false;
      }
      if (b.is_input) skips.push_back(cur);
    }
    IVID_REQUIRE(skips.empty(), "internal: skip stack not consumed");

    pl->op_block = -1;
    keep32(cur);
    const bool split_head = out_split_ && cur.has16;
    void* a1 = s16(kA1, SH, SW, cur.C);
    void* a2 = split_head ? s16(kA2, SH, SW, cur.C) : nullptr;
    GnApplyDesc go;
    if (cur.has16) { go.x0 = cur.d16; go.x0_half = true; } else go.x0 = use32(cur);
    go.C0 = cur.C; go.N = N; go.H = SH; go.W = SW; go.mode = 0; go.silu = 1; go.out_act = a1; go.out_lo = a2;
    add_gn(go, cur, nullptr, out_gn_, -1);
    if (split_head) {
      float* Y = s32(kH, SH, SW, 64);
      ConvDesc d;
      d.act0 = a1; d.C0 = cur.C; d.taps0 = 1;
      d.act1 = a2; d.C1 = cur.C; d.taps1 = 1;
      d.act2 = a1; d.C2 = cur.C; d.taps2 = 1;
      bind(d, out1x1_);
      d.out = Y; d.ldc = 64; d.out_mode = 0; d.N = N; d.H = SH; d.W = SW;
      add_conv(d, nullptr, 9.0 * cur.C, static_cast<double>(cfg_.out_channels));
      if (create) {
        const float* ob = Wf(out_conv_.b_off);
        const int Co = cfg_.out_channels;
        pl->add_op("eps_gather", 0, static_cast<double>(N) * SH * SW * (9.0 * Co * 4 + Co * 4), "", [=](cudaStream_t s) {
          if (pl->hook != nullptr) pl->hook->launch(Y, ob, N, SH, SW, Co, 64, s);
          else launch_eps_gather(Y, ob, pl->eps, N, SH, SW, Co, 64, s);
        });
      }
    } else if (create) {
      ConvDesc d;
      d.act0 = a1; d.C0 = cur.C; d.taps0 = 9;
      bind(d, out_conv_);
      d.out = nullptr; d.ldc = 0; d.out_mode = 2; d.N = N; d.H = SH; d.W = SW;
      ConvLaunch* l = conv_launch_create(d);
      pl->convs.push_back(l);
      pl->add_op("conv_gemm<16>", 2.0 * N * SH * SW * 9.0 * cur.C * cfg_.out_channels,
                 static_cast<double>(N) * SH * SW * (cur.C * 2 + cfg_.out_channels * 4), "",
                 [l, pl](cudaStream_t s) { conv_launch_run_out(l, pl->eps, s); });
    }
    if (!create) stats_bytes = soff;
  };

  walk(nullptr);
  size_t total = 0;
  auto place = [&](size_t bytes) {
    const size_t off = (total + 1023) & ~size_t(1023);
    total = off + bytes;
    return off;
  };
  stats_off = place(stats_bytes);
  for (int s = 0; s < kSlots; ++s) slot_off[s] = place(slot_bytes[s]);
  for (auto& o : outs) {
    const size_t n = static_cast<size_t>(N) * o.H * o.W * o.C;
    if (conv_can_out16(o.C)) o.off16 = place(n * 2);
    o.only16 = o.may16 && !o.need32;
    if (!o.only16) o.off32 = place(n * 4);
  }
  IVID_CHECK_CUDA(cudaMalloc(&pl->ws, total + 4096));
  pl->ws_bytes = total;
  pl->stats_base = reinterpret_cast<double*>(pl->ws + stats_off);
  pl->stats_bytes = stats_bytes;
  walk(pl->ws);
  return plan.release();
}

bool Unet::can_fuse_head(int W) const {
  return out_split_ && conv_can_out16(final_ch_) && cfg_.out_channels == 4 && W % 4 == 0;
}

void Unet::forward(const float* x, int Nx, int H, int W, const ivid_cond_t* cond, const int64_t* t, const int64_t* classes,
                   float* eps, int N, cudaStream_t stream, const HeadHook* hook, int cache_branch, const AttnPerturb* pert) {
  if (!finalized()) throw Error(kErrState, "AdmUnet2d: forward before .cuda()/finalize");
  IVID_REQUIRE(cache_branch >= -1 && cache_branch <= cfg_.num_res_blocks,
               "cache_branch must be in [0, num_res_blocks] = [0, " + std::to_string(cfg_.num_res_blocks) + "]");
  check_geometry(H, W);
  IVID_REQUIRE(N >= 1 && Nx >= 1 && N % Nx == 0, "forward: N must be a positive multiple of Nx");
  IVID_REQUIRE(classes == nullptr || cfg_.num_classes > 0, "this model is not class-conditioned");
  IVID_CHECK_CUDA(cudaSetDevice(device_));
  ivid_cond_t cnd = cond ? *cond : ivid_cond_t{};
  const int expect_in = cnd.kind == 1 ? (cnd.mask_rgb_dev ? 10 : 9) : (cnd.kind == 2 ? 8 : cfg_.in_channels);
  IVID_REQUIRE(expect_in == cfg_.in_channels, "forward: conditional inputs do not match the model's in_channels");
  IVID_REQUIRE(hook == nullptr || can_fuse_head(W), "forward: a head hook needs the tap-column output head");
  IVID_REQUIRE(cnd.kind != 2 || (cnd.sr_scale >= 0 && H % std::max(cnd.sr_scale, 1) == 0 && W % std::max(cnd.sr_scale, 1) == 0),
               "forward: the super-resolution scale must divide the input size");
  IVID_REQUIRE(hook != nullptr || eps != nullptr, "forward: eps output missing");
  AttnPerturb pt;
  pt.row0 = N;
  if (pert != nullptr && !pert->layers.empty()) {
    IVID_REQUIRE(pert->row0 >= 0 && pert->row0 <= N, "forward: the perturbed-row start must lie in [0, N]");
    pt.layers = pert->layers;
    std::sort(pt.layers.begin(), pt.layers.end());
    for (size_t i = 0; i < pt.layers.size(); ++i) {
      IVID_REQUIRE(pt.layers[i] >= 0 && pt.layers[i] < num_attention_layers(),
                   "forward: attention layer index " + std::to_string(pt.layers[i]) + " out of range [0, " +
                       std::to_string(num_attention_layers()) + ")");
      IVID_REQUIRE(i == 0 || pt.layers[i] != pt.layers[i - 1], "forward: an attention layer is listed twice");
    }
    pt.row0 = pert->row0;
    if (pt.row0 == N) pt.layers.clear();
  }

  Plan* pl = get_plan(N, H, W, pt);
  if (cache_branch >= 0 && !pl->cache_valid)
    throw Error(kErrState, "reuse forward: no full forward of this batch size and input size has run since the plan was built");
  pl->x = x; pl->Nx = Nx; pl->t = t; pl->classes = classes; pl->eps = eps;
  pl->cond = cnd;
  pl->cond_stream_dev = cond_stream_dev_;
  pl->hook = hook;
  if (cache_branch < 0) pl->cache_valid = true;
  if (!profile_) {
    static const bool graphs_on = getenv("IVID_NO_GRAPH") == nullptr;
    ++pl->runs;
    if (graphs_on && pl->runs > 1) {
      const Plan::GraphKey key{x, Nx, t, classes, eps, cnd.kind, cnd.y_dev, cnd.mask_dev, cnd.mask_rgb_dev, cnd.noise_dev,
                               cnd.kind != 0 ? cnd.seed : 0ull, cnd.kind != 0 ? cnd.stream_id : 0u, cond_stream_dev_,
                               hook ? hook->key : 0ull, cnd.kind == 2 ? cnd.sr_scale : 0, cache_branch};
      for (auto& g : pl->graphs)
        if (g.key == key) {
          g.last_use = pl->runs;
          ++pl->graph_hits;
          IVID_CHECK_CUDA(cudaGraphLaunch(g.exec, stream));
          return;
        }
      const bool thrash = pl->graph_captures >= 32 && pl->graph_hits < pl->graph_captures;
      if (thrash) {
        pl->run(stream, nullptr, cache_branch);
        return;
      }
      ++pl->graph_captures;
      if (cap_stream_ == nullptr) IVID_CHECK_CUDA(cudaStreamCreateWithFlags(&cap_stream_, cudaStreamNonBlocking));
      cudaGraph_t graph = nullptr;
      IVID_CHECK_CUDA(cudaStreamBeginCapture(cap_stream_, cudaStreamCaptureModeRelaxed));
      try {
        pl->run(cap_stream_, nullptr, cache_branch);
      } catch (...) {
        cudaStreamEndCapture(cap_stream_, &graph);
        if (graph) cudaGraphDestroy(graph);
        throw;
      }
      IVID_CHECK_CUDA(cudaStreamEndCapture(cap_stream_, &graph));
      cudaGraphExec_t exec = nullptr;
      const cudaError_t ie = cudaGraphInstantiate(&exec, graph, 0);
      cudaGraphDestroy(graph);
      IVID_CHECK_CUDA(ie);
      if (pl->graphs.size() >= 16) {
        size_t victim = 0;
        for (size_t i = 1; i < pl->graphs.size(); ++i) if (pl->graphs[i].last_use < pl->graphs[victim].last_use) victim = i;
        IVID_CHECK_CUDA(cudaStreamSynchronize(stream));
        cudaGraphExecDestroy(pl->graphs[victim].exec);
        pl->graphs.erase(pl->graphs.begin() + victim);
      }
      pl->graphs.push_back(Plan::GraphEntry{key, exec, pl->runs});
      IVID_CHECK_CUDA(cudaGraphLaunch(exec, stream));
      return;
    }
    pl->run(stream, nullptr, cache_branch);
    return;
  }
  std::vector<cudaEvent_t> ev(pl->ops.size() + 1);
  for (auto& e : ev) IVID_CHECK_CUDA(cudaEventCreate(&e));
  pl->run(stream, ev.data(), cache_branch);
  IVID_CHECK_CUDA(cudaStreamSynchronize(stream));
  for (size_t i = 0; i < pl->ops.size(); ++i) {
    const Plan::OpRec& op = pl->ops[i];
    if (!pl->kept(op.block, cache_branch)) continue;
    float ms = 0.f;
    IVID_CHECK_CUDA(cudaEventElapsedTime(&ms, ev[i], ev[i + 1]));
    auto& agg = profile_acc_[op.label];
    agg.launches += 1; agg.ms += ms; agg.flops += op.flops; agg.bytes += op.bytes;
    if (!op.note.empty()) {
      char buf[256];
      snprintf(buf, sizeof(buf), "[\"%s\", \"%s\", %.5f, %.4e, %.4e]", op.label, op.note.c_str(), ms, op.flops, op.bytes);
      if (!profile_ops_.empty()) profile_ops_ += ", ";
      profile_ops_ += buf;
    }
  }
  for (auto& e : ev) cudaEventDestroy(e);
}

void Unet::debug_tap(int N, const std::string& name, float* host_out, size_t capacity, int* C, int* H, int* W) {
  Plan* pl = nullptr;
  for (auto& p : plans_)
    if (p->N == N && (pl == nullptr || p->last_use > pl->last_use)) pl = p.get();
  if (pl == nullptr) throw Error(kErrState, "debug_tap: no forward of this batch size has run");
  for (const auto& t : pl->taps) {
    if (t.name != name) continue;
    const size_t n = static_cast<size_t>(N) * t.C * t.H * t.W;
    if (C) *C = t.C; if (H) *H = t.H; if (W) *W = t.W;
    if (host_out == nullptr) return;
    IVID_REQUIRE(capacity >= n, "debug_tap: output buffer too small");
    IVID_CHECK_CUDA(cudaSetDevice(device_));
    IVID_CHECK_CUDA(cudaDeviceSynchronize());
    std::vector<float> nhwc(n);
    if (t.d32 != nullptr) {
      IVID_CHECK_CUDA(cudaMemcpy(nhwc.data(), t.d32, n * 4, cudaMemcpyDeviceToHost));
    } else {
      std::vector<__half> h(n);
      IVID_CHECK_CUDA(cudaMemcpy(h.data(), t.d16, n * 2, cudaMemcpyDeviceToHost));
      for (size_t i = 0; i < n; ++i) nhwc[i] = __half2float(h[i]);
    }
    const size_t HW = static_cast<size_t>(t.H) * t.W;
    for (int b = 0; b < N; ++b)
      for (size_t px = 0; px < HW; ++px)
        for (int c = 0; c < t.C; ++c) host_out[(static_cast<size_t>(b) * t.C + c) * HW + px] = nhwc[(static_cast<size_t>(b) * HW + px) * t.C + c];
    return;
  }
  throw Error(kErrInvalidArgument, "debug_tap: unknown layer '" + name + "'");
}

void Unet::profile_begin() { profile_ = true; profile_acc_.clear(); profile_ops_.clear(); }
std::string Unet::profile_end() {
  profile_ = false;
  std::string js = "{";
  bool first = true;
  for (const auto& kv : profile_acc_) {
    if (!first) js += ", ";
    first = false;
    char buf[256];
    snprintf(buf, sizeof(buf), "\"%s\": {\"launches\": %d, \"ms\": %.6f, \"flops\": %.6e, \"bytes\": %.6e}", kv.first.c_str(),
             kv.second.launches, kv.second.ms, kv.second.flops, kv.second.bytes);
    js += buf;
  }
  if (getenv("IVID_PROFILE_OPS") != nullptr) js += ", \"_ops\": [" + profile_ops_ + "]";
  js += "}";
  return js;
}

}
```

Measured before the change: 0.3594.

## Add 256-wide N tile for slab 3x3 convs with fp16 output

Adds a BN=256 variant of the warp-specialized conv GEMM that uses m64n256k16 wgmma, setmaxnreg to shift registers from producer warpgroup to consumers, one block per SM, and a restricted epilogue (fp16 out only, no residual/skip). A table of measured shapes selects the wide tile by default when the grid still fills the SMs. The aim is more operand reuse per tile and fewer B-tile reloads per A slab. The cost is lower occupancy and a larger register footprint, and the shape whitelist is tuned to specific layer sizes.

```diff
diff --git a/include/ivid_b200.h b/include/ivid_b200.h
--- a/include/ivid_b200.h
+++ b/include/ivid_b200.h
@@ -221,6 +221,7 @@
   const float* residual_dev; int residual_up;
   int N, H, W, Cout;
   void* out_dev; int out_mode; void* out16_dev; double* stats_dev;
+  int bn;
 } ivid_op_conv_t;
 int ivid_op_conv2d_ex(const ivid_op_conv_t* args, void* stream);
 typedef struct {
diff --git a/ivid_b200/_lib.py b/ivid_b200/_lib.py
--- a/ivid_b200/_lib.py
+++ b/ivid_b200/_lib.py
@@ -90,6 +90,7 @@
         ("residual_dev", c_void_p), ("residual_up", c_int),
         ("N", c_int), ("H", c_int), ("W", c_int), ("Cout", c_int),
         ("out_dev", c_void_p), ("out_mode", c_int), ("out16_dev", c_void_p), ("stats_dev", c_void_p),
+        ("bn", c_int),
     ]
 
 
diff --git a/ivid_b200/csrc/api.cu b/ivid_b200/csrc/api.cu
--- a/ivid_b200/csrc/api.cu
+++ b/ivid_b200/csrc/api.cu
@@ -297,6 +297,7 @@
     IVID_REQUIRE(a->act1_dev == nullptr || a->wskip_host != nullptr, "conv: a skip input needs its weights (w2_host; wskip_host of ivid_op_conv2d_ex)");
     IVID_REQUIRE(a->act2_dev == nullptr || (a->act1_dev != nullptr && a->C2 > 0), "conv: act2_dev is the second part of a skip over act1_dev");
     IVID_REQUIRE(a->out_mode >= 0 && a->out_mode <= 2, "conv: out_mode must be 0, 1 or 2");
+    IVID_REQUIRE(a->bn == 0 || a->bn == 128 || a->bn == 256, "conv: bn must be 0, 128 or 256");
     const int C1 = a->act1_dev ? a->C1 : 0, C2 = a->act2_dev ? a->C2 : 0;
     const ConvPack pk = conv_pack(a->w0_host, a->b0_host, a->Cout, a->C0, a->ksize, conv_pad_k(a->C0), C1 ? a->wskip_host : nullptr,
                                   C1 ? a->bskip_host : nullptr, C1 + C2, C2 ? C1 : 0, a->e4m3 != 0);
@@ -314,7 +315,7 @@
     d.cout_pad = pk.cout_pad; d.cout = a->Cout; d.bias = static_cast<const float*>(db.p);
     d.residual = a->residual_dev; d.ldr = a->Cout; d.residual_up = a->residual_up != 0;
     d.out = a->out_dev; d.ldc = a->Cout; d.out_mode = a->out_mode; d.out16 = a->out16_dev; d.stats = a->stats_dev;
-    d.N = a->N; d.H = a->H; d.W = a->W;
+    d.N = a->N; d.H = a->H; d.W = a->W; d.bn = a->bn;
     std::unique_ptr<ConvLaunch, void (*)(ConvLaunch*)> l(conv_launch_create(d), conv_launch_destroy);
     conv_launch_run(l.get(), st);
     IVID_CHECK_CUDA(cudaStreamSynchronize(st));
diff --git a/ivid_b200/csrc/common.cuh b/ivid_b200/csrc/common.cuh
--- a/ivid_b200/csrc/common.cuh
+++ b/ivid_b200/csrc/common.cuh
@@ -114,6 +114,11 @@
   for (int i = 0; i < R; ++i) asm volatile("" : "+f"(d[i])::"memory");
 }
 
+template <int R>
+__device__ __forceinline__ void setmaxnreg_inc() { asm volatile("setmaxnreg.inc.sync.aligned.u32 %0;\n" ::"n"(R)); }
+template <int R>
+__device__ __forceinline__ void setmaxnreg_dec() { asm volatile("setmaxnreg.dec.sync.aligned.u32 %0;\n" ::"n"(R)); }
+
 __device__ __forceinline__ uint64_t make_smem_desc_sw128(uint32_t smem_addr, uint32_t sbo_bytes, uint32_t lbo_bytes) {
   uint64_t d = 0;
   d |= static_cast<uint64_t>((smem_addr & 0x3FFFF) >> 4);
@@ -152,6 +157,14 @@
       : "l"(desc_a), "l"(desc_b), "r"(scale_d));
 }
 template <>
+__device__ __forceinline__ void wgmma_ss<256>(float (&d)[128], uint64_t desc_a, uint64_t desc_b, uint32_t scale_d) {
+  asm volatile(
+      "{\n\t.reg .pred p;\n\tsetp.ne.b32 p, %130, 0;\n\t"
+      "wgmma.mma_async.sync.aligned.m64n256k16.f32.f16.f16 {%0, %1, %2, %3, %4, %5, %6, %7, %8, %9, %10, %11, %12, %13, %14, %15, %16, %17, %18, %19, %20, %21, %22, %23, %24, %25, %26, %27, %28, %29, %30, %31, %32, %33, %34, %35, %36, %37, %38, %39, %40, %41, %42, %43, %44, %45, %46, %47, %48, %49, %50, %51, %52, %53, %54, %55, %56, %57, %58, %59, %60, %61, %62, %63, %64, %65, %66, %67, %68, %69, %70, %71, %72, %73, %74, %75, %76, %77, %78, %79, %80, %81, %82, %83, %84, %85, %86, %87, %88, %89, %90, %91, %92, %93, %94, %95, %96, %97, %98, %99, %100, %101, %102, %103, %104, %105, %106, %107, %108, %109, %110, %111, %112, %113, %114, %115, %116, %117, %118, %119, %120, %121, %122, %123, %124, %125, %126, %127}, %128, %129, p, 1, 1, 0, 0;\n\t}\n"
+      : "+f"(d[0]), "+f"(d[1]), "+f"(d[2]), "+f"(d[3]), "+f"(d[4]), "+f"(d[5]), "+f"(d[6]), "+f"(d[7]), "+f"(d[8]), "+f"(d[9]), "+f"(d[10]), "+f"(d[11]), "+f"(d[12]), "+f"(d[13]), "+f"(d[14]), "+f"(d[15]), "+f"(d[16]), "+f"(d[17]), "+f"(d[18]), "+f"(d[19]), "+f"(d[20]), "+f"(d[21]), "+f"(d[22]), "+f"(d[23]), "+f"(d[24]), "+f"(d[25]), "+f"(d[26]), "+f"(d[27]), "+f"(d[28]), "+f"(d[29]), "+f"(d[30]), "+f"(d[31]), "+f"(d[32]), "+f"(d[33]), "+f"(d[34]), "+f"(d[35]), "+f"(d[36]), "+f"(d[37]), "+f"(d[38]), "+f"(d[39]), "+f"(d[40]), "+f"(d[41]), "+f"(d[42]), "+f"(d[43]), "+f"(d[44]), "+f"(d[45]), "+f"(d[46]), "+f"(d[47]), "+f"(d[48]), "+f"(d[49]), "+f"(d[50]), "+f"(d[51]), "+f"(d[52]), "+f"(d[53]), "+f"(d[54]), "+f"(d[55]), "+f"(d[56]), "+f"(d[57]), "+f"(d[58]), "+f"(d[59]), "+f"(d[60]), "+f"(d[61]), "+f"(d[62]), "+f"(d[63]), "+f"(d[64]), "+f"(d[65]), "+f"(d[66]), "+f"(d[67]), "+f"(d[68]), "+f"(d[69]), "+f"(d[70]), "+f"(d[71]), "+f"(d[72]), "+f"(d[73]), "+f"(d[74]), "+f"(d[75]), "+f"(d[76]), "+f"(d[77]), "+f"(d[78]), "+f"(d[79]), "+f"(d[80]), "+f"(d[81]), "+f"(d[82]), "+f"(d[83]), "+f"(d[84]), "+f"(d[85]), "+f"(d[86]), "+f"(d[87]), "+f"(d[88]), "+f"(d[89]), "+f"(d[90]), "+f"(d[91]), "+f"(d[92]), "+f"(d[93]), "+f"(d[94]), "+f"(d[95]), "+f"(d[96]), "+f"(d[97]), "+f"(d[98]), "+f"(d[99]), "+f"(d[100]), "+f"(d[101]), "+f"(d[102]), "+f"(d[103]), "+f"(d[104]), "+f"(d[105]), "+f"(d[106]), "+f"(d[107]), "+f"(d[108]), "+f"(d[109]), "+f"(d[110]), "+f"(d[111]), "+f"(d[112]), "+f"(d[113]), "+f"(d[114]), "+f"(d[115]), "+f"(d[116]), "+f"(d[117]), "+f"(d[118]), "+f"(d[119]), "+f"(d[120]), "+f"(d[121]), "+f"(d[122]), "+f"(d[123]), "+f"(d[124]), "+f"(d[125]), "+f"(d[126]), "+f"(d[127])
+      : "l"(desc_a), "l"(desc_b), "r"(scale_d));
+}
+template <>
 __device__ __forceinline__ void wgmma_rs_tb<64>(float (&d)[32], const uint32_t (&a)[4], uint64_t desc_b, uint32_t scale_d) {
   asm volatile(
       "{\n\t.reg .pred p;\n\tsetp.ne.b32 p, %37, 0;\n\t"
diff --git a/ivid_b200/csrc/conv_gemm.cuh b/ivid_b200/csrc/conv_gemm.cuh
--- a/ivid_b200/csrc/conv_gemm.cuh
+++ b/ivid_b200/csrc/conv_gemm.cuh
@@ -38,6 +38,8 @@
 
 template <int BN, bool SLAB = false>
 struct ConvGemmCfg {
+  static constexpr bool WIDE = BN == 256;
+  static_assert(!WIDE || SLAB, "the 256-wide tile exists in slab K order only");
   static constexpr int BM = 128;
   static constexpr int BK = 64;
   static constexpr int A_BYTES = BM * BK * 2;
@@ -52,7 +54,9 @@
   static constexpr bool STATS_ON_RING = SLAB;
   static constexpr int SMEM_BYTES = RING_BYTES + BAR_BYTES + (STATS_ON_RING ? 0 : STAT_BYTES) + 1024;
   static constexpr int CONSUMER_THREADS = 256;
-  static constexpr int THREADS = CONSUMER_THREADS + 32;
+  static constexpr int THREADS = CONSUMER_THREADS + (WIDE ? 128 : 32);
+  static constexpr int MIN_BLOCKS = WIDE ? 1 : 2;
+  static constexpr int PRODUCER_REGS = 40, CONSUMER_REGS = 232;
 
   static constexpr int F32_CH = SLAB ? BN / 4 : (BN < 32 ? BN : 32);
   static constexpr int F32_BOX = BM * F32_CH * 4;
@@ -63,9 +67,11 @@
   static constexpr int F16_CH = BN < 64 ? BN : 64;
   static constexpr int F16_BOX = BM * F16_CH * 2;
   static constexpr int F16_TILE = BM * BN * 2;
+  static constexpr int F16_AT = WIDE ? SLAB_STAGES * SLAB_BYTES : 0;
   static_assert(UNIT_BOXES * F32_BOX <= UNIT_STRIDE, "an fp32 unit must fit its ring slot");
   static_assert(SLAB ? UNITS == STAGES : UNITS < STAGES && F16_TILE <= STAGE_BYTES, "fp32 units and the fp16 tile must fit the ring");
-  static_assert(!SLAB || F16_TILE + STAT_BYTES <= SLAB_STAGES * SLAB_BYTES, "the fp16 tile and statistics must fit the slab slots");
+  static_assert(!SLAB || F16_TILE + STAT_BYTES <= (WIDE ? STAGES * B_BYTES : SLAB_STAGES * SLAB_BYTES),
+                "the fp16 tile and statistics must fit the slots they lie over");
 };
 
 struct ConvKCursor {
@@ -73,7 +79,7 @@
 };
 
 template <int BN, bool A8 = false, bool SLAB = false>
-__global__ void __launch_bounds__(ConvGemmCfg<BN>::THREADS, 2)
+__global__ void __launch_bounds__(ConvGemmCfg<BN, SLAB>::THREADS, ConvGemmCfg<BN, SLAB>::MIN_BLOCKS)
 conv_gemm_kernel(const __grid_constant__ std::conditional_t<A8, ConvMaps8, ConvMaps> maps, const __grid_constant__ ConvGemmParams p) {
   using Cfg = ConvGemmCfg<BN, SLAB>;
   constexpr int STAGES = Cfg::STAGES;
@@ -84,7 +90,7 @@
   uint64_t* empty_bar = full_bar + STAGES;
   uint64_t* slab_full = empty_bar + STAGES;
   uint64_t* slab_empty = slab_full + SLAB_STAGES;
-  float* stat_smem = reinterpret_cast<float*>(Cfg::STATS_ON_RING ? smem + Cfg::F16_TILE : smem + Cfg::RING_BYTES + Cfg::BAR_BYTES);
+  float* stat_smem = reinterpret_cast<float*>(Cfg::STATS_ON_RING ? smem + Cfg::F16_AT + Cfg::F16_TILE : smem + Cfg::RING_BYTES + Cfg::BAR_BYTES);
   uint8_t* const slab_ring = smem;
   uint8_t* const w_ring = smem + SLAB_STAGES * Cfg::SLAB_BYTES;
 
@@ -121,13 +127,18 @@
   const int n0 = tn * p.TN, h0 = th * p.TH, w0 = tw * p.TW;
   uint8_t* const unit_ring = SLAB ? w_ring : smem;
 
-  if (warp == Cfg::CONSUMER_THREADS / 32) {
-    if (lane == 0) {
+  if constexpr (Cfg::WIDE) {
+    if (warp >= Cfg::CONSUMER_THREADS / 32) setmaxnreg_dec<Cfg::PRODUCER_REGS>();
+    else setmaxnreg_inc<Cfg::CONSUMER_REGS>();
+  }
+
+  if (Cfg::WIDE ? warp >= Cfg::CONSUMER_THREADS / 32 : warp == Cfg::CONSUMER_THREADS / 32) {
+    if (lane == 0 && (!Cfg::WIDE || warp == Cfg::CONSUMER_THREADS / 32)) {
       const int rw0 = p.res_up ? w0 >> 1 : w0, rh0 = p.res_up ? h0 >> 1 : h0;
       tma_prefetch_desc(&maps.a[0]);
       tma_prefetch_desc(&maps.b);
       if constexpr (A8) tma_prefetch_desc(&maps.b8);
-      if (p.residual != nullptr) {
+      if (!Cfg::WIDE && p.residual != nullptr) {
 #pragma unroll
         for (int q = 0; q < Cfg::UNITS * Cfg::UNIT_BOXES; ++q) tma_prefetch_l2_4d(&maps.r, colbase + q * Cfg::F32_CH, rw0, rh0, n0);
       }
@@ -199,7 +210,7 @@
           while (c.seg < 3 && p.seg_chunks[c.seg] == 0) ++c.seg;
         }
       }
-      if (p.residual != nullptr) {
+      if (!Cfg::WIDE && p.residual != nullptr) {
         const uint32_t bytes = static_cast<uint32_t>(Cfg::UNIT_BOXES * Cfg::F32_BOX) >> (p.res_up ? 2 : 0);
 #pragma unroll 1
         for (int i = 0; i < Cfg::UNITS; ++i) {
@@ -313,7 +324,7 @@
 #pragma unroll
   for (int i = 0; i < 2; ++i) ok[i] = n0 + (wg * 64 + wr * 16 + (lane >> 2) + 8 * i) / rows_per_n < p.N;
 
-  if (p.residual != nullptr) {
+  if (!Cfg::WIDE && p.residual != nullptr) {
 #pragma unroll 1
     for (int q = 0; q < Cfg::UNITS; ++q) {
       const uint32_t g = static_cast<uint32_t>(nunits + q);
@@ -341,7 +352,7 @@
         } else {
           v0 = acc[4 * j + 2 * i] + b.x; v1 = acc[4 * j + 2 * i + 1] + b.y;
         }
-        if (p.residual != nullptr) {
+        if (!Cfg::WIDE && p.residual != nullptr) {
           float r0, r1;
           asm volatile("ld.shared.v2.f32 {%0, %1}, [%2];\n" : "=f"(r0), "=f"(r1) : "r"(f32_at(j, tr[i])) : "memory");
           v0 += r0; v1 += r1;
@@ -351,7 +362,7 @@
     }
   }
 
-  if (p.out_mode == 2) {
+  if (!Cfg::WIDE && p.out_mode == 2) {
     const uint32_t hw = static_cast<uint32_t>(p.H) * p.W;
 #pragma unroll
     for (int i = 0; i < 2; ++i) {
@@ -372,7 +383,7 @@
   }
   asm volatile("bar.sync 1, %0;\n" ::"n"(Cfg::CONSUMER_THREADS) : "memory");
 
-  const uint32_t f16_u32 = SLAB ? smem_u32(slab_ring) : smem_u32(smem) + ((s_res + Cfg::UNITS) % STAGES) * Cfg::STAGE_BYTES;
+  const uint32_t f16_u32 = SLAB ? smem_u32(slab_ring + Cfg::F16_AT) : smem_u32(smem) + ((s_res + Cfg::UNITS) % STAGES) * Cfg::STAGE_BYTES;
   uint32_t t32[2], t16[2];
 #pragma unroll
   for (int i = 0; i < 2; ++i) {
@@ -390,7 +401,7 @@
     for (int i = 0; i < 2; ++i) {
       float v0 = acc[4 * j + 2 * i], v1 = acc[4 * j + 2 * i + 1];
       const uint32_t a16 = f16_u32 + (8 * j) / Cfg::F16_CH * Cfg::F16_BOX + (t16[i] ^ ((8 * j) % Cfg::F16_CH) * 2);
-      if (p.out_mode == 0) {
+      if (!Cfg::WIDE && p.out_mode == 0) {
         asm volatile("st.shared.v2.f32 [%0], {%1, %2};\n" ::"r"(f32_at(j, t32[i])), "f"(v0), "f"(v1) : "memory");
         if (p.out16 != nullptr) asm volatile("st.shared.b32 [%0], %1;\n" ::"r"(a16), "r"(pack_h2(v0, v1)) : "memory");
       } else {
@@ -404,7 +415,19 @@
         q0 = fmaf(v0, v0, q0); q1 = fmaf(v1, v1, q1);
       }
     }
-    if (do_stats) {
+    if (Cfg::WIDE && do_stats) {
+      const bool sq = (lane & 4) != 0, hi = (lane & 8) != 0;
+      float k0 = sq ? q0 : s0, k1 = sq ? q1 : s1;
+      k0 += __shfl_xor_sync(0xffffffffu, sq ? s0 : q0, 4);
+      k1 += __shfl_xor_sync(0xffffffffu, sq ? s1 : q1, 4);
+      float k = hi ? k1 : k0;
+      k += __shfl_xor_sync(0xffffffffu, hi ? k0 : k1, 8);
+      k += __shfl_xor_sync(0xffffffffu, k, 16);
+      if (lane < 16) {
+        const uint32_t st = st_u32 + 32 * j + (sq ? 4 * BN : 0) + (hi ? 4 : 0);
+        asm volatile("st.shared.f32 [%0], %1;\n" ::"r"(st), "f"(k) : "memory");
+      }
+    } else if (do_stats) {
 #pragma unroll
       for (int off = 4; off < 32; off <<= 1) {
         s0 += __shfl_xor_sync(0xffffffffu, s0, off);
@@ -422,7 +445,7 @@
   fence_proxy_async_smem();
   asm volatile("bar.sync 1, %0;\n" ::"n"(Cfg::CONSUMER_THREADS) : "memory");
   if (tid == 0) {
-    if (p.out_mode == 0) {
+    if (!Cfg::WIDE && p.out_mode == 0) {
 #pragma unroll
       for (int q = 0; q < Cfg::UNITS * Cfg::UNIT_BOXES; ++q) {
         const int u = q / Cfg::UNIT_BOXES, k = q % Cfg::UNIT_BOXES;
@@ -435,7 +458,7 @@
 #pragma unroll
       for (int q = 0; q < BN / Cfg::F16_CH; ++q) {
         const int col = colbase + q * Cfg::F16_CH;
-        if (col < p.Cout) tma_store_4d(&maps.o16, (SLAB ? slab_ring : smem + ((s_res + Cfg::UNITS) % STAGES) * Cfg::STAGE_BYTES) + q * Cfg::F16_BOX, col, w0, h0, n0);
+        if (col < p.Cout) tma_store_4d(&maps.o16, (SLAB ? slab_ring + Cfg::F16_AT : smem + ((s_res + Cfg::UNITS) % STAGES) * Cfg::STAGE_BYTES) + q * Cfg::F16_BOX, col, w0, h0, n0);
       }
     }
     tma_store_commit();
diff --git a/ivid_b200/csrc/ops.cu b/ivid_b200/csrc/ops.cu
--- a/ivid_b200/csrc/ops.cu
+++ b/ivid_b200/csrc/ops.cu
@@ -108,10 +108,28 @@
 }
 static void epilogue_box_channels(int BN, bool slab, int* f32_ch, int* f16_ch) {
   switch (BN) {
+    case 256: epilogue_box_channels<256, true>(f32_ch, f16_ch); break;
     case 128: slab ? epilogue_box_channels<128, true>(f32_ch, f16_ch) : epilogue_box_channels<128, false>(f32_ch, f16_ch); break;
     case 64: slab ? epilogue_box_channels<64, true>(f32_ch, f16_ch) : epilogue_box_channels<64, false>(f32_ch, f16_ch); break;
     default: slab ? epilogue_box_channels<16, true>(f32_ch, f16_ch) : epilogue_box_channels<16, false>(f32_ch, f16_ch); break;
   }
+}
+
+struct ConvWideShape {
+  int H, W, C0, cout;
+};
+static constexpr ConvWideShape kConvWideShapes[] = {
+    {128, 128, 512, 256}, {128, 128, 256, 256},
+    {64, 64, 768, 256}, {64, 64, 640, 256}, {64, 64, 512, 256}, {64, 64, 512, 512}, {64, 64, 384, 256},
+    {32, 32, 1280, 512}, {32, 32, 1024, 512}, {32, 32, 768, 512}, {32, 32, 768, 768}, {32, 32, 512, 512}, {32, 32, 256, 512},
+    {32, 32, 256, 256},
+    {16, 16, 1024, 1024},
+};
+static bool conv_wide_measured_faster(const ConvDesc& d, int wide_grid) {
+  if (wide_grid < sm_count()) return false;
+  for (const ConvWideShape& c : kConvWideShapes)
+    if (c.H == d.H && c.W == d.W && c.C0 == d.C0 && c.cout == d.cout) return true;
+  return false;
 }
 
 ConvLaunch* conv_launch_create(const ConvDesc& d) {
@@ -136,6 +154,12 @@
   l->slab = any3x3 && p.TN == 1 && p.TW >= 8;
   IVID_REQUIRE(!l->slab || p.TW * (p.TH + 2) * 128 <= (ConvGemmCfg<128, true>::SLAB_BYTES), "internal: conv slab larger than its slot");
   l->BN = conv_pick_bn(d.cout_pad);
+  const bool wide_ok = l->slab && !a8 && d.out_mode == 1 && d.residual == nullptr && d.C1 == 0 && d.C2 == 0 && d.cout % 256 == 0;
+  IVID_REQUIRE(d.bn == 0 || (d.bn == 128 && l->BN == 128) || (d.bn == 256 && wide_ok),
+               "conv: a 256-wide tile needs a 3x3 slab launch with an fp16 output, no residual or skip segment and Cout % 256 == 0; "
+               "a 128-wide tile needs a padded Cout that is a multiple of 128");
+  const int wide_grid = p.tiles_w * p.tiles_h * p.tiles_n * (d.cout_pad / 256);
+  if (d.bn == 256 || (d.bn == 0 && wide_ok && conv_wide_measured_faster(d, wide_grid))) l->BN = 256;
   p.n_blocks = d.cout_pad / l->BN;
   p.seg_chunks[0] = a8 ? conv_pad_k8(d.C0) / 128 : conv_pad_k(d.C0) / 64; p.seg_taps[0] = d.taps0;
   p.acc_scale = d.acc_scale;
@@ -206,6 +230,9 @@
 template <bool A8, bool SLAB>
 static void run_conv_bn(const ConvLaunch* l, cudaStream_t s) {
   switch (l->BN) {
+    case 256:
+      if constexpr (!A8 && SLAB) run_conv<256, false, true>(l, s);
+      break;
     case 128: run_conv<128, A8, SLAB>(l, s); break;
     case 64: run_conv<64, A8, SLAB>(l, s); break;
     default: run_conv<16, A8, SLAB>(l, s); break;
diff --git a/ivid_b200/csrc/ops.h b/ivid_b200/csrc/ops.h
--- a/ivid_b200/csrc/ops.h
+++ b/ivid_b200/csrc/ops.h
@@ -29,6 +29,7 @@
   void* out = nullptr; int ldc = 0; int out_mode = 0;
   double* stats = nullptr;
   int N = 0, H = 0, W = 0;
+  int bn = 0;
 };
 
 ConvLaunch* conv_launch_create(const ConvDesc& d);
diff --git a/ivid_b200/csrc/unet.cu b/ivid_b200/csrc/unet.cu
--- a/ivid_b200/csrc/unet.cu
+++ b/ivid_b200/csrc/unet.cu
@@ -599,12 +599,12 @@
                        (d.C2 > 0 ? static_cast<double>(d.taps2) * d.C2 : 0.0);
       const double M = static_cast<double>(d.N) * d.H * d.W;
       const double Nalg = n_alg > 0.0 ? n_alg : static_cast<double>(d.cout);
-      static const char* names[2][3] = {{"conv_gemm<16>", "conv_gemm<64>", "conv_gemm<128>"},
-                                        {"conv_gemm<16,e4m3>", "conv_gemm<64,e4m3>", "conv_gemm<128,e4m3>"}};
+      static const char* names[2][4] = {{"conv_gemm<16>", "conv_gemm<64>", "conv_gemm<128>", "conv_gemm<256>"},
+                                        {"conv_gemm<16,e4m3>", "conv_gemm<64,e4m3>", "conv_gemm<128,e4m3>", nullptr}};
       const int bn = conv_launch_bn(l);
       const bool a8 = conv_launch_a8(l);
       const double K0 = static_cast<double>(d.taps0) * d.C0;
-      pl->add_op(names[a8 ? 1 : 0][bn == 128 ? 2 : bn == 64 ? 1 : 0], 2.0 * M * K * Nalg,
+      pl->add_op(names[a8 ? 1 : 0][bn == 256 ? 3 : bn == 128 ? 2 : bn == 64 ? 1 : 0], 2.0 * M * K * Nalg,
                  M * (d.C0 * (a8 ? 1 : 2) + (d.C1 + d.C2) * 2) + M * d.cout * ((d.out_mode == 1 ? 2 : 4) + (d.out16 ? 2 : 0) + (d.residual ? 4 : 0)) +
                      (a8 ? K0 + 2 * (K - K0) : 2 * K) * d.cout_pad,
                  std::to_string(d.H) + "x" + std::to_string(d.W) + " " + std::to_string(d.C0) + (d.C1 ? "+" + std::to_string(d.C1) : "") + (d.C2 ? "+" + std::to_string(d.C2) : "") +
```

After: 0.3669, median of 6. 1.02x the previous value.
